# AbnerVictor/OOD-GAN-inversion

Measured on AMD Instinct MI355X. Metric: 1024² face inversions/sec (100 W+ steps), higher is better.
Workload: dtype f16-split (hi+lo f16 operands, f32 accumulate): 3 MFMA/product in every forward conv (fp32-equivalent), 2 in the input-gradient convs (back-propagated gradient rounded to f16 before each contraction, weights keep hi+lo); dL/dW+ vs the float64 reference 1.4e-5..3.6e-5 ('f16s': 1.3e-5..2.6e-5, the ref

## Files before the change

include/oodgan.h:

```cpp
#ifndef OODGAN_H
#define OODGAN_H

#ifdef __cplusplus
extern "C" {
#endif

#define OODGAN_OK 0
#define OODGAN_E_ARG (-1)
#define OODGAN_E_LAUNCH (-2)
#define OODGAN_E_STATE (-3)
#define OODGAN_E_NODEV (-4)

int oodgan_version(void);
const char* oodgan_last_error(void);
int oodgan_device_count(void);
int oodgan_set_tunable(const char* name, long value);
long oodgan_get_tunable(const char* name);
long oodgan_dispatch_count(const char* name);
int oodgan_dispatch_reset(void);
int oodgan_zero(void* p, long bytes, void* stream);

void* oodgan_plan_create(void);
int oodgan_plan_destroy(void* plan);
int oodgan_plan_record_begin(void* plan);
// ... 10 lines not shown
int oodgan_bias_act_bwd(const float* gy, const float* y, float* gx, float* gbias, int B, int C, long HW,
                        float slope, float scale, void* stream);

int oodgan_upfirdn2d(const float* x, const float* kernel, float* y, int planes, int in_h, int in_w,
                     int in_pitch, int out_pitch, int kh, int kw, int up_x, int up_y, int down_x, int down_y,
                     int pad_x0, int pad_x1, int pad_y0, int pad_y1, void* stream);

int oodgan_blur_bias_act(const float* x, const float* kernel, float* y, int B, int C, int in_h, int in_w,
                         int in_pitch, int kh, int kw, int pad0, int pad1, const float* bias, const float* noise,
                         int noise_batch, const float* noise_w, int act, void* stream);


int oodgan_style_affine_fwd(const float* latent, const float* wcat, const float* bcat, const int* row_lat,
                            float* s, int B, int L, int S, int R, float scale, float lr_mul, void* stream);
int oodgan_style_affine_bwd(const float* gs, const float* wcat, const int* lat_start, float* glat,
                            int B, int L, int S, int R, float scale, void* stream);
int oodgan_equal_linear(const float* x, const float* w, const float* b, float* y, int B, int in_dim, int out_dim,
                        float scale, float lr_mul, int activate, void* stream);
int oodgan_equal_linear_grouped(const float* x, const float* w, const float* b, float* y, int B, int G, int in_dim, int out_dim,
                                float scale, float lr_mul, int activate, void* stream);
int oodgan_pixel_norm(const float* x, float* y, int B, int S, void* stream);


int oodgan_weight_sqsum(const float* w, float* wsq, int Co, int Ci, int KK, void* stream);
int oodgan_demod_fwd(const float* s, int s_stride, const float* wsq, float* d, int d_stride,
                     int B, int Ci, int Co, float scale, void* stream);
int oodgan_demod_bwd(const float* s, int s_stride, const float* wsq, const float* d, int d_stride,
                     const float* r, float* gs, int gs_stride, int B, int Ci, int Co, float scale, void* stream);

int oodgan_pack_conv3x3(const float* w, float* wpk, int Co, int Ci, float scale, int transpose, int flip,
                        void* stream);

#define OODGAN_CONV_S1 0
#define OODGAN_CONV_T2 1
#define OODGAN_CONV_S2 2

#define OODGAN_ACT_NONE 0
#define OODGAN_ACT_LRELU 1
#define OODGAN_ACT_PRELU 2

struct oodgan_actbwd_fuse;
typedef struct oodgan_conv_args {
    const float* x;
    const float* wpk;
    const float* in_scale;
    const float* in_shift;
    const float* out_scale;
    const float* bias;
    const float* noise;
    const float* noise_w;
    const float* slope;
    const float* dotx;
    float* dot_part;
    float* y;
    int B, K, M, Hin, Win;
    int in_pitch, out_pitch;
    int in_scale_stride, out_scale_stride;
    int noise_batch;
    int mode, act;
    int dot_nparts;
    const float* in_mul2;
    int x_sform;
    void* ys;
    const float* ys_scale;
    int ys_scale_stride;
    const float* rgb_w;
    const float* rgb_s;
    float* rgb_y;
    int rgb_s_stride;
    float rgb_scale;
    const struct oodgan_actbwd_fuse* fuse;
    int dot_actgrad;
    int groups;
    int y_fform;
    int x_fform;
    int dotx_fform;
    int dotx_sform;
    const float* dotx_scale;
    int dotx_scale_stride;
    void* workspace;
    long workspace_bytes;
    unsigned* ys_vmax;
    int x_hi_only;
} oodgan_conv_args;

typedef struct oodgan_actbwd_fuse {
    const float* g_rgb;
    const float* w_rgb;
    const float* s_rgb;
    const float* noise;
    const float* noise_w;
    const float* bias;
    const float* dscale;
    const float* mul2;
    void* ys;
    float* part_r;
    float* part_t;
    float* part_max;
    int s_rgb_stride, noise_batch, dscale_stride;
    float rgb_scale;
    long nmax;
    int ys_hi_only;
} oodgan_actbwd_fuse;

int oodgan_conv3x3(const oodgan_conv_args* args, void* stream);

long oodgan_pack_conv3x3_f16s_bytes(int Co, int Ci, int transpose);
int oodgan_pack_conv3x3_f16s(const float* w, void* wpk16, float* unscale2, int Co, int Ci, float scale, int transpose,
                             int flip, void* stream);
int oodgan_conv3x3_f16s(const oodgan_conv_args* args, const float* unscale2, void* stream);
int oodgan_conv3x3_f16s_nparts(int mode, int Hin, int Win);
int oodgan_conv3x3_f16s_nparts2(int mode, int Hin, int Win, int x_sform);
int oodgan_conv3x3_s2_fuse_supported(int B, int K, int M, int Hin, int Win);
int oodgan_conv3x3_s2_grouped_supported(int B, int K, int M, int groups, int Hin, int Win);
int oodgan_conv3x3_s1_actgrad_supported(int B, int K, int M, int H, int W);
int oodgan_conv3x3_s1_ys_supported(int B, int K, int M, int H, int W);
int oodgan_conv3x3_xf_supported(int B, int K, int M, int H, int W);
int oodgan_conv3x3_xf_nparts(int B, int H, int W);
long oodgan_conv3x3_tiny_workspace(int mode, int B, int K, int M, int Hin, int Win);

#define OODGAN_VMAX_SLOTS 64
long oodgan_sform_bytes(int B, int C, int H, int W);
int oodgan_to_sform(const float* x, const float* scale, int scale_stride, const float* shift, int shift_stride,
                    const float* mul2, void* out, int B, int C, int H, int W, int in_pitch, unsigned* vmax, void* stream);
long oodgan_sform_phases_bytes(int B, int C, int H, int W);
int oodgan_from_sform(const void* xs, const float* scale, int scale_stride, float* y, int B, int C, int H, int W, void* stream);
int oodgan_blurT_to_sform_phases(const float* g, const float* kernel, const float* scale, int scale_stride,
                                 const float* mul2, void* out, int B, int C, int H, int W, void* stream);
int oodgan_to_sform_phases(const float* x, const float* scale, int scale_stride, const float* mul2, void* out, int B,
                           int C, int H, int W, int in_pitch, void* stream);
int oodgan_to_sform_phases_padtl(const float* x, const float* scale, int scale_stride, const float* mul2, void* out, int B,
                                 int C, int H, int W, int in_pitch, void* stream);
int oodgan_conv3x3_nparts(int mode, int Hin, int Win);
int oodgan_absmax_scaled(const float* x, const float* s, int s_stride, unsigned* vmax, int B, int C, long HW, void* stream);
int oodgan_fwd_range_update(unsigned* vmax, float* q, int* flag, int n, void* stream);
int oodgan_fwd_range_plan(const float* s_all, const float* d_all, const int* row_layer, const int* drow_layer, const float* q,
                          float* s_sc, float* d_sc, int B, int R, int DR, int row0, int nrows, int drow0, int ndrows,
                          void* stream);

int oodgan_blur_act_sform(const float* z, const float* kernel, float* y, void* ys, const float* ys_scale, int ys_scale_stride,
                          const float* bias, const float* noise, int noise_batch, const float* noise_w, int act, int B, int C,
                          int H, int W, int in_pitch, unsigned* vmax, void* stream);
int oodgan_blur_act_fform(const float* z, const float* kernel, float* y, const float* ys_scale, int ys_scale_stride,
                          const float* bias, const float* noise, int noise_batch, const float* noise_w, int act,
                          int B, int C, int H, int W, int in_pitch, unsigned* vmax, int kernel_rank_one, void* stream);
int oodgan_upconv_vblur_supported(int B, int K, int M, int H, int W);
int oodgan_upconv_vblur_fform(const void* xs, const void* wpk2, long wset_bytes, const float* unscale4, const float* kh4,
                              const float* out_scale, int out_scale_stride, const float* bias, const float* noise, int noise_batch,
                              const float* noise_w, int act, const float* ys_scale, int ys_scale_stride, unsigned* vmax, float* y,
                              int B, int K, int M, int H, int W, void* stream);
int oodgan_blur_act_sform_sep(const float* z, const float* kernel, float* y, void* ys, const float* ys_scale, int ys_scale_stride,
                              const float* bias, const float* noise, int noise_batch, const float* noise_w, int act, int B, int C,
                              int H, int W, int in_pitch, unsigned* vmax, int kernel_rank_one, void* stream);

int oodgan_act_bwd_sform_nparts(int H, int W);
int oodgan_act_bwd_sform(const float* g_feat, const float* out, const float* noise, int noise_batch, const float* noise_w,
                         const float* bias, const float* g_rgb, const float* w_rgb, const float* s_rgb, int s_rgb_stride,
                         float rgb_scale, const float* dscale, int dscale_stride, const float* mul2, void* ys, float* part_r,
                         float* part_t, float* part_max, int B, int C, int H, int W, void* stream);
int oodgan_act_bwd_sform_f(const float* out_f, const float* noise, int noise_batch, const float* noise_w, const float* bias,
                           const float* g_rgb, const float* w_rgb, const float* s_rgb, int s_rgb_stride, float rgb_scale,
                           const float* dscale, int dscale_stride, const float* mul2, void* ys, float* part_r, float* part_t,
                           float* part_max, int B, int C, int H, int W, void* stream);
int oodgan_from_fform(const float* f, float* y, int B, int C, int H, int W, void* stream);
int oodgan_act_bwd_blurT_nparts(int H, int W);
int oodgan_act_bwd_blurT_pre_supported(int H, int W);
int oodgan_act_bwd_blurT_sform_phases(const float* g_feat, const float* out, const float* noise, int noise_batch,
                                      const float* noise_w, const float* bias, const float* g_rgb, const float* w_rgb,
                                      const float* s_rgb, int s_rgb_stride, float rgb_scale, const float* dscale,
                                      int dscale_stride, const float* mul2, const float* kernel, void* out_phases,
                                      float* part_r, float* part_t, float* part_max, int B, int C, int H, int W, void* stream);
int oodgan_act_bwd_blurT_hi_supported(int H, int W);
int oodgan_conv3x3_s1_xh_supported(int B, int K, int M, int H, int W);
int oodgan_act_bwd_blurT_sform_phases_hi(const float* g_feat, const float* out, const float* noise, int noise_batch, const float* noise_w,
                                         const float* bias, const float* dscale, int dscale_stride, const float* mul2, const float* kernel,
                                         void* out_phases, float* part_r, float* part_max, int B, int C, int H, int W, void* stream);
int oodgan_absmax_scale_check(const float* part, long n, float* state, int* flag, void* stream);

typedef struct oodgan_reduce_job {
    const float* part;
    float* out;
    int B, C, nparts, out_stride, accumulate;
    const float* part2;
    const float* scale2;
    int nparts2, scale2_stride;
} oodgan_reduce_job;
typedef struct oodgan_demod_bwd_job {
    const float* s; const float* wsq; const float* d; const float* r; float* gs;
    int s_stride, d_stride, gs_stride, B, Ci, Co;
    float scale;
} oodgan_demod_bwd_job;
typedef struct oodgan_demod_fwd_job {
    const float* s; const float* wsq; float* d;
    int s_stride, d_stride, B, Ci, Co;
    float scale;
} oodgan_demod_fwd_job;
typedef struct oodgan_scale_check_job {
    const float* part; long n; float* state;
} oodgan_scale_check_job;
int oodgan_reduce_batch(const oodgan_reduce_job* jobs, int njobs, void* stream);
int oodgan_demod_bwd_batch(const oodgan_demod_bwd_job* jobs, int njobs, void* stream);
int oodgan_demod_fwd_batch(const oodgan_demod_fwd_job* jobs, int njobs, void* stream);
int oodgan_absmax_scale_check_batch(const oodgan_scale_check_job* jobs, int njobs, int* flag, void* stream);

long oodgan_hform_bytes(int B, int C, int H, int W);
int oodgan_to_hform(const float* x, void* out, int B, int C, int H, int W, void* stream);
int oodgan_from_hform(const void* in, float* y, int B, int C, int H, int W, void* stream);
long oodgan_modconv_f16_wbytes(int B, int M, int K);
int oodgan_modconv_f16_pack(const float* weight, const float* style, int style_stride, float scale, int demodulate,
                            int act, void* wpk, int B, int M, int K, void* stream);
int oodgan_modconv_f16_pack_affine(const float* weight, const float* latent, int latent_stride, const float* mod_weight,
                                   const float* mod_bias, int S, float scale, int demodulate, int act, void* wpk, int B, int M,
                                   int K, void* stream);
int oodgan_modconv_f16(const void* x, const void* wpk, const float* noise, int noise_batch, const float* noise_w,
                       const float* bias, int act, void* y, int B, int K, int M, int H, int W, void* stream);
int oodgan_reduce_parts(const float* part, float* out, long rows, int nparts, int accumulate, void* stream);
int oodgan_reduce_parts_cols(const float* part, float* out, int B, int C, int nparts, int out_stride, int accumulate,
                             void* stream);


int oodgan_torgb_fwd(const float* x, const float* w, const float* s, int s_stride, const float* bias,
                     const float* skip, const float* kernel, float* y, int B, int Ci, int H, int W,
                     float scale, void* stream);
int oodgan_torgb_fwd_sform(const float* x, const float* w, const float* s, int s_stride, const float* bias,
                           const float* skip, const float* kernel, float* y, void* ys, const float* ys_scale,
                           int ys_scale_stride, int B, int Ci, int H, int W, float scale, unsigned* vmax, void* stream);
int oodgan_rgb_finish(const float* partial, const float* bias, const float* skip, const float* kernel, float* y, int B, int H,
                      int W, void* stream);
int oodgan_rgb_finish_parts(const float* partial, int nparts, const float* bias, const float* skip, const float* kernel, float* y, int B,
                            int H, int W, void* stream);

int oodgan_feature_modulation(const float* x, const float* c0, const float* c1, float* y, long n, int mode, void* stream);

int oodgan_act_bwd_fused(const float* g_feat, const float* out, const float* noise, int noise_batch,
                         const float* noise_w, const float* bias, const float* g_rgb, const float* w_rgb,
                         const float* s_rgb, int s_rgb_stride, float rgb_scale, float* g_pre,
                         float* part_r, float* part_rgb, int B, int C, long HW, void* stream);
int oodgan_act_bwd_nparts(long HW);
int oodgan_act_bwd_fused_max(const float* g_feat, const float* out, const float* noise, int noise_batch,
                             const float* noise_w, const float* bias, const float* g_rgb, const float* w_rgb,
                             const float* s_rgb, int s_rgb_stride, float rgb_scale, float* g_pre,
                             float* part_r, float* part_rgb, float* part_max, const float* dscale, int dscale_stride, int B,
                             int C, long HW, void* stream);
int oodgan_absmax_scale(const float* part, long n, float* out2, void* stream);
int oodgan_absmax_scale_clear(float* part, long n, float* out2, void* stream);


int oodgan_mse_fwd_bwd(const float* img, const float* target, float* gimg, float* part, float* loss,
                       int B, long CHW, float grad_mul, void* stream);
int oodgan_mse_nparts(long CHW);
int oodgan_mse_fwd_bwd_row(const float* img, const float* target, float* gimg, float* part, float* loss_table,
                           const int* row_dev, int nrows, int B, long CHW, float grad_mul, void* stream);
int oodgan_composite_mse_fwd_bwd(const float* img, const float* target, const float* beta, float* gimg, float* comp, float* part,
                                 float* loss, int B, int C, long HW, int wrt_gen, float grad_mul, void* stream);
int oodgan_composite_mse_fwd_bwd_row(const float* img, const float* target, const float* beta, float* gimg, float* comp, float* part,
                                     float* loss_table, const int* row_dev, int nrows, int B, int C, long HW, int wrt_gen,
                                     float grad_mul, void* stream);
int oodgan_scale_by_plane(float* g, const float* beta, int B, int C, long HW, void* stream);
int oodgan_loss_weight_from_alpha(const float* alpha, float* beta, long n, int power, void* stream);
// ... 59 lines not shown
```

ood-gan-inversion_amd/csrc/bwd_producers.hip:

```cpp
#include "common.hpp"
#include "sform.hpp"
#include <type_traits>
#include <cstdint>
#include <cstdlib>

using namespace oodgan;

typedef _Float16 half8 __attribute__((ext_vector_type(8)));
typedef _Float16 half2v __attribute__((ext_vector_type(2)));

namespace {

struct SPDims { int KC, Hq, Wq; long plane; };

__host__ __device__ inline SPDims sp_dims(int C, int H, int W) {
    SPDims d;
    d.KC = (C + 15) / 16;
    d.Hq = (H + 7) / 8 * 8 + 2;
    d.Wq = (W + 31) / 32 * 32 + 2;
    d.plane = (long)d.Hq * d.Wq * 4;
    return d;
}

struct ActArgs {
    const float* g_feat;
    const float* out;
    const float* noise;
    const float* noise_w;
    const float* bias;
    const float* g_rgb;
    const float* w_rgb;
    const float* s_rgb;
    const float* dscale;
    const float* mul2;
    float* part_r;
    float* part_t;
    float* part_max;
    int noise_batch, s_rgb_stride, dscale_stride;
    float rgb_scale;
    int B, C, H, W, nparts;
};


struct ConstSel { int which, c; bool has; };
__device__ __forceinline__ ConstSel const_sel(const ActArgs& a, int kc) {
    const int t = threadIdx.x;
    ConstSel s;
    s.which = t >> 4;
    s.c = kc * 16 + (t & 15);
    s.has = s.which < 4 ? a.g_rgb != nullptr : s.which == 4 ? a.bias != nullptr : a.dscale != nullptr;
    return s;
}

__device__ __forceinline__ float fetch_const(const ActArgs& a, int b, int kc) {
    float raw = 0.f;
    if (threadIdx.x < 112) {
        const ConstSel s = const_sel(a, kc);
        const int cc = min(s.c, a.C - 1);
        const float* src = a.part_r;
        if (s.has) {
            if (s.which < 3) src = a.w_rgb + s.which * a.C + cc;
            else if (s.which == 3) src = a.s_rgb + (long)b * a.s_rgb_stride + cc;
            else if (s.which == 4) src = a.bias + cc;
            else src = a.dscale + (long)b * a.dscale_stride + cc;
        }
        raw = *src;
    }
    return raw;
}

__device__ __forceinline__ void put_const(const ActArgs& a, int kc, float (*cst)[16], float raw) {
    const int t = threadIdx.x;
    if (t < 112) {
        const ConstSel s = const_sel(a, kc);
        const float m2 = a.mul2 ? a.mul2[1] : 1.f;
        float v;
        if (s.which < 3) v = s.has ? raw * a.rgb_scale : 0.f;
        else if (s.which <= 4) v = s.has ? raw : 0.f;
        else if (s.which == 5) v = (s.has ? raw : 1.f) * m2;
        else v = s.has ? fabsf(raw) : 1.f;
        cst[t >> 4][t & 15] = s.c < a.C ? v : 0.f;
    }
}

__device__ __forceinline__ void load_consts(const ActArgs& a, int b, int kc, float (*cst)[16]) { put_const(a, kc, cst, fetch_const(a, b, kc)); }

constexpr int kP1Chunk = 512;
constexpr int kP1Pitch = kP1Chunk + 4;

__global__ __launch_bounds__(256) void act_bwd_sform_kernel(const ActArgs a, uint4* __restrict__ ys, const SDims yd) {
    __shared__ __attribute__((aligned(16))) float lst[16 * kP1Pitch];
    __shared__ float cst[7][16];
    __shared__ float redm[4];
    const int KC = yd.KC;
    const int bk = blockIdx.y, b = bk / KC, kc = bk % KC;
    const int tid = threadIdx.x;
    const long HW = (long)a.H * a.W;
    load_consts(a, b, kc, cst);
    __syncthreads();
    const float nw = a.noise ? (a.noise_w ? a.noise_w[0] : 1.f) : 0.f;
    const float* np = a.noise ? a.noise + (long)(a.noise_batch > 1 ? b : 0) * HW : nullptr;
    const float* gr = a.g_rgb ? a.g_rgb + (long)b * 3 * HW : nullptr;
    const long p0 = (long)blockIdx.x * kP1Chunk;
    float amax = 0.f;
    {
        const int ch = tid >> 4, q = tid & 15, c = kc * 16 + ch;
        const float w0 = cst[0][ch], w1 = cst[1][ch], w2 = cst[2][ch], sr = cst[3][ch], bv = cst[4][ch], ds = cst[5][ch];
        const long cbase = ((long)b * a.C + c) * HW;
        float acc_r = 0.f, acc_t = 0.f;
#pragma unroll
        for (int k = 0; k < kP1Chunk / 64; ++k) {
            const int lp = 4 * (q + 16 * k);
            const long p = p0 + lp;
            float4 v = make_float4(0.f, 0.f, 0.f, 0.f);
            if (c < a.C && p < HW) {
                const float4 o4 = *reinterpret_cast<const float4*>(a.out + cbase + p);
                float4 g4 = make_float4(0.f, 0.f, 0.f, 0.f), nz = g4, r0 = g4, r1 = g4, r2 = g4;
                if (a.g_feat) g4 = *reinterpret_cast<const float4*>(a.g_feat + cbase + p);
                if (np) nz = *reinterpret_cast<const float4*>(np + p);
                if (gr) {
                    r0 = *reinterpret_cast<const float4*>(gr + p);
                    r1 = *reinterpret_cast<const float4*>(gr + HW + p);
                    r2 = *reinterpret_cast<const float4*>(gr + 2 * HW + p);
// ... 283 lines not shown
    if (tid == 0) a.part_max[((long)b * sp.KC + kc) * a.nparts + tile] = fmaxf(fmaxf(redm[0], redm[1]), fmaxf(redm[2], redm[3]));
    const int ch = tid >> 4, tq = tid & 15;
    const int yrow = tq >> 1, xh = tq & 1;
    float o[32];
    if (sep_ok) {
        float kv[4], kh[4];
#pragma unroll
        for (int i = 0; i < 4; ++i) { kv[i] = ksep[3 - i]; kh[i] = ksep[4 + 3 - i]; }
#pragma unroll
        for (int hf = 0; hf < 2; ++hf) {
            float tmp[20];
#pragma unroll
            for (int j = 0; j < 20; ++j) tmp[j] = 0.f;
#pragma unroll
            for (int aa = 0; aa < 4; ++aa) {
                const float2* row = reinterpret_cast<const float2*>(lin + ch * BT_Q + (yrow + aa) * BT_P + 32 * xh + 16 * hf + 2);
#pragma unroll
                for (int j = 0; j < 10; ++j) {
                    const float2 v = row[j];
                    tmp[2 * j] += kv[aa] * v.x;
                    tmp[2 * j + 1] += kv[aa] * v.y;
                }
            }
#pragma unroll
            for (int j = 0; j < 16; ++j)
                o[16 * hf + j] = kh[0] * tmp[j] + kh[1] * tmp[j + 1] + kh[2] * tmp[j + 2] + kh[3] * tmp[j + 3];
        }
    } else {
#pragma unroll
        for (int j = 0; j < 32; ++j) o[j] = 0.f;
#pragma unroll
        for (int aa = 0; aa < 4; ++aa) {
            const float* row = lin + ch * BT_Q + (yrow + aa) * BT_P + 32 * xh + 2;
            float win[35];
#pragma unroll
            for (int j = 0; j < 35; ++j) win[j] = row[j];
#pragma unroll
            for (int bb = 0; bb < 4; ++bb) {
                const float kv = kf[(3 - aa) * 4 + (3 - bb)];
#pragma unroll
                for (int j = 0; j < 32; ++j) o[j] += kv * win[j + bb];
            }
        }
    }
    const float sc_ = cst[5][ch];
    __syncthreads();
    float* lst = lin;
#pragma unroll
    for (int j = 0; j < 32; ++j) {
        const int Xl = 32 * xh + j;
        const int ph = (yrow & 1) * 2 + (Xl & 1);
        lst[ch * BX_CH + ph * BX_PH + (yrow >> 1) * 32 + ((Xl >> 1) ^ ((yrow & 4) << 1))] = o[j] * sc_;
    }
    __syncthreads();
#pragma unroll
    for (int rep = 0; rep < 2; ++rep) {
        const int pos = tid + rep * 256;
        const int ph = pos >> 7, il = (pos >> 5) & 3, jl = pos & 31;
        const int i = i0 + il, j = j0 + jl;
        if (i > H || j > W) continue;
        half8 h0, h1, l0, l1;
#pragma unroll
        for (int cc = 0; cc < 16; ++cc) {
            float v = lst[cc * BX_CH + ph * BX_PH + il * 32 + (jl ^ ((il & 2) << 2))];
            const int Y = 2 * i + (ph >> 1), X = 2 * j + (ph & 1);
            if (Y > 2 * H || X > 2 * W) v = 0.f;
            const _Float16 hh = (_Float16)v;
            const _Float16 ll = (_Float16)(v - (float)hh);
            if (cc < 8) { h0[cc] = hh; l0[cc] = ll; } else { h1[cc - 8] = hh; l1[cc - 8] = ll; }
        }
        half8* rec = reinterpret_cast<half8*>(outp + ((((long)b * sp.KC + kc) * 4 + ph) * sp.plane + ((long)i * sp.Wq + j) * 4));
        rec[0] = h0; rec[1] = h1; rec[2] = l0; rec[3] = l1;
    }
}


struct StripGeo {
    int nstrips, nseg, seg_rows;
    int tiles_x, tiles_y;
    int extra;
    int hi_only;
};

template <int QN, bool XTRA, bool PRE>
__global__ __launch_bounds__(16 * QN) __attribute__((amdgpu_waves_per_eu((PRE && !XTRA) ? 4 : 2, 4))) void act_bwd_blurT_strip_kernel(const ActArgs a, const float* __restrict__ kern, uint4* __restrict__ outp,
                                                                   int H, int W, SPDims sp, StripGeo geo) {
    constexpr int SW = 4 * QN, NT = 16 * QN, NWV = NT / 64;
    constexpr int BS_RP = SW + 4;
    constexpr int BS_GP = SW + 4;
    static_assert(QN == 16, "a channel row is one DPP row of 16 lanes");
    __shared__ __attribute__((aligned(16))) float gat[2][2][16][BS_GP];
    __shared__ float cst[7][16];
    __shared__ float redm[NWV];
    const int tid = threadIdx.x;
    int w;
    {
        const int total = gridDim.x, bid = blockIdx.x, xcd = bid & 7, idx = bid >> 3, q = total >> 3, r = total & 7;
        w = (xcd < r ? xcd * (q + 1) : r * (q + 1) + (xcd - r) * q) + idx;
    }
    const int strip = w % geo.nstrips; w /= geo.nstrips;
    const int seg = w % geo.nseg; w /= geo.nseg;
    const int kc = w % sp.KC, b = w / sp.KC;
    const int Hg = 2 * H, Wg = 2 * W;
    const long HW = (long)Hg * Wg;
    const int i0 = seg * geo.seg_rows;
    const int i1 = min(i0 + geo.seg_rows, H + 1);
    const int X0 = SW * strip, j0 = (SW / 2) * strip;
    const bool xtra = XTRA && strip == geo.nstrips - 1;
    const float cval = fetch_const(a, b, kc);
    float kp[4][4];
#pragma unroll
    for (int aa = 0; aa < 4; ++aa)
#pragma unroll
        for (int bb = 0; bb < 4; ++bb) kp[aa][bb] = kern[(3 - aa) * 4 + (3 - bb)];
    float kv[4], kh[4];
    bool rank1 = kp[0][0] != 0.f;
    {
        float kmax = 0.f;
#pragma unroll
        for (int aa = 0; aa < 4; ++aa)
#pragma unroll
            for (int bb = 0; bb < 4; ++bb) kmax = fmaxf(kmax, fabsf(kp[aa][bb]));
#pragma unroll
        for (int aa = 0; aa < 4; ++aa) {
            kv[aa] = rank1 ? kp[aa][0] / kp[0][0] : 0.f;
            kh[aa] = kp[0][aa];
        }
#pragma unroll
        for (int aa = 0; aa < 4; ++aa)
#pragma unroll
            for (int bb = 0; bb < 4; ++bb) rank1 = rank1 && fabsf(kp[aa][bb] - kv[aa] * kh[bb]) <= 1e-7f * kmax;
#pragma unroll
        for (int aa = 0; aa < 4; ++aa)
            kv[aa] = __builtin_bit_cast(float, __builtin_amdgcn_readfirstlane(__builtin_bit_cast(int, kv[aa])));
    }
    const int ch = tid / QN, q = tid % QN, c = kc * 16 + ch;
    float bv = 0.f, sc_ = 0.f;
    const int csw = (ch >> 3) & 1;
    const float nw = a.noise ? (a.noise_w ? a.noise_w[0] : 1.f) : 0.f;
    const float* np = a.noise ? a.noise + (long)(a.noise_batch > 1 ? b : 0) * HW : nullptr;
    const long cbase = ((long)b * a.C + c) * HW;
    const bool cok = c < a.C;
    const int gxm = X0 + 4 * q;
    const bool vm = cok && gxm + 3 < Wg;
    const bool vl = cok && q == 0 && X0 >= 2;
    const bool vr = cok && q == QN - 1 && X0 + SW < Wg;

    struct Rows { float4 o[PRE ? 1 : 2], g[2], n[2]; float2 oe[PRE ? 1 : 2], ge[2]; };
    const int gxc = min(gxm, Wg - 4);
    const int ecol = q == QN - 1 ? min(X0 + SW, Wg - 2) : max(X0 - 2, 0);
    const long cbase_c = ((long)b * a.C + min(c, a.C - 1)) * HW;
    const float* gsrc = a.g_feat ? a.g_feat : a.out;
    const bool has_g = a.g_feat != nullptr;
    const float* nsrc = np ? np : gsrc + cbase_c;
    const bool has_n = np != nullptr && gxm + 3 < Wg;
    auto load_rows = [&](int i, Rows& R) __attribute__((always_inline)) {
#pragma unroll
        for (int rr = 0; rr < 2; ++rr) {
            const int rc = min(max(2 * i + 1 + rr, 0), Hg - 1);
            const long p = cbase_c + (long)rc * Wg;
            if (!PRE) {
                R.o[PRE ? 0 : rr] = *reinterpret_cast<const float4*>(a.out + p + gxc);
                R.oe[PRE ? 0 : rr] = *reinterpret_cast<const float2*>(a.out + p + ecol);
            }
            R.g[rr] = *reinterpret_cast<const float4*>(gsrc + p + gxc);
            R.ge[rr] = *reinterpret_cast<const float2*>(gsrc + p + ecol);
            R.n[rr] = *reinterpret_cast<const float4*>(nsrc + (long)rc * Wg + gxc);
        }
    };

    float acc_r = 0.f, amax = 0.f;
    float pend[3][4], pendx[3] = {0.f, 0.f, 0.f};
#pragma unroll
    for (int k = 0; k < 3; ++k)
#pragma unroll
        for (int e = 0; e < 4; ++e) pend[k][e] = 0.f;

    auto step = [&](int i, const Rows& R, auto r1_c) __attribute__((always_inline)) {
        constexpr bool R1 = decltype(r1_c)::value;
        float done[2][4];
        float (*gt)[16][BS_GP] = gat[i & 1];
#pragma unroll
        for (int rr = 0; rr < 2; ++rr) {
            const int r = 2 * i + 1 + rr;
            const bool rok = r >= 0 && r < Hg;
            const bool own = r >= 2 * i0 + 1 || (seg == 0 && r == 0);
            const bool mg = rok && vm && has_g, mn = rok && has_n;
            const bool me0 = rok && has_g && (vl || vr), me1 = rok && has_g && vl;
            const float gv[4] = {mg ? R.g[rr].x : 0.f, mg ? R.g[rr].y : 0.f, mg ? R.g[rr].z : 0.f, mg ? R.g[rr].w : 0.f};
            float gp[4], e0, e1;
            const float nv[4] = {mn ? R.n[rr].x : 0.f, mn ? R.n[rr].y : 0.f, mn ? R.n[rr].z : 0.f, mn ? R.n[rr].w : 0.f};
            const float ge0 = me0 ? R.ge[rr].x : 0.f, ge1 = me1 ? R.ge[rr].y : 0.f;
            if (PRE) {
#pragma unroll
                for (int e = 0; e < 4; ++e) {
                    gp[e] = gv[e];
                    if (own) {
                        acc_r -= gp[e] * (nw * nv[e] + bv);
                        amax = fmaxf(amax, fabsf(gp[e]));
                    }
                }
                e0 = ge0;
                e1 = ge1;
            } else {
                const float4 o4 = R.o[PRE ? 0 : rr];
                const float2 oe = R.oe[PRE ? 0 : rr];
                const bool mo = rok && vm;
                const float ov[4] = {mo ? o4.x : 0.f, mo ? o4.y : 0.f, mo ? o4.z : 0.f, mo ? o4.w : 0.f};
#pragma unroll
                for (int e = 0; e < 4; ++e) {
                    const float o = ov[e];
                    gp[e] = gv[e] * (o > 0.f ? kSqrt2 : 0.2f * kSqrt2);
                    if (own) {
                        const float ycv = (o > 0.f ? o * kInvPos : o * kInvNeg) - nw * nv[e] - bv;
                        acc_r += gp[e] * ycv;
                        amax = fmaxf(amax, fabsf(gp[e]));
                    }
                }
                e0 = ge0 * (oe.x > 0.f ? kSqrt2 : 0.2f * kSqrt2);
                e1 = ge1 * (oe.y > 0.f ? kSqrt2 : 0.2f * kSqrt2);
            }
            float lz = __builtin_bit_cast(float, __builtin_amdgcn_update_dpp(0, __builtin_bit_cast(int, gp[2]), 0x111, 0xF, 0xF, false));
            float lw = __builtin_bit_cast(float, __builtin_amdgcn_update_dpp(0, __builtin_bit_cast(int, gp[3]), 0x111, 0xF, 0xF, false));
            float rx = __builtin_bit_cast(float, __builtin_amdgcn_update_dpp(0, __builtin_bit_cast(int, gp[0]), 0x101, 0xF, 0xF, false));
            if (q == 0) { lz = e0; lw = e1; }
            if (q == QN - 1) rx = e0;
            const float x[7] = {lz, lw, gp[0], gp[1], gp[2], gp[3], rx};
            float dxx = 0.f;
            if constexpr (R1) {
#pragma unroll
                for (int e = 0; e < 4; ++e) {
                    const float hr = __builtin_fmaf(kh[3], x[e + 3], __builtin_fmaf(kh[2], x[e + 2], __builtin_fmaf(kh[1], x[e + 1], kh[0] * x[e])));
                    done[rr][e] = __builtin_fmaf(kv[3], hr, pend[0][e]);
                    pend[0][e] = __builtin_fmaf(kv[2], hr, pend[1][e]);
                    pend[1][e] = __builtin_fmaf(kv[1], hr, pend[2][e]);
                    pend[2][e] = kv[0] * hr;
                }
                if (XTRA && xtra && q == QN - 1) {
                    const float hr = __builtin_fmaf(kh[1], x[5], kh[0] * x[4]);
                    dxx = __builtin_fmaf(kv[3], hr, pendx[0]);
                    pendx[0] = __builtin_fmaf(kv[2], hr, pendx[1]);
                    pendx[1] = __builtin_fmaf(kv[1], hr, pendx[2]);
                    pendx[2] = kv[0] * hr;
                }
            } else {
                float fresh[4];
#pragma unroll
                for (int e = 0; e < 4; ++e) {
                    done[rr][e] = pend[0][e] + (kp[3][0] * x[e] + kp[3][1] * x[e + 1] + kp[3][2] * x[e + 2] + kp[3][3] * x[e + 3]);
                    pend[0][e] = pend[1][e] + (kp[2][0] * x[e] + kp[2][1] * x[e + 1] + kp[2][2] * x[e + 2] + kp[2][3] * x[e + 3]);
                    pend[1][e] = pend[2][e] + (kp[1][0] * x[e] + kp[1][1] * x[e + 1] + kp[1][2] * x[e + 2] + kp[1][3] * x[e + 3]);
                    fresh[e] = kp[0][0] * x[e] + kp[0][1] * x[e + 1] + kp[0][2] * x[e + 2] + kp[0][3] * x[e + 3];
                }
#pragma unroll
                for (int e = 0; e < 4; ++e) pend[2][e] = fresh[e];
                if (XTRA && xtra && q == QN - 1) {
                    dxx = pendx[0] + (kp[3][0] * x[4] + kp[3][1] * x[5]);
                    pendx[0] = pendx[1] + (kp[2][0] * x[4] + kp[2][1] * x[5]);
                    pendx[1] = pendx[2] + (kp[1][0] * x[4] + kp[1][1] * x[5]);
                    pendx[2] = kp[0][0] * x[4] + kp[0][1] * x[5];
                }
            }
            if (XTRA && xtra && q == QN - 1 && i >= i0) gt[rr][ch][SW ^ csw] = dxx * sc_;
        }
        if (i >= i0) {
#pragma unroll
            for (int rr = 0; rr < 2; ++rr) {
                const float d0 = done[rr][0] * sc_, d1 = done[rr][1] * sc_, d2 = done[rr][2] * sc_, d3 = done[rr][3] * sc_;
                *reinterpret_cast<float4*>(&gt[rr][ch][4 * q]) = csw ? make_float4(d1, d0, d3, d2) : make_float4(d0, d1, d2, d3);
            }
        }
        __syncthreads();
        if (i >= i0) {
            static_assert(4 * SW == NT, "one gather task per thread");
            const int ph = tid / SW, v = tid % SW;
            const int py = ph >> 1, px = ph & 1, jl = v >> 1, hf = v & 1;
            const int j = j0 + jl, Xl = 2 * jl + px;
            if (j <= W) {
                const bool zero = (2 * i + py > 2 * H) || (X0 + Xl > 2 * W);
                half8 h8, l8;
#pragma unroll
                for (int cc = 0; cc < 8; ++cc) {
                    float val = gt[py][8 * hf + cc][Xl ^ hf];
                    if (zero) val = 0.f;
                    const _Float16 hh = (_Float16)val;
                    h8[cc] = hh;
                    l8[cc] = (_Float16)(val - (float)hh);
                }
                if (geo.hi_only) {
                    half8* recp = reinterpret_cast<half8*>(outp + ((((long)b * sp.KC + kc) * 4 + ph) * sp.plane + ((long)i * sp.Wq + j) * 2));
                    recp[hf] = h8;
                } else {
                    half8* recp = reinterpret_cast<half8*>(outp + ((((long)b * sp.KC + kc) * 4 + ph) * sp.plane + ((long)i * sp.Wq + j) * 4));
                    recp[hf] = h8;
                    recp[2 + hf] = l8;
                }
            }
            if (XTRA && xtra && tid < 16) {
                const int ph = tid >> 2, sl = tid & 3, py = ph >> 1, px = ph & 1;
                const bool zero = px == 1 || (2 * i + py > 2 * H);
                half8 o8;
#pragma unroll
                for (int cc = 0; cc < 8; ++cc) {
                    float val = zero ? 0.f : gt[py][8 * (sl & 1) + cc][SW ^ (sl & 1)];
                    const _Float16 hh = (_Float16)val;
                    o8[cc] = (sl & 2) ? (_Float16)(val - (float)hh) : hh;
                }
                if (geo.hi_only) {
                    if (sl < 2) reinterpret_cast<half8*>(outp + ((((long)b * sp.KC + kc) * 4 + ph) * sp.plane + ((long)i * sp.Wq + W) * 2))[sl] = o8;
                } else {
                    half8* recp = reinterpret_cast<half8*>(outp + ((((long)b * sp.KC + kc) * 4 + ph) * sp.plane + ((long)i * sp.Wq + W) * 4));
                    recp[sl] = o8;
                }
            }
        }
    };

    Rows ra, rb;
    load_rows(i0 - 2, ra);
    put_const(a, kc, cst, cval);
    __syncthreads();
    bv = cst[4][ch];
    sc_ = cst[5][ch];
    int i = i0 - 2;
    auto walk = [&](auto r1_c) __attribute__((always_inline)) {
        for (; i + 1 < i1; i += 2) {
            load_rows(i + 1, rb);
            step(i, ra, r1_c);
            load_rows(i + 2, ra);
            step(i + 1, rb, r1_c);
        }
        if (i < i1) step(i, ra, r1_c);
    };
    if (rank1) walk(std::true_type{});
    else walk(std::false_type{});

#pragma unroll
    for (int o = QN / 2; o > 0; o >>= 1) acc_r += __shfl_xor(acc_r, o, 64);
    auto put = [&](float* tab, int row, int rows_used, float v) {
        const int r1 = row == rows_used - 1 ? geo.tiles_y : row + 1;
        const int c1 = strip == geo.nstrips - 1 ? geo.tiles_x : strip + 1;
        for (int r = row; r < r1; ++r)
            for (int cx = strip; cx < c1; ++cx) tab[(long)r * geo.tiles_x + cx] = (r == row && cx == strip) ? v : 0.f;
    };
    if (q == 0 && cok) put(a.part_r + ((long)b * a.C + c) * a.nparts, seg, geo.nseg, acc_r);
    amax *= cst[6][ch];
#pragma unroll
    for (int o = 32; o > 0; o >>= 1) amax = fmaxf(amax, __shfl_xor(amax, o, 64));
    if ((tid & 63) == 0) redm[tid >> 6] = amax;
    __syncthreads();
    if (tid == 0) {
        float m = redm[0];
        for (int wv = 1; wv < NWV; ++wv) m = fmaxf(m, redm[wv]);
        put(a.part_max + ((long)b * sp.KC + kc) * a.nparts, seg, geo.nseg, m);
    }
}

__global__ __launch_bounds__(1024) void absmax_scale_check_kernel(const float* __restrict__ part, long n, float* __restrict__ state,
                                                                  int* __restrict__ flag) {
    __shared__ float red[16];
    float m = 0.f;
    bool bad = false;
    for (long i = threadIdx.x; i < n; i += 4096) {
        float v[4];
#pragma unroll
        for (int u = 0; u < 4; ++u) v[u] = i + 1024 * u < n ? part[i + 1024 * u] : 0.f;
#pragma unroll
        for (int u = 0; u < 4; ++u) {
            if (!isfinite(v[u])) bad = true;
            m = fmaxf(m, fabsf(v[u]));
        }
    }
#pragma unroll
    for (int o = 32; o > 0; o >>= 1) m = fmaxf(m, __shfl_xor(m, o, 64));
    if (__any(bad) && (threadIdx.x & 63) == 0) atomicOr(flag, 2);
    if ((threadIdx.x & 63) == 0) red[threadIdx.x >> 6] = m;
    __syncthreads();
    if (threadIdx.x == 0) {
        m = red[0];
#pragma unroll
        for (int i = 1; i < 16; ++i) m = fmaxf(m, red[i]);
        const float used = state[1];
        if (m > 0.f && isfinite(m)) {
            const float scaled = m * used;
            if (!(scaled >= 0.00390625f && scaled < 32768.f)) atomicOr(flag, 1);
        }
        int e = 0;
        if (m > 0.f && isfinite(m)) e = 9 - (int)floorf(log2f(m));
        e = e < -100 ? -100 : (e > 100 ? 100 : e);
        state[0] = ldexpf(1.f, -e);
        state[1] = ldexpf(1.f, e);
    }
}

int fill_args(ActArgs& a, const float* g_feat, const float* out, const float* noise, int noise_batch, const float* noise_w,
              const float* bias, const float* g_rgb, const float* w_rgb, const float* s_rgb, int s_rgb_stride, float rgb_scale,
              const float* dscale, int dscale_stride, const float* mul2, float* part_r, float* part_t, float* part_max, int B,
              int C, int H, int W) {
    OODGAN_REQUIRE(part_r && part_max && mul2 && B > 0 && C > 0 && H > 0 && W > 0, "act_bwd producer: bad args");
    OODGAN_REQUIRE(out || (g_feat && !g_rgb), "act_bwd producer: without out, g_feat must be the pre-activation gradient (no ToRGB branch)");
    OODGAN_REQUIRE(!g_rgb || (w_rgb && s_rgb && part_t), "act_bwd producer: rgb branch needs w_rgb, s_rgb and part_t");
    OODGAN_REQUIRE(noise == nullptr || noise_batch == 1 || noise_batch == B, "act_bwd producer: noise_batch");
    OODGAN_REQUIRE((W % 4) == 0, "act_bwd producer: W must be a multiple of 4");
    a.g_feat = g_feat; a.out = out; a.noise = noise; a.noise_w = noise_w; a.bias = bias;
    a.g_rgb = g_rgb; a.w_rgb = w_rgb; a.s_rgb = s_rgb; a.dscale = dscale; a.mul2 = mul2;
    a.part_r = part_r; a.part_t = g_rgb ? part_t : nullptr; a.part_max = part_max;
    a.noise_batch = noise_batch; a.s_rgb_stride = s_rgb_stride; a.dscale_stride = dscale_stride; a.rgb_scale = rgb_scale;
    a.B = B; a.C = C; a.H = H; a.W = W;
    return OODGAN_OK;
}

}

extern "C" int oodgan_act_bwd_sform_nparts(int H, int W) { return (int)(((long)H * W + kP1Chunk - 1) / kP1Chunk); }

extern "C" int oodgan_act_bwd_sform(const float* g_feat, const float* out, const float* noise, int noise_batch,
                                    const float* noise_w, const float* bias, const float* g_rgb, const float* w_rgb,
                                    const float* s_rgb, int s_rgb_stride, float rgb_scale, const float* dscale, int dscale_stride,
                                    const float* mul2, void* ys, float* part_r, float* part_t, float* part_max, int B, int C,
                                    int H, int W, void* stream) {
    ActArgs a;
    int rc = fill_args(a, g_feat, out, noise, noise_batch, noise_w, bias, g_rgb, w_rgb, s_rgb, s_rgb_stride, rgb_scale, dscale,
                       dscale_stride, mul2, part_r, part_t, part_max, B, C, H, W);
    if (rc != OODGAN_OK) return rc;
    OODGAN_REQUIRE(ys != nullptr, "act_bwd_sform: null output");
    const SDims yd = sform_dims(C, H, W);
    a.nparts = oodgan_act_bwd_sform_nparts(H, W);
    OODGAN_REQUIRE((long)B * yd.KC <= 65535, "act_bwd_sform: B*C too large");
    hipLaunchKernelGGL(act_bwd_sform_kernel, dim3(a.nparts, B * yd.KC), dim3(256), 0, as_stream(stream), a,
                       reinterpret_cast<uint4*>(ys), yd);
    return check_launch("act_bwd_sform");
}

extern "C" int oodgan_act_bwd_sform_f(const float* out_f, const float* noise, int noise_batch, const float* noise_w, const float* bias,
                                      const float* g_rgb, const float* w_rgb, const float* s_rgb, int s_rgb_stride, float rgb_scale,
                                      const float* dscale, int dscale_stride, const float* mul2, void* ys, float* part_r, float* part_t,
                                      float* part_max, int B, int C, int H, int W, void* stream) {
    ActArgs a;
    int rc = fill_args(a, nullptr, out_f, noise, noise_batch, noise_w, bias, g_rgb, w_rgb, s_rgb, s_rgb_stride, rgb_scale, dscale,
                       dscale_stride, mul2, part_r, part_t, part_max, B, C, H, W);
    if (rc != OODGAN_OK) return rc;
    OODGAN_REQUIRE(ys != nullptr && (C % 16) == 0 && (reinterpret_cast<uintptr_t>(out_f) & 15) == 0,
                   "act_bwd_sform_f: needs ys, C %% 16 == 0 and a 16-byte aligned F-form input");
    const SDims yd = sform_dims(C, H, W);
    a.nparts = oodgan_act_bwd_sform_nparts(H, W);
    OODGAN_REQUIRE((long)B * yd.KC <= 65535, "act_bwd_sform_f: B*C too large");
    hipLaunchKernelGGL(act_bwd_sform_f_kernel, dim3(a.nparts, B * yd.KC), dim3(256), 0, as_stream(stream), a,
                       reinterpret_cast<uint4*>(ys), yd);
    return check_launch("act_bwd_sform_f");
}

extern "C" int oodgan_from_fform(const float* f, float* y, int B, int C, int H, int W, void* stream) {
    OODGAN_REQUIRE(f && y && B > 0 && C > 0 && (C % 16) == 0 && H > 0 && W > 0, "from_fform: bad args");
    const long HW = (long)H * W, total = (long)B * C * HW;
    hipLaunchKernelGGL(from_fform_kernel, dim3(stream_grid(total, 256)), dim3(256), 0, as_stream(stream), f, y, C, HW, total);
    return check_launch("from_fform");
}

static bool blurT_strip_enabled() { return oodgan::tunable(oodgan::OODGAN_TUN_BLURT_STRIP) != 0; }

extern "C" int oodgan_act_bwd_blurT_pre_supported(int H, int W) { return H >= 32 && W >= 32 && blurT_strip_enabled() ? 1 : 0; }

extern "C" int oodgan_act_bwd_blurT_nparts(int H, int W) { return ((W + 1 + 31) / 32) * ((H + 1 + 3) / 4); }

static int act_bwd_blurT_impl(const float* g_feat, const float* out, const float* noise, int noise_batch, const float* noise_w, const float* bias,
                              const float* g_rgb, const float* w_rgb, const float* s_rgb, int s_rgb_stride, float rgb_scale, const float* dscale,
                              int dscale_stride, const float* mul2, const float* kernel, void* out_phases, float* part_r, float* part_t, float* part_max,
                              int B, int C, int H, int W, void* stream, int hi_only);

extern "C" int oodgan_act_bwd_blurT_hi_supported(int H, int W) { return H >= 32 && W >= 32 && blurT_strip_enabled() ? 1 : 0; }

extern "C" int oodgan_act_bwd_blurT_sform_phases(const float* g_feat, const float* out, const float* noise, int noise_batch,
                                                 const float* noise_w, const float* bias, const float* g_rgb,
                                                 const float* w_rgb, const float* s_rgb, int s_rgb_stride, float rgb_scale,
                                                 const float* dscale, int dscale_stride, const float* mul2,
                                                 const float* kernel, void* out_phases, float* part_r, float* part_t,
                                                 float* part_max, int B, int C, int H, int W, void* stream) {
    return act_bwd_blurT_impl(g_feat, out, noise, noise_batch, noise_w, bias, g_rgb, w_rgb, s_rgb, s_rgb_stride, rgb_scale, dscale, dscale_stride, mul2, kernel,
                              out_phases, part_r, part_t, part_max, B, C, H, W, stream, 0);
}

extern "C" int oodgan_act_bwd_blurT_sform_phases_hi(const float* g_feat, const float* out, const float* noise, int noise_batch,
                                                    const float* noise_w, const float* bias, const float* dscale, int dscale_stride,
                                                    const float* mul2, const float* kernel, void* out_phases, float* part_r, float* part_max,
                                                    int B, int C, int H, int W, void* stream) {
    OODGAN_REQUIRE(oodgan_act_bwd_blurT_hi_supported(H, W), "act_bwd_blurT hi-only records: the strip walk only (H, W >= 32, tunable blurt_strip)");
    return act_bwd_blurT_impl(g_feat, out, noise, noise_batch, noise_w, bias, nullptr, nullptr, nullptr, 0, 0.f, dscale, dscale_stride, mul2, kernel,
                              out_phases, part_r, nullptr, part_max, B, C, H, W, stream, 1);
}

static int act_bwd_blurT_impl(const float* g_feat, const float* out, const float* noise, int noise_batch, const float* noise_w, const float* bias,
                              const float* g_rgb, const float* w_rgb, const float* s_rgb, int s_rgb_stride, float rgb_scale, const float* dscale,
                              int dscale_stride, const float* mul2, const float* kernel, void* out_phases, float* part_r, float* part_t, float* part_max,
                              int B, int C, int H, int W, void* stream, int hi_only) {
    ActArgs a;
    int rc = fill_args(a, g_feat, out, noise, noise_batch, noise_w, bias, g_rgb, w_rgb, s_rgb, s_rgb_stride, rgb_scale, dscale,
                       dscale_stride, mul2, part_r, part_t, part_max, B, C, 2 * H, 2 * W);
    if (rc != OODGAN_OK) return rc;
    OODGAN_REQUIRE(kernel && out_phases, "act_bwd_blurT: null tensor");
    OODGAN_REQUIRE((reinterpret_cast<uintptr_t>(out) & 15) == 0 && (!g_feat || (reinterpret_cast<uintptr_t>(g_feat) & 15) == 0),
                   "act_bwd_blurT: unaligned input");
    OODGAN_REQUIRE(out || oodgan_act_bwd_blurT_pre_supported(H, W), "act_bwd_blurT: the pre-activated form (out == NULL) exists only in the "
                   "strip walk (H, W >= 32)");
    const SPDims d = sp_dims(C, H, W);
    const int tiles_x = (W + 1 + 31) / 32, tiles_y = (H + 1 + 3) / 4;
    a.nparts = tiles_x * tiles_y;
    const long nb = (long)tiles_x * tiles_y * d.KC * B;
    OODGAN_REQUIRE(nb < (1L << 31), "act_bwd_blurT: grid too large");
    if (!g_rgb && !part_t && H >= 32 && W >= 32 && blurT_strip_enabled()) {
        constexpr int QN = 16;
        StripGeo geo;
        geo.hi_only = hi_only;
        geo.extra = ((W % (2 * QN)) == 0 && W <= 32) ? 1 : 0;
        geo.nstrips = geo.extra ? W / (2 * QN) : (W + 1 + 2 * QN - 1) / (2 * QN);
        geo.tiles_x = tiles_x;
        geo.tiles_y = tiles_y;
        const long base = (long)B * d.KC * geo.nstrips;
        long nseg = (4L * 1024) / base;
        if (nseg < 1) nseg = 1;
        int seg_rows = (int)((H + 1 + nseg - 1) / nseg);
        if (seg_rows < 16) seg_rows = 16;
        geo.seg_rows = seg_rows;
        geo.nseg = (H + 1 + seg_rows - 1) / seg_rows;
        OODGAN_REQUIRE(geo.nseg <= tiles_y && geo.nstrips <= tiles_x, "act_bwd_blurT strip: slot table too small");
        const long nbs = base * geo.nseg;
#define OODGAN_STRIP_LAUNCH(X, P)                                                                                              \
    hipLaunchKernelGGL((act_bwd_blurT_strip_kernel<QN, X, P>), dim3((unsigned)nbs), dim3(256), 0, as_stream(stream), a, kernel, \
                       reinterpret_cast<uint4*>(out_phases), H, W, d, geo)
        if (geo.extra) {
            if (out) OODGAN_STRIP_LAUNCH(true, false); else OODGAN_STRIP_LAUNCH(true, true);
        } else {
            if (out) OODGAN_STRIP_LAUNCH(false, false); else OODGAN_STRIP_LAUNCH(false, true);
        }
#undef OODGAN_STRIP_LAUNCH
        return check_launch("act_bwd_blurT_sform_phases/strip");
    }
    OODGAN_REQUIRE(!hi_only, "act_bwd_blurT hi-only records: not reachable (strip walk refused this call)");
    if (g_rgb)
        hipLaunchKernelGGL(act_bwd_blurT_sp_kernel<true>, dim3((unsigned)nb), dim3(256), 0, as_stream(stream), a, kernel,
                           reinterpret_cast<uint4*>(out_phases), H, W, d, tiles_x, tiles_y);
    else
        hipLaunchKernelGGL(act_bwd_blurT_sp_kernel<false>, dim3((unsigned)nb), dim3(256), 0, as_stream(stream), a, kernel,
                           reinterpret_cast<uint4*>(out_phases), H, W, d, tiles_x, tiles_y);
    return check_launch("act_bwd_blurT_sform_phases");
}

extern "C" int oodgan_absmax_scale_check(const float* part, long n, float* state, int* flag, void* stream) {
    OODGAN_REQUIRE(part && state && flag && n > 0, "absmax_scale_check: bad args");
    hipLaunchKernelGGL(absmax_scale_check_kernel, dim3(1), dim3(1024), 0, as_stream(stream), part, n, state, flag);
    return check_launch("absmax_scale_check");
}
```

ood-gan-inversion_amd/csrc/common.hpp:

```cpp
#pragma once
#include <hip/hip_runtime.h>
#include <cstdio>
#include <cstdarg>
#include <functional>
#include <utility>
#include "../../include/oodgan.h"

namespace oodgan {
struct PlanRec;
extern thread_local PlanRec* tl_plan_rec;
extern int g_null_launch;
void plan_append(std::function<void()>&& f);
template <class F>
inline void launch_rec(F&& f) {
    f();
    if (__builtin_expect(tl_plan_rec != nullptr, 0)) plan_append(std::function<void()>(std::forward<F>(f)));
}
}
#undef hipLaunchKernelGGL
#define hipLaunchKernelGGL(kernelName, numBlocks, numThreads, memPerBlock, streamId, ...)                                        \
    ::oodgan::launch_rec([=]() {                                                                                                 \
        if (!::oodgan::g_null_launch) (kernelName)<<<(numBlocks), (numThreads), (memPerBlock), (streamId)>>>(__VA_ARGS__);      \
    })

namespace oodgan {

void set_error(const char* fmt, ...);

enum { OODGAN_TUN_S1_BIG_MIN_ITEMS = 0, OODGAN_TUN_S2_BIG_MIN_ITEMS, OODGAN_TUN_T2_BIG_MIN_ITEMS, OODGAN_TUN_BLURT_STRIP, OODGAN_TUN_BLUR_STRIP, OODGAN_TUN_UPVB_WAVES, OODGAN_TUN_FEWOUT_QUAD, OODGAN_TUN_TINY_MID_MAX, OODGAN_TUN_STRIPX_WAVES, OODGAN_TUN_COUNT };
long tunable(int id);

enum { OODGAN_DC_STRIPX = 0, OODGAN_DC_STRIP, OODGAN_DC_S1BIG, OODGAN_DC_S1V2, OODGAN_DC_S1PP, OODGAN_DC_TINY, OODGAN_DC_T2BIG,
       OODGAN_DC_T2V2, OODGAN_DC_T2GEN, OODGAN_DC_S2BIG, OODGAN_DC_S2V2, OODGAN_DC_S2GEN, OODGAN_DC_UPVB,
       OODGAN_DC_S1BIG_YS, OODGAN_DC_S2BIG_FUSE, OODGAN_DC_S2BIG_DOTXS,
       OODGAN_DC_S1BIG_G2, OODGAN_DC_S2BIG_G2, OODGAN_DC_STRIPX_G2, OODGAN_DC_S2BIG_XH, OODGAN_DC_S1BIG_XH,
       OODGAN_DC_COMPOSITE_MSE, OODGAN_DC_COUNT };
void count_dispatch(int id);

bool bound_device_ok(const char* what);

inline int check_launch(const char* what) {
    hipError_t e = hipGetLastError();
    if (e != hipSuccess) {
        set_error("%s: %s", what, hipGetErrorString(e));
        return OODGAN_E_LAUNCH;
    }
    return OODGAN_OK;
}

#define OODGAN_REQUIRE(cond, ...)          \
    do {                                    \
        if (!(cond)) {                      \
            oodgan::set_error(__VA_ARGS__); \
            return OODGAN_E_ARG;            \
        }                                   \
    } while (0)

constexpr float kSqrt2 = 1.4142135623730951f;
constexpr float kInvPos = 1.f / kSqrt2, kInvNeg = 1.f / (0.2f * kSqrt2);
constexpr int kWave = 64;

inline hipStream_t as_stream(void* s) { return reinterpret_cast<hipStream_t>(s); }

inline int stream_grid(long work_items, int block) {
    long g = (work_items + block - 1) / block;
    if (g > 2048) g = 2048;
    if (g < 1) g = 1;
    return static_cast<int>(g);
}

__device__ __forceinline__ float wave_sum(float v) {
#pragma unroll
    for (int o = 32; o > 0; o >>= 1) v += __shfl_xor(v, o, 64);
    return v;
}

__device__ __forceinline__ float row_sum16(const float* __restrict__ p, int n, int l) {
    float v[4];
#pragma unroll
    for (int u = 0; u < 4; ++u) v[u] = p[min(l + 16 * u, n - 1)];
#pragma unroll
    for (int u = 0; u < 4; ++u) v[u] = l + 16 * u < n ? v[u] : 0.f;
    float r = (v[0] + v[1]) + (v[2] + v[3]);
    r += __shfl_xor(r, 8, 64);
    r += __shfl_xor(r, 4, 64);
    r += __shfl_xor(r, 2, 64);
    r += __shfl_xor(r, 1, 64);
    return r;
}

__device__ __forceinline__ float row_sum_wave(const float* __restrict__ p, int n, int lane) {
    float a0 = 0.f, a1 = 0.f, a2 = 0.f, a3 = 0.f;
    for (int i0 = lane; i0 < n; i0 += 512) {
        float v[8];
#pragma unroll
        for (int u = 0; u < 8; ++u) v[u] = p[min(i0 + 64 * u, n - 1)];
#pragma unroll
        for (int u = 0; u < 8; ++u) v[u] = i0 + 64 * u < n ? v[u] : 0.f;
        a0 += v[0] + v[4]; a1 += v[1] + v[5]; a2 += v[2] + v[6]; a3 += v[3] + v[7];
    }
    return wave_sum((a0 + a1) + (a2 + a3));
}

__device__ __forceinline__ float row_sum(const float* __restrict__ p, int n, int lane) {
    return n <= 64 ? row_sum16(p, n, lane & 15) : row_sum_wave(p, n, lane);
}

__device__ __forceinline__ float demod_dot(const float* __restrict__ sp, const float* __restrict__ wp, int Ci, int lane) {
    float a0 = 0.f, a1 = 0.f, a2 = 0.f, a3 = 0.f;
    for (int c0 = lane; c0 < Ci; c0 += 512) {
        float sv[8], wv[8];
#pragma unroll
        for (int u = 0; u < 8; ++u) {
            const int ci = min(c0 + 64 * u, Ci - 1);
            sv[u] = sp[ci];
            wv[u] = wp[ci];
        }
#pragma unroll
        for (int u = 0; u < 8; ++u) {
// ... 78 lines not shown
```

ood-gan-inversion_amd/csrc/conv_f16s.hip:

```cpp
#include "conv_common.hpp"
#include <cstdlib>
#include <cstdint>

extern "C" int oodgan_conv3x3_f16s_nparts(int mode, int Hin, int Win);

using namespace oodgan;

namespace oodgan {
int launch_s1pp(const oodgan_conv_args& a, const void* wpk16, const float* unscale, hipStream_t st);
int launch_s1v2(const oodgan_conv_args& a, const void* wpk16, const float* unscale, hipStream_t st);
bool s1_strip_eligible(const oodgan_conv_args& a);
bool s1_big_eligible(const oodgan_conv_args& a);
int launch_s1_big(const oodgan_conv_args& a, const void* wpk16, const float* unscale, hipStream_t st);
int launch_s1_strip(const oodgan_conv_args& a, const void* wpk16, const float* unscale, hipStream_t st);
int launch_s1_stripx(const oodgan_conv_args& a, const void* wpk16, const float* unscale, hipStream_t st);
bool tiny_eligible(const oodgan_conv_args& a);
int launch_tiny(const oodgan_conv_args& a, const void* wpk16, const float* unscale, hipStream_t st);
int launch_t2v2(const oodgan_conv_args& a, const void* wpk16, const float* unscale, hipStream_t st);
int launch_s2v2(const oodgan_conv_args& a, const void* wpk16, const float* unscale, hipStream_t st);
bool s2_big_eligible(const oodgan_conv_args& a);
bool t2_big_eligible(const oodgan_conv_args& a);
int launch_t2_big(const oodgan_conv_args& a, const void* wpk16, const float* unscale, hipStream_t st);
int launch_s2_big(const oodgan_conv_args& a, const void* wpk16, const float* unscale, hipStream_t st);
}
// ... 311 lines not shown
}

__global__ __launch_bounds__(256) void pack_f16s_kernel(const float* __restrict__ w, _Float16* __restrict__ out, int Co, int Ci,
                                                        int Mp, float scale, int transpose, int flip,
                                                        const float* __restrict__ sc2) {
    const int K = transpose ? Co : Ci, M = transpose ? Ci : Co;
    const int nchunk = (K + CK - 1) / CK;
    const long total = (long)nchunk * 9 * 2 * Mp * 8;
    const float s2 = sc2[1] * scale;
    for (long e = blockIdx.x * 256L + threadIdx.x; e < total; e += (long)gridDim.x * 256) {
        const int j = (int)(e & 7);
        long r = e >> 3;
        const int m = (int)(r % Mp); r /= Mp;
        const int h = (int)(r & 1); r >>= 1;
        const int tap = (int)(r % 9);
        const int t = (int)(r / 9);
        const int k = t * CK + 8 * h + j;
        float v = 0.f;
        if (m < M && k < K) {
            const int co = transpose ? k : m, ci = transpose ? m : k;
            v = w[((long)co * Ci + ci) * 9 + (flip ? 8 - tap : tap)] * s2;
        }
        const _Float16 hi = (_Float16)v;
        const _Float16 lo = (_Float16)(v - (float)hi);
        const long base = (((long)t * 9 + tap) * 2) * 2;
        out[((base + 0 * 2 + h) * Mp + m) * 8 + j] = hi;
        out[((base + 1 * 2 + h) * Mp + m) * 8 + j] = lo;
    }
}

}

extern "C" int oodgan_conv3x3_f16s_nparts2(int mode, int Hin, int Win, int x_sform) {
    if (mode == OODGAN_CONV_S2 && x_sform) return (((Hin - 1) / 2 + 7) / 8) * (((Win - 1) / 2 + 31) / 32);
    return oodgan_conv3x3_f16s_nparts(mode, Hin, Win);
}

extern "C" int oodgan_conv3x3_f16s_nparts(int mode, int Hin, int Win) {
    if (mode == OODGAN_CONV_S1) return ((Hin + 7) / 8) * ((Win + 31) / 32) ;
    if (mode == OODGAN_CONV_S2) return (((Hin - 1) / 2 + 7) / 8) * (((Win - 1) / 2 + 31) / 32) * 4;
    return 0;
}

extern "C" long oodgan_pack_conv3x3_f16s_bytes(int Co, int Ci, int transpose) {
    const int M = transpose ? Ci : Co, K = transpose ? Co : Ci;
    const long Mp = (M + 63) / 64 * 64;
    return (long)((K + CK - 1) / CK) * 9 * 2 * 2 * Mp * 16;
}

extern "C" int oodgan_pack_conv3x3_f16s(const float* w, void* wpk16, float* unscale2, int Co, int Ci, float scale, int transpose,
                                        int flip, void* stream) {
    OODGAN_REQUIRE(w && wpk16 && unscale2 && Co > 0 && Ci > 0, "pack_conv3x3_f16s: bad args");
    const int M = transpose ? Ci : Co, K = transpose ? Co : Ci;
    const int Mp = (M + 63) / 64 * 64;
    hipStream_t st = as_stream(stream);
    if (hipMemsetAsync(unscale2, 0, 2 * sizeof(float), st) != hipSuccess) {
        set_error("pack_conv3x3_f16s: memset failed");
        return OODGAN_E_LAUNCH;
    }
    hipLaunchKernelGGL(absmax_kernel, dim3(stream_grid((long)Co * Ci * 9, 256 * 16)), dim3(256), 0, st, w, (long)Co * Ci * 9, scale, unscale2);
    hipLaunchKernelGGL(absmax_finish_kernel, dim3(1), dim3(1), 0, st, unscale2);
    const long total = (long)((K + CK - 1) / CK) * 9 * 2 * Mp * 8;
    hipLaunchKernelGGL(pack_f16s_kernel, dim3(stream_grid(total, 256)), dim3(256), 0, st, w, reinterpret_cast<_Float16*>(wpk16),
                       Co, Ci, Mp, scale, transpose, flip, unscale2);
    return check_launch("pack_conv3x3_f16s");
}

extern "C" int oodgan_conv3x3_s1_actgrad_supported(int B, int K, int M, int H, int W) {
    oodgan_conv_args a = {};
    a.mode = OODGAN_CONV_S1; a.x_sform = 1; a.B = B; a.K = K; a.M = M; a.Hin = H; a.Win = W;
    a.y = reinterpret_cast<float*>(1);
    a.dotx = reinterpret_cast<const float*>(1);
    return (s1_strip_eligible(a) || s1_big_eligible(a)) && oodgan_act_bwd_blurT_pre_supported(H / 2, W / 2) && !(H & 1) && !(W & 1) ? 1 : 0;
}

extern "C" int oodgan_conv3x3_s1_xh_supported(int B, int K, int M, int H, int W) {
    oodgan_conv_args a = {};
    a.mode = OODGAN_CONV_S1; a.x_sform = 1; a.B = B; a.K = K; a.M = M; a.Hin = H; a.Win = W;
    a.y = reinterpret_cast<float*>(1);
    a.dotx = reinterpret_cast<const float*>(1);
    return (H > 8 && W > 8 && !s1_strip_eligible(a) && s1_big_eligible(a)) ? 1 : 0;
}

extern "C" int oodgan_conv3x3_s1_ys_supported(int B, int K, int M, int H, int W) {
    oodgan_conv_args a = {};
    a.mode = OODGAN_CONV_S1; a.x_sform = 1; a.B = B; a.K = K; a.M = M; a.Hin = H; a.Win = W;
    a.ys = reinterpret_cast<void*>(1);
    return s1_big_eligible(a) ? 1 : 0;
}

extern "C" int oodgan_conv3x3_f16s(const oodgan_conv_args* args, const float* unscale2, void* stream) {
    OODGAN_REQUIRE(args != nullptr, "conv3x3_f16s: null args");
    const oodgan_conv_args& a = *args;
    OODGAN_REQUIRE(a.x && a.wpk && unscale2 && (a.y || a.x_sform), "conv3x3_f16s: null tensor");
    OODGAN_REQUIRE(a.B > 0 && a.K > 0 && a.M > 0 && a.Hin > 0 && a.Win > 0, "conv3x3_f16s: bad shape");
    OODGAN_REQUIRE(a.act != OODGAN_ACT_PRELU || a.slope, "conv3x3_f16s: PReLU without slopes");
    OODGAN_REQUIRE(a.noise == nullptr || a.noise_batch == 1 || a.noise_batch == a.B, "conv3x3_f16s: noise_batch");
    if (!bound_device_ok("conv3x3_f16s")) return OODGAN_E_ARG;
    if (a.x_fform) {
        OODGAN_REQUIRE(a.x_fform == 1 || a.x_fform == 2, "conv3x3_f16s: x_fform must be 0, 1 or 2");
        count_dispatch(OODGAN_DC_STRIPX);
        return launch_s1_stripx(a, a.wpk, unscale2, as_stream(stream));
    }
    OODGAN_REQUIRE(!a.dotx_fform, "conv3x3_f16s: an F-form dotx exists only with x_fform == 2");
    OODGAN_REQUIRE(a.rgb_y == nullptr || (a.mode == OODGAN_CONV_S1 && a.x_sform), "conv3x3_f16s: fused ToRGB output only for mode S1 with S-form input");
    OODGAN_REQUIRE(a.fuse == nullptr || (a.mode == OODGAN_CONV_S2 && a.x_sform && a.M >= 64),
                   "conv3x3_f16s: the fused activation backward exists only for mode S2 with S-form input and M >= 64");
    OODGAN_REQUIRE(a.groups <= 1 || (a.mode == OODGAN_CONV_S2 && (!a.x_sform || tiny_eligible(a) || s2_big_eligible(a))),
                   "conv3x3_f16s: groups > 1 only for mode S2 with fp32 NCHW input, or a phase-split S-form input of a shape the 8-wave or the skinny-GEMM kernel "
                   "takes (oodgan_conv3x3_s2_grouped_supported; oodgan_conv3x3_tiny_workspace > 0 with a workspace)");
    OODGAN_REQUIRE(!a.y_fform || (a.mode == OODGAN_CONV_S1 && a.x_sform && s1_strip_eligible(a)),
                   "conv3x3_f16s: the F-form output exists only in the strip kernel (mode S1, S-form input, 16 < K,M <= 32)");
    OODGAN_REQUIRE(!a.dot_actgrad || (a.mode == OODGAN_CONV_S1 && a.x_sform && a.dotx && (s1_strip_eligible(a) || s1_big_eligible(a))),
                   "conv3x3_f16s: dot_actgrad exists only in the strip / 8-wave kernels of mode S1 (oodgan_conv3x3_s1_actgrad_supported)");
    OODGAN_REQUIRE(!a.dotx_sform || (a.mode == OODGAN_CONV_S2 && a.x_sform && a.fuse && a.dotx && a.dotx_scale && a.dotx_scale_stride >= a.M &&
                                     !tiny_eligible(a) && s2_big_eligible(a)),
                   "conv3x3_f16s: dotx_sform needs mode S2, a phase-split S-form input, `fuse`, dotx, dotx_scale and a shape of the 8-wave kernel "
                   "(oodgan_conv3x3_s2_fuse_supported)");
    OODGAN_REQUIRE(a.ys_vmax == nullptr || (a.ys != nullptr && a.mode == OODGAN_CONV_S1 && a.x_sform && !tiny_eligible(a) && !s1_strip_eligible(a) && s1_big_eligible(a)),
                   "conv3x3_f16s: ys_vmax only with ys from the 8-wave stride-1 kernel (oodgan_conv3x3_s1_ys_supported)");
    OODGAN_REQUIRE(a.x_hi_only != 2 || (a.x_sform && a.dotx && !tiny_eligible(a) &&
                                        ((a.mode == OODGAN_CONV_S2 && s2_big_eligible(a)) || (a.mode == OODGAN_CONV_S1 && !s1_strip_eligible(a) && s1_big_eligible(a)))),
                   "conv3x3_f16s: x_hi_only = 2 (32-byte hi-only input records) exists only in the two-instruction 8-wave kernels (S-form input, dotx; mode S2 on a "
                   "shape oodgan_conv3x3_s2_fuse_supported accepts, mode S1 on a shape of the 8-wave stride-1 kernel)");
    hipStream_t st = as_stream(stream);
    switch (a.mode) {
        case OODGAN_CONV_S1:
            if (tiny_eligible(a)) { count_dispatch(OODGAN_DC_TINY); return launch_tiny(a, a.wpk, unscale2, st); }
            if (a.x_sform && s1_strip_eligible(a)) { count_dispatch(OODGAN_DC_STRIP); return launch_s1_strip(a, a.wpk, unscale2, st); }
            if (a.x_sform && s1_big_eligible(a)) { count_dispatch(OODGAN_DC_S1BIG); if (a.ys) count_dispatch(OODGAN_DC_S1BIG_YS); return launch_s1_big(a, a.wpk, unscale2, st); }
            OODGAN_REQUIRE(a.rgb_y == nullptr, "conv3x3_f16s: the fused ToRGB output exists only in the strip kernel (16 < K,M <= 32) and, as partial "
                                               "sums together with ys, in the 8-wave kernel (oodgan_conv3x3_s1_ys_supported)");
            if (a.x_sform) { count_dispatch(OODGAN_DC_S1V2); return launch_s1v2(a, a.wpk, unscale2, st); }
            OODGAN_REQUIRE(a.ys == nullptr, "conv3x3_f16s: S-form output needs the S-form input kernel");
            count_dispatch(OODGAN_DC_S1PP);
            return launch_s1pp(a, a.wpk, unscale2, st);
        case OODGAN_CONV_T2:
            if (a.x_sform && t2_big_eligible(a)) { count_dispatch(OODGAN_DC_T2BIG); return launch_t2_big(a, a.wpk, unscale2, st); }
            if (a.x_sform) { count_dispatch(OODGAN_DC_T2V2); return launch_t2v2(a, a.wpk, unscale2, st); }
            count_dispatch(OODGAN_DC_T2GEN);
            return launch_mode<OODGAN_CONV_T2>(a, a.wpk, unscale2, st);
        case OODGAN_CONV_S2:
            OODGAN_REQUIRE((a.Hin & 1) && (a.Win & 1) && a.Hin >= 3 && a.Win >= 3, "conv3x3_f16s S2: input must be odd-sized");
            if (tiny_eligible(a)) { count_dispatch(OODGAN_DC_TINY); return launch_tiny(a, a.wpk, unscale2, st); }
            if (a.x_sform && s2_big_eligible(a)) { count_dispatch(OODGAN_DC_S2BIG); if (a.fuse) count_dispatch(OODGAN_DC_S2BIG_FUSE); if (a.dotx_sform) count_dispatch(OODGAN_DC_S2BIG_DOTXS); return launch_s2_big(a, a.wpk, unscale2, st); }
            if (a.x_sform) { count_dispatch(OODGAN_DC_S2V2); return launch_s2v2(a, a.wpk, unscale2, st); }
            count_dispatch(OODGAN_DC_S2GEN);
            return launch_mode<OODGAN_CONV_S2>(a, a.wpk, unscale2, st);
        default: break;
    }
    set_error("conv3x3_f16s: unknown mode %d", a.mode);
    return OODGAN_E_ARG;
}
```

ood-gan-inversion_amd/csrc/conv_f16s_big.hip:

```cpp
#include "conv_common.hpp"
#include "sform.hpp"
#include <cstdint>
#include <cstdlib>
#include <type_traits>

using namespace oodgan;

typedef _Float16 half8 __attribute__((ext_vector_type(8)));
typedef __attribute__((address_space(3))) void lds_void;

namespace {

constexpr int BG_R = 18, BG_C = 34;
constexpr int BG_XSLOTS = BG_R * BG_C * 4;
constexpr int BG_XPIECES = (BG_XSLOTS + 63) / 64;
constexpr int BG_XBYTES = BG_XPIECES * 1024;
constexpr int BG_WPIECES = 36;
constexpr int BG_STAGE = BG_XBYTES + BG_WPIECES * 1024;
constexpr int BG_PIECES = BG_XPIECES + BG_WPIECES;
constexpr int BG_RED = 2 * BG_STAGE;
constexpr int BG_SMEM = BG_RED + 8 * 64 * 4;

struct BigConv {
    oodgan_conv_args a;
    const uint4* xs;
    SDims xd;
    const float* w_unscale;
    int tiles_x, tiles_y, mblocks, Mp;
    long out_plane;
    SDims yd;
};

constexpr int BG_ZERO = BG_SMEM;
constexpr int BG_ZBYTES = 3584;
constexpr int BG_CST = BG_SMEM + BG_ZBYTES;
constexpr int BG_NZ = BG_CST + 3 * 64 * 4;
constexpr int BG_RGBW = BG_NZ + 2048;
constexpr int BG_SMEM16 = BG_RGBW + 3 * 64 * 4;
typedef float f32x4v __attribute__((ext_vector_type(4)));

#ifdef OODGAN_CLOCK_STAMP
__device__ unsigned long long* g_s1big_stamp = nullptr;
__device__ long g_s1big_stamp_n = 0;
#endif

template <bool DOT, bool PRE, bool YS = false, bool G2 = false>
__global__ __launch_bounds__(512) void conv_f16s_s1big_kernel(const BigConv p, const uint4* __restrict__ wpk16) {
    constexpr int NW = 8, NT = 2;
    extern __shared__ __attribute__((aligned(16))) unsigned char smem[];
    const oodgan_conv_args& a = p.a;
    const int tid = threadIdx.x, lane = tid & 63;
    const int wave = __builtin_amdgcn_readfirstlane(tid >> 6);
    const int n16 = lane & 15, g = lane >> 4;

    int w = xcd_remap(blockIdx.x, gridDim.x);
    const int mblk = w % p.mblocks;
    w /= p.mblocks;
    const int ntile = p.tiles_x * p.tiles_y;
    const int tile = w % ntile, b = w / ntile;
    const int ty = tile / p.tiles_x, tx = tile % p.tiles_x;
    const int r0 = ty * 16, c0 = tx * 32, m0 = mblk * 64;
    const int H = a.Hin, W = a.Win, M = a.M;

    constexpr int NPW = (BG_PIECES + NW - 1) / NW;
    unsigned off[NPW];
    const bool xh = G2 && a.x_hi_only == 2;
    unsigned xmask = 0;
    const int KC = p.xd.KC;
#pragma unroll
    for (int i = 0; i < NPW; ++i) {
        const int pc = wave + NW * i;
        if (pc < BG_XPIECES) {
            int P = pc * 64 + lane;
            if (P >= BG_XSLOTS) P = BG_XSLOTS - 1;
            const int row = P / (BG_C * 4), q = P % (BG_C * 4);
            const int c = q >> 2, sl = ((q & 3) - 2 * ((c >> 2) & 1)) & 3;
            const int rr = min(r0 + row, p.xd.Hp - 1);
            if (xh) {
                off[i] = (unsigned)((((long)rr * p.xd.Wp + (c0 + c)) * 2 + (sl & 1)) * 16);
                if (sl < 2) xmask |= 1u << i;
            } else {
                off[i] = (unsigned)((((long)rr * p.xd.Wp + (c0 + c)) * 4 + sl) * 16);
                xmask |= 1u << i;
            }
        } else {
            xmask |= 1u << i;
            const int u = (pc - BG_XPIECES) * 64 + lane;
            const int row = u >> 6, j = u & 63;
            off[i] = (unsigned)((((long)row * p.Mp) + m0 + j) * 16);
        }
    }
    const unsigned char* xb = reinterpret_cast<const unsigned char*>(p.xs) + (long)b * KC * p.xd.plane * 16;
    const long xplane_bytes = p.xd.plane * 16;
    const unsigned char* wb = reinterpret_cast<const unsigned char*>(wpk16);
    const long wchunk_bytes = (long)36 * p.Mp * 16;
    const int nchunk = (a.K + 15) / 16;
    auto dma_piece = [&](int t, int buf, int i) {
        const int pc = wave + NW * i;
        if (pc >= BG_PIECES) return;
        unsigned char* dst = smem + buf * BG_STAGE;
        const unsigned char* src = (pc < BG_XPIECES ? xb + (long)t * xplane_bytes : wb + (long)t * wchunk_bytes) + off[i];
        if (!G2 || ((xmask >> i) & 1u))
            __builtin_amdgcn_global_load_lds((const __attribute__((address_space(1))) void*)src, (lds_void*)(dst + pc * 1024), 16, 0, 0);
    };
    for (int i = tid; i < BG_ZBYTES / 16; i += 512) reinterpret_cast<uint4*>(smem + BG_ZERO)[i] = make_uint4(0, 0, 0, 0);
    __syncthreads();

    f32x4v acc[4][4];
#pragma unroll
    for (int mt = 0; mt < 4; ++mt)
#pragma unroll
        for (int n = 0; n < 4; ++n) acc[mt][n] = f32x4v{0.f, 0.f, 0.f, 0.f};

    const unsigned laneA = (unsigned)((((g & 1) * 64 + n16) * 16) + (g >> 1) * 4096);
    const unsigned laneA1 = (unsigned)(((g & 1) * 64 + n16) * 16);
    unsigned offBh[4], offBl[4];
#pragma unroll
    for (int pp = 0; pp < 4; ++pp) {
        const int tp = 2 * pp + (g >> 1), ky = tp / 3, kx = tp % 3, col = n16 + kx;
        offBh[pp] = (unsigned)(ky * (BG_C * 64) + col * 64 + ((((g & 1) + 2 * ((col >> 2) & 1)) & 3) << 4));
        offBl[pp] = (unsigned)(ky * (BG_C * 64) + col * 64 + ((((g & 1) + 2 + 2 * ((col >> 2) & 1)) & 3) << 4));
    }
    const int col8 = n16 + 2;
    const unsigned offB1 = (unsigned)(2 * (BG_C * 64) + col8 * 64 + ((((G2 ? (g & 1) : g) + 2 * ((col8 >> 2) & 1)) & 3) << 4));

    struct AF { half8 x[2], y[2]; };
    struct BF { half8 u[4], v[4]; };
    auto load_a = [&](AF& f, const unsigned char* lw, auto pp_c, auto mh_c) {
        constexpr int pp = decltype(pp_c)::value, mh = decltype(mh_c)::value;
// ... 50 lines not shown
#pragma unroll
            for (int i = 0; i < 2; ++i)
#pragma unroll
                for (int n = 0; n < 4; ++n) acc[2 * mh + i][n] = __builtin_amdgcn_mfma_f32_16x16x32_f16(fa.x[i], fb.u[n], acc[2 * mh + i][n], 0, 0, 0);
#pragma unroll
            for (int i = 0; i < 2; ++i)
#pragma unroll
                for (int n = 0; n < 4; ++n) acc[2 * mh + i][n] = __builtin_amdgcn_mfma_f32_16x16x32_f16(fa.y[i], fb.v[n], acc[2 * mh + i][n], 0, 0, 0);
        }
    };
#define BH_IC(n) std::integral_constant<int, n>{}
#define BH_SB() __builtin_amdgcn_sched_barrier(0)
#ifdef OODGAN_CLOCK_STAMP
    const unsigned long long st_t0 = __builtin_amdgcn_s_memtime(), st_r0 = __builtin_amdgcn_s_memrealtime();
#endif
    float cst_o = 0.f, cst_b = 0.f, cst_s = 1.f, rgb_c0 = 0.f, rgb_c1 = 0.f, rgb_c2 = 0.f;
    if (tid < 64 && m0 + tid < M) {
        const int m = m0 + tid;
        cst_o = a.out_scale ? a.out_scale[(long)b * a.out_scale_stride + m] : 1.f;
        if (!DOT && a.bias) cst_b = a.bias[m];
        if (!DOT && a.act == OODGAN_ACT_PRELU) cst_s = a.slope[m];
        if (YS && a.rgb_y) {
            const float sv = a.rgb_scale * a.rgb_s[(long)b * a.rgb_s_stride + m];
            rgb_c0 = sv * a.rgb_w[m]; rgb_c1 = sv * a.rgb_w[M + m]; rgb_c2 = sv * a.rgb_w[2 * M + m];
        }
    }
    const bool has_nz = !DOT && a.noise != nullptr;
    if (has_nz) {
        const int ry = min(r0 + wave * NT + (lane >> 5), H - 1), rx = min(c0 + (lane & 31), W - 1);
        const float* src = a.noise + (long)(a.noise_batch > 1 ? b : 0) * H * W + (long)ry * W + rx;
        __builtin_amdgcn_global_load_lds((const __attribute__((address_space(1))) void*)src, (lds_void*)(smem + BG_NZ + wave * 256), 4, 0, 0);
    }
#pragma unroll
    for (int i = 0; i < NPW; ++i) dma_piece(0, 0, i);
    if (tid < 64) {
        float* cst = reinterpret_cast<float*>(smem + BG_CST);
        cst[tid] = cst_o;
        if (!DOT) { cst[64 + tid] = cst_b; cst[128 + tid] = cst_s; }
        if (YS) {
            float* rw = reinterpret_cast<float*>(smem + BG_RGBW);
            rw[tid] = rgb_c0; rw[64 + tid] = rgb_c1; rw[128 + tid] = rgb_c2;
        }
        __builtin_amdgcn_s_waitcnt(0xC07F);
    }
    for (int t = 0; t < nchunk; ++t) {
        __builtin_amdgcn_s_waitcnt(0x0F70);
        __builtin_amdgcn_s_barrier();
        const bool pf = t + 1 < nchunk;
        const int nb = (t + 1) & 1;
        const unsigned char* lx = smem + (t & 1) * BG_STAGE + (wave * NT) * (BG_C * 64);
        const unsigned char* lw = smem + (t & 1) * BG_STAGE + BG_XBYTES;
        const unsigned col8r = (unsigned)(2 * (BG_C * 64) + col8 * 64 + ((((g & 1) + 2 * ((col8 >> 2) & 1)) & 3) << 4));
        const unsigned char* lz = g < 2 ? lx + col8r : smem + BG_ZERO;
        AF a0, a1;
        BF b0, b1;
#define BH_DMA(i) if (pf && (i) < NPW) dma_piece(t + 1, nb, (i));
        load_b(b0, lx, lz, BH_IC(0), BH_IC(0)); load_b(b0, lx, lz, BH_IC(0), BH_IC(1));
        load_a(a0, lw, BH_IC(0), BH_IC(0));
        BH_SB();
        load_a(a1, lw, BH_IC(0), BH_IC(1)); load_b(b1, lx, lz, BH_IC(1), BH_IC(0)); BH_DMA(0) BH_SB(); mfma_half(a0, b0, BH_IC(0), BH_IC(0)); BH_SB();
        load_a(a0, lw, BH_IC(1), BH_IC(0)); load_b(b1, lx, lz, BH_IC(1), BH_IC(1)); BH_DMA(1) BH_SB(); mfma_half(a1, b0, BH_IC(0), BH_IC(1)); BH_SB();
        load_a(a1, lw, BH_IC(1), BH_IC(1)); load_b(b0, lx, lz, BH_IC(2), BH_IC(0)); BH_DMA(2) BH_SB(); mfma_half(a0, b1, BH_IC(1), BH_IC(0)); BH_SB();
        load_a(a0, lw, BH_IC(2), BH_IC(0)); load_b(b0, lx, lz, BH_IC(2), BH_IC(1)); BH_DMA(3) BH_SB(); mfma_half(a1, b1, BH_IC(1), BH_IC(1)); BH_SB();
        load_a(a1, lw, BH_IC(2), BH_IC(1)); load_b(b1, lx, lz, BH_IC(3), BH_IC(0)); BH_DMA(4) BH_SB(); mfma_half(a0, b0, BH_IC(2), BH_IC(0)); BH_SB();
        load_a(a0, lw, BH_IC(3), BH_IC(0)); load_b(b1, lx, lz, BH_IC(3), BH_IC(1)); BH_DMA(5) BH_SB(); mfma_half(a1, b0, BH_IC(2), BH_IC(1)); BH_SB();
        load_a(a1, lw, BH_IC(3), BH_IC(1)); load_b(b0, lx, lz, BH_IC(4), BH_IC(0)); BH_DMA(6) BH_SB(); mfma_half(a0, b1, BH_IC(3), BH_IC(0)); BH_SB();
        load_a(a0, lw, BH_IC(4), BH_IC(0)); load_b(b0, lx, lz, BH_IC(4), BH_IC(1)); BH_DMA(7) BH_SB(); mfma_half(a1, b1, BH_IC(3), BH_IC(1)); BH_SB();
        load_a(a1, lw, BH_IC(4), BH_IC(1)); BH_DMA(8) BH_SB(); mfma_half(a0, b0, BH_IC(4), BH_IC(0)); BH_SB();
        BH_DMA(9) BH_SB();
        mfma_half(a1, b0, BH_IC(4), BH_IC(1));
#undef BH_DMA
    }
#undef BH_IC
#undef BH_SB
#ifdef OODGAN_CLOCK_STAMP
    if (tid == 0 && g_s1big_stamp && (long)blockIdx.x < g_s1big_stamp_n) {
        g_s1big_stamp[2 * blockIdx.x] = __builtin_amdgcn_s_memtime() - st_t0;
        g_s1big_stamp[2 * blockIdx.x + 1] = __builtin_amdgcn_s_memrealtime() - st_r0;
    }
#endif

    const float us = (p.w_unscale ? p.w_unscale[0] : 1.f) * (a.in_mul2 ? a.in_mul2[0] : 1.f);
    const float nw = (!DOT && a.noise) ? (a.noise_w ? a.noise_w[0] : 1.f) : 0.f;
    float* red = reinterpret_cast<float*>(smem + BG_RED);
    float osc[16], bia[16], slp[16];
    unsigned moff[16], doff[16];
    float dsum[16];
    const bool prelu = !DOT && a.act == OODGAN_ACT_PRELU;
    const float* cst = reinterpret_cast<const float*>(smem + BG_CST);
#pragma unroll
    for (int q = 0; q < 16; ++q) {
        const int j = 16 * (q >> 2) + 4 * g + (q & 3), m = m0 + j;
        const bool mok = m < M;
        osc[q] = cst[j] * us;
        bia[q] = DOT ? 0.f : cst[64 + j];
        slp[q] = DOT ? 1.f : cst[128 + j];
        moff[q] = mok ? (unsigned)((long)m * p.out_plane * 4) : 0xFFFFFFFFu;
        doff[q] = mok ? (unsigned)((long)m * H * W * 4) : 0u;
        dsum[q] = 0.f;
    }
    const bool mfull = m0 + 64 <= M;
    float ysc[16], ysmax = 0.f;
    if (YS) {
#pragma unroll
        for (int q = 0; q < 16; ++q) {
            const int m = m0 + 16 * (q >> 2) + 4 * g + (q & 3);
            ysc[q] = a.ys_scale ? a.ys_scale[(long)b * a.ys_scale_stride + min(m, M - 1)] : 1.f;
        }
    }
#pragma unroll
    for (int n = 0; n < 4; ++n) {
        const int py = r0 + wave * NT + (n >> 1), px = c0 + 16 * (n & 1) + n16;
        const bool ok = py < H && px < W;
        float nz = 0.f;
        if (has_nz) nz = nw * reinterpret_cast<const float*>(smem + BG_NZ)[wave * 64 + (n >> 1) * 32 + 16 * (n & 1) + n16];
        unsigned char* yr = reinterpret_cast<unsigned char*>(a.y) + ((long)b * M * p.out_plane + (long)py * a.out_pitch + px) * 4;
        const unsigned char* dr = DOT ? reinterpret_cast<const unsigned char*>(a.dotx) + ((long)b * M * H * W + (long)py * W + px) * 4 : nullptr;
        float o[16], dv[16];
        if (DOT) {
#pragma unroll
            for (int q = 0; q < 16; ++q) dv[q] = 0.f;
            if (ok) {
                if (mfull) {
#pragma unroll
                    for (int q = 0; q < 16; ++q) dv[q] = *reinterpret_cast<const float*>(dr + doff[q]);
                } else {
#pragma unroll
                    for (int q = 0; q < 16; ++q)
                        if (moff[q] != 0xFFFFFFFFu) dv[q] = *reinterpret_cast<const float*>(dr + doff[q]);
                }
            }
        }
#pragma unroll
        for (int q = 0; q < 16; ++q) {
            const float v = acc[q >> 2][n][q & 3];
            o[q] = v * osc[q];
            if (DOT) {
                dsum[q] += (v * us) * dv[q];
                if (PRE) o[q] *= dv[q] > 0.f ? kSqrt2 : 0.2f * kSqrt2;
            } else {
                o[q] += nz + bia[q];
                if (a.act == OODGAN_ACT_LRELU) o[q] = (o[q] > 0.f ? o[q] : 0.2f * o[q]) * kSqrt2;
                else if (prelu) o[q] = o[q] > 0.f ? o[q] : slp[q] * o[q];
            }
        }
        if (ok && (!YS || a.y != nullptr)) {
            if (mfull) {
#pragma unroll
                for (int q = 0; q < 16; ++q) *reinterpret_cast<float*>(yr + moff[q]) = o[q];
            } else {
#pragma unroll
                for (int q = 0; q < 16; ++q)
                    if (moff[q] != 0xFFFFFFFFu) *reinterpret_cast<float*>(yr + moff[q]) = o[q];
            }
        }
        if (YS && !DOT && ok) {
#pragma unroll
            for (int mt = 0; mt < 4; ++mt) {
                if (m0 + 16 * mt < M) {
                    const float v0 = o[4 * mt] * ysc[4 * mt], v1 = o[4 * mt + 1] * ysc[4 * mt + 1], v2 = o[4 * mt + 2] * ysc[4 * mt + 2],
                                v3 = o[4 * mt + 3] * ysc[4 * mt + 3];
                    ysmax = fmaxf(fmaxf(ysmax, fmaxf(fabsf(v0), fabsf(v1))), fmaxf(fabsf(v2), fabsf(v3)));
                    uint2 hi, lo;
                    split_pair(v0, v1, hi.x, lo.x);
                    split_pair(v2, v3, hi.y, lo.y);
                    unsigned char* rec = reinterpret_cast<unsigned char*>(a.ys) + sform_unit(p.yd, b, (m0 >> 4) + mt, py, px, g >> 1) * 16 + (g & 1) * 8;
                    *reinterpret_cast<uint2*>(rec) = hi;
                    *reinterpret_cast<uint2*>(rec + 32) = lo;
                }
            }
        }
        if (YS && !DOT && a.rgb_y) {
            const float* rw = reinterpret_cast<const float*>(smem + BG_RGBW);
            float c0 = 0.f, c1 = 0.f, c2 = 0.f;
#pragma unroll
            for (int q = 0; q < 16; ++q) {
                const int j = 16 * (q >> 2) + 4 * g + (q & 3);
                c0 += rw[j] * o[q]; c1 += rw[64 + j] * o[q]; c2 += rw[128 + j] * o[q];
            }
            c0 += __shfl_xor(c0, 16, 64); c1 += __shfl_xor(c1, 16, 64); c2 += __shfl_xor(c2, 16, 64);
            c0 += __shfl_xor(c0, 32, 64); c1 += __shfl_xor(c1, 32, 64); c2 += __shfl_xor(c2, 32, 64);
            if (ok && g == 0) {
                float* rp = a.rgb_y + (((long)mblk * a.B + b) * 3) * ((long)H * W) + (long)py * W + px;
                rp[0] = c0; rp[(long)H * W] = c1; rp[2 * (long)H * W] = c2;
            }
        }
    }
    if (YS && a.ys_vmax) record_vmax(a.ys_vmax, b, ysmax);
    if (DOT) {
#pragma unroll
        for (int q = 0; q < 16; ++q) {
            float v = dsum[q];
            v += dpp_take<0xB1, 0xF>(v);
            v += dpp_take<0x4E, 0xF>(v);
            v += dpp_take<0x141, 0xF>(v);
            v += dpp_take<0x140, 0xF>(v);
            if (n16 == 0) red[wave * 64 + 16 * (q >> 2) + 4 * g + (q & 3)] = v;
        }
        __syncthreads();
        if (tid < 64 && m0 + tid < M) {
            float v = 0.f;
#pragma unroll
            for (int wv = 0; wv < NW; ++wv) v += red[wv * 64 + tid];
            float* dp = a.dot_part + ((long)b * M + m0 + tid) * a.dot_nparts;
            const int tx8 = (W + 31) / 32;
            dp[(long)(2 * ty) * tx8 + tx] = v;
            if (2 * ty + 1 < (H + 7) / 8) dp[(long)(2 * ty + 1) * tx8 + tx] = 0.f;
        }
    }
}

}

namespace oodgan {

bool s1_big_eligible(const oodgan_conv_args& a) {
    const int min_k = 64;
    if (!(a.mode == OODGAN_CONV_S1 && a.x_sform && a.K >= min_k && a.M >= 64 && (a.ys == nullptr ? (a.y != nullptr && a.rgb_y == nullptr) : (a.dotx == nullptr && a.M % 16 == 0)) &&
          (a.act == OODGAN_ACT_NONE || a.act == OODGAN_ACT_LRELU || (a.act == OODGAN_ACT_PRELU && a.slope)) && a.in_scale == nullptr &&
          a.in_shift == nullptr &&
          !(a.dotx && (a.noise || a.bias || a.act != OODGAN_ACT_NONE))))
        return false;
    const long items = (long)((a.Hin + 15) / 16) * ((a.Win + 31) / 32) * a.B * ((a.M + 63) / 64);
    return items >= tunable(OODGAN_TUN_S1_BIG_MIN_ITEMS);
}

int launch_s1_big(const oodgan_conv_args& a_in, const void* wpk16, const float* unscale, hipStream_t st) {
    BigConv p;
    p.a = a_in;
    oodgan_conv_args& a = p.a;
    if (a.out_pitch == 0) a.out_pitch = a.Win;
    p.out_plane = (long)a.Hin * a.out_pitch;
    p.xs = reinterpret_cast<const uint4*>(a.x);
    p.xd = sform_dims(a.K, a.Hin, a.Win);
    p.w_unscale = unscale;
    p.tiles_y = (a.Hin + 15) / 16;
    p.tiles_x = (a.Win + 31) / 32;
    p.Mp = (a.M + 63) / 64 * 64;
    p.mblocks = (a.M + 63) / 64;
    p.yd = sform_dims(a.M, a.Hin, a.Win);
    if (a.dotx) {
        OODGAN_REQUIRE(a.dot_part != nullptr, "conv3x3: dotx without dot_part");
        OODGAN_REQUIRE(a.dot_nparts == ((a.Hin + 7) / 8) * p.tiles_x, "conv3x3 f16s S1: dot_nparts %d != %d", a.dot_nparts,
                       ((a.Hin + 7) / 8) * p.tiles_x);
    }
    OODGAN_REQUIRE((long)a.M * p.out_plane * 4 < (1L << 32) && (long)a.M * a.Hin * a.Win * 4 < (1L << 32), "conv3x3 big: plane too large");
    const long total = (long)p.tiles_x * p.tiles_y * a.B * p.mblocks;
    OODGAN_REQUIRE(total > 0 && total < (1L << 31), "conv3x3: grid too large");
    static bool once = ((void)hipFuncSetAttribute(reinterpret_cast<const void*>(&conv_f16s_s1big_kernel<true, false>), hipFuncAttributeMaxDynamicSharedMemorySize, BG_SMEM16),
                        (void)hipFuncSetAttribute(reinterpret_cast<const void*>(&conv_f16s_s1big_kernel<true, true>), hipFuncAttributeMaxDynamicSharedMemorySize, BG_SMEM16),
                        (void)hipFuncSetAttribute(reinterpret_cast<const void*>(&conv_f16s_s1big_kernel<false, false>), hipFuncAttributeMaxDynamicSharedMemorySize, BG_SMEM16),
                        (void)hipFuncSetAttribute(reinterpret_cast<const void*>(&conv_f16s_s1big_kernel<false, false, true>), hipFuncAttributeMaxDynamicSharedMemorySize, BG_SMEM16),
                        (void)hipFuncSetAttribute(reinterpret_cast<const void*>(&conv_f16s_s1big_kernel<true, false, false, true>), hipFuncAttributeMaxDynamicSharedMemorySize, BG_SMEM16),
                        (void)hipFuncSetAttribute(reinterpret_cast<const void*>(&conv_f16s_s1big_kernel<true, true, false, true>), hipFuncAttributeMaxDynamicSharedMemorySize, BG_SMEM16), true);
    (void)once;
    const uint4* w16 = reinterpret_cast<const uint4*>(wpk16);
    OODGAN_REQUIRE(!a.dot_actgrad || a.dotx, "conv3x3 big: dot_actgrad without dotx");
    const bool g2 = a.x_hi_only != 0 && a.dotx != nullptr;
    OODGAN_REQUIRE(a.x_hi_only != 2 || g2, "conv3x3 big: hi-only input records (x_hi_only = 2) need dotx (the two-instruction instances)");
    if (g2) count_dispatch(OODGAN_DC_S1BIG_G2);
    if (g2 && a.x_hi_only == 2) count_dispatch(OODGAN_DC_S1BIG_XH);
    if (a.dot_actgrad && g2) hipLaunchKernelGGL((conv_f16s_s1big_kernel<true, true, false, true>), dim3((unsigned)total), dim3(512), BG_SMEM16, st, p, w16);
    else if (g2) hipLaunchKernelGGL((conv_f16s_s1big_kernel<true, false, false, true>), dim3((unsigned)total), dim3(512), BG_SMEM16, st, p, w16);
    else if (a.dot_actgrad) hipLaunchKernelGGL((conv_f16s_s1big_kernel<true, true>), dim3((unsigned)total), dim3(512), BG_SMEM16, st, p, w16);
    else if (a.dotx) hipLaunchKernelGGL((conv_f16s_s1big_kernel<true, false>), dim3((unsigned)total), dim3(512), BG_SMEM16, st, p, w16);
    else if (a.ys) hipLaunchKernelGGL((conv_f16s_s1big_kernel<false, false, true>), dim3((unsigned)total), dim3(512), BG_SMEM16, st, p, w16);
    else hipLaunchKernelGGL((conv_f16s_s1big_kernel<false, false>), dim3((unsigned)total), dim3(512), BG_SMEM16, st, p, w16);
    return check_launch("conv3x3_f16s_s1big");
}

}

#ifdef OODGAN_CLOCK_STAMP
extern "C" int oodgan_debug_set_stamp_buffer(void* buf, long n) {
    unsigned long long* p = reinterpret_cast<unsigned long long*>(buf);
    if (hipMemcpyToSymbol(HIP_SYMBOL(g_s1big_stamp), &p, sizeof(p)) != hipSuccess ||
        hipMemcpyToSymbol(HIP_SYMBOL(g_s1big_stamp_n), &n, sizeof(n)) != hipSuccess) {
        oodgan::set_error("debug_set_stamp_buffer: hipMemcpyToSymbol failed");
        return OODGAN_E_LAUNCH;
    }
    return 0;
}
#endif
```

ood-gan-inversion_amd/csrc/runtime.hip:

```cpp
#include "common.hpp"
#include <atomic>
#include <cstdlib>
#include <cstring>
#include <new>

namespace oodgan {
static thread_local char g_err[512] = "";
void set_error(const char* fmt, ...) {
    va_list ap;
    va_start(ap, fmt);
    vsnprintf(g_err, sizeof(g_err), fmt, ap);
    va_end(ap);
}
}

namespace oodgan {
namespace {
struct Tunable { const char* name; const char* env; long def; std::atomic<long> val; std::atomic<int> init; };
Tunable g_tun[OODGAN_TUN_COUNT] = {
    {"s1_big_min_items", "OODGAN_S1_BIG_MIN_ITEMS", 128, {0}, {0}},
    {"s2_big_min_items", "OODGAN_S2_BIG_MIN_ITEMS", 128, {0}, {0}},
    {"t2_big_min_items", "OODGAN_T2_BIG_MIN_ITEMS", 128, {0}, {0}},
    {"blurt_strip", "OODGAN_BLURT_STRIP", 1, {0}, {0}},
    {"blur_strip", "OODGAN_BLUR_STRIP", 1, {0}, {0}},
    {"upvb_waves", "OODGAN_UPVB_WAVES", 12, {0}, {0}},
    {"fewout_quad", "OODGAN_FEWOUT_QUAD", 1, {0}, {0}},
    {"tiny_mid_max", "OODGAN_TINY_MID_MAX", 1024, {0}, {0}},
    {"stripx_waves", "OODGAN_STRIPX_WAVES", 4, {0}, {0}},
};
}
long tunable(int id) {
    Tunable& t = g_tun[id];
    if (!t.init.load(std::memory_order_acquire)) {
        const char* e = getenv(t.env);
        t.val.store(e ? atol(e) : t.def, std::memory_order_relaxed);
        t.init.store(1, std::memory_order_release);
    }
    return t.val.load(std::memory_order_relaxed);
}
}

extern "C" int oodgan_set_tunable(const char* name, long value) {
    OODGAN_REQUIRE(name != nullptr, "set_tunable: null name");
    for (int i = 0; i < oodgan::OODGAN_TUN_COUNT; ++i)
        if (strcmp(name, oodgan::g_tun[i].name) == 0) {
            oodgan::g_tun[i].val.store(value, std::memory_order_relaxed);
            oodgan::g_tun[i].init.store(1, std::memory_order_release);
            return OODGAN_OK;
        }
    oodgan::set_error("set_tunable: unknown tunable '%s'", name);
    return OODGAN_E_ARG;
}
extern "C" long oodgan_get_tunable(const char* name) {
    if (name)
        for (int i = 0; i < oodgan::OODGAN_TUN_COUNT; ++i)
            if (strcmp(name, oodgan::g_tun[i].name) == 0) return oodgan::tunable(i);
    return -1;
}

namespace oodgan {
bool bound_device_ok(const char* what) {
    static std::atomic<int> bound{-1};
    int dev = 0;
    if (hipGetDevice(&dev) != hipSuccess) {
        (void)hipGetLastError();
        set_error("%s: no current HIP device", what);
        return false;
    }
    int expected = -1;
    if (bound.compare_exchange_strong(expected, dev, std::memory_order_acq_rel) || expected == dev) return true;
    set_error("%s: liboodgan_hip.so is bound to HIP device %d (its first use in this process) but device %d is current — one process per GPU "
              "(select the device with HIP_VISIBLE_DEVICES or torch.cuda.set_device before the first call)", what, expected, dev);
    return false;
}
}

namespace oodgan {
namespace {
const char* const g_dc_name[OODGAN_DC_COUNT] = {"stripx", "strip", "s1big", "s1v2", "s1pp", "tiny", "t2big", "t2v2", "t2gen", "s2big", "s2v2", "s2gen", "upvb", "s1big_ys", "s2big_fuse", "s2big_dotx_sform", "s1big_g2", "s2big_g2", "stripx_g2", "s2big_xh", "s1big_xh", "composite_mse"};
std::atomic<long> g_dc[OODGAN_DC_COUNT];
}
void count_dispatch(int id) { g_dc[id].fetch_add(1, std::memory_order_relaxed); }
}
extern "C" long oodgan_dispatch_count(const char* name) {
    if (name)
        for (int i = 0; i < oodgan::OODGAN_DC_COUNT; ++i)
            if (strcmp(name, oodgan::g_dc_name[i]) == 0) return oodgan::g_dc[i].load(std::memory_order_relaxed);
    return -1;
}
extern "C" int oodgan_dispatch_reset(void) {
    for (int i = 0; i < oodgan::OODGAN_DC_COUNT; ++i) oodgan::g_dc[i].store(0, std::memory_order_relaxed);
    return OODGAN_OK;
}

namespace {
__global__ __launch_bounds__(256) void zero_kernel(unsigned char* __restrict__ p, long bytes) {
    const long i = (long)blockIdx.x * 256 + threadIdx.x;
    const long head = (16 - (reinterpret_cast<uintptr_t>(p) & 15)) & 15;
    const long h = head < bytes ? head : bytes;
    const long n16 = (bytes - h) >> 4;
    if (i < n16) reinterpret_cast<uint4*>(p + h)[i] = make_uint4(0u, 0u, 0u, 0u);
    if (i < h) p[i] = 0;
    const long tail = h + (n16 << 4);
    if (i < bytes - tail) p[tail + i] = 0;
}
}

extern "C" int oodgan_zero(void* p, long bytes, void* stream) {
    OODGAN_REQUIRE(p != nullptr && bytes >= 0, "zero: bad args");
    if (bytes == 0) return OODGAN_OK;
    const long items = (bytes >> 4) + 16;
    OODGAN_REQUIRE((items + 255) / 256 < (1L << 31), "zero: too large");
    hipLaunchKernelGGL(zero_kernel, dim3((unsigned)((items + 255) / 256)), dim3(256), 0, oodgan::as_stream(stream),
                       reinterpret_cast<unsigned char*>(p), bytes);
    return oodgan::check_launch("zero");
}

#include <vector>
namespace oodgan {
struct PlanRec {
    std::vector<std::function<void()>> ops;
    bool recording = false;
};
thread_local PlanRec* tl_plan_rec = nullptr;
int g_null_launch = 0;
void plan_append(std::function<void()>&& f) { tl_plan_rec->ops.emplace_back(std::move(f)); }
}

extern "C" void* oodgan_plan_create(void) { return new (std::nothrow) oodgan::PlanRec(); }
extern "C" int oodgan_plan_destroy(void* plan) {
    oodgan::PlanRec* p = static_cast<oodgan::PlanRec*>(plan);
    if (p && oodgan::tl_plan_rec == p) oodgan::tl_plan_rec = nullptr;
    delete p;
    return OODGAN_OK;
}
extern "C" int oodgan_plan_record_begin(void* plan) {
    oodgan::PlanRec* p = static_cast<oodgan::PlanRec*>(plan);
    OODGAN_REQUIRE(p != nullptr, "plan_record_begin: null plan");
    OODGAN_REQUIRE(oodgan::tl_plan_rec == nullptr, "plan_record_begin: this thread is already recording a plan");
    p->ops.clear();
    p->recording = true;
    oodgan::tl_plan_rec = p;
    return OODGAN_OK;
}
extern "C" long oodgan_plan_record_end(void* plan) {
    oodgan::PlanRec* p = static_cast<oodgan::PlanRec*>(plan);
    if (p == nullptr || oodgan::tl_plan_rec != p) {
        oodgan::set_error("plan_record_end: this thread is not recording that plan");
        return -1;
    }
    oodgan::tl_plan_rec = nullptr;
    p->recording = false;
    return (long)p->ops.size();
}
extern "C" long oodgan_plan_size(const void* plan) { return plan ? (long)static_cast<const oodgan::PlanRec*>(plan)->ops.size() : -1; }
extern "C" int oodgan_plan_run(void* plan, int times) {
    oodgan::PlanRec* p = static_cast<oodgan::PlanRec*>(plan);
    OODGAN_REQUIRE(p != nullptr && !p->recording && times >= 0, "plan_run: null plan, a plan still recording, or times < 0");
    OODGAN_REQUIRE(oodgan::tl_plan_rec == nullptr, "plan_run: this thread is recording a plan");
    for (int t = 0; t < times; ++t)
        for (const std::function<void()>& f : p->ops) f();
    return oodgan::check_launch("plan_run");
}
extern "C" int oodgan_plan_set_null_launch(int on) {
    oodgan::g_null_launch = on ? 1 : 0;
    return OODGAN_OK;
}

extern "C" int oodgan_version(void) { return 110; }
extern "C" const char* oodgan_last_error(void) { return oodgan::g_err; }
extern "C" int oodgan_device_count(void) {
    int n = 0;
    if (hipGetDeviceCount(&n) != hipSuccess) {
        (void)hipGetLastError();
        return 0;
    }
    return n;
}
```

ood-gan-inversion_amd/oodgan/_lib.py:

```python
import ctypes
import os
from ctypes import POINTER, Structure, c_char_p, c_float, c_int, c_long, c_void_p

_HERE = os.path.dirname(os.path.abspath(__file__))
LIB_PATH = os.environ.get('OODGAN_LIB') or os.path.join(_HERE, 'liboodgan_hip.so')

CONV_S1, CONV_T2, CONV_S2 = 0, 1, 2
ACT_NONE, ACT_LRELU, ACT_PRELU = 0, 1, 2

P = c_void_p


ABI_VERSION = 110


class ConvArgs(Structure):
    _fields_ = [
        ('x', P), ('wpk', P), ('in_scale', P), ('in_shift', P), ('out_scale', P), ('bias', P), ('noise', P),
        ('noise_w', P), ('slope', P), ('dotx', P), ('dot_part', P), ('y', P),
        ('B', c_int), ('K', c_int), ('M', c_int), ('Hin', c_int), ('Win', c_int),
        ('in_pitch', c_int), ('out_pitch', c_int), ('in_scale_stride', c_int), ('out_scale_stride', c_int),
        ('noise_batch', c_int), ('mode', c_int), ('act', c_int), ('dot_nparts', c_int), ('in_mul2', P),
        ('x_sform', c_int), ('ys', P), ('ys_scale', P), ('ys_scale_stride', c_int),
        ('rgb_w', P), ('rgb_s', P), ('rgb_y', P), ('rgb_s_stride', c_int), ('rgb_scale', c_float), ('fuse', P), ('dot_actgrad', c_int), ('groups', c_int), ('y_fform', c_int), ('x_fform', c_int), ('dotx_fform', c_int), ('dotx_sform', c_int), ('dotx_scale', P), ('dotx_scale_stride', c_int), ('workspace', P), ('workspace_bytes', c_long), ('ys_vmax', P), ('x_hi_only', c_int),
    ]


class ActBwdFuse(Structure):
    _fields_ = [('g_rgb', P), ('w_rgb', P), ('s_rgb', P), ('noise', P), ('noise_w', P), ('bias', P), ('dscale', P), ('mul2', P), ('ys', P),
                ('part_r', P), ('part_t', P), ('part_max', P), ('s_rgb_stride', c_int), ('noise_batch', c_int), ('dscale_stride', c_int),
                ('rgb_scale', c_float), ('nmax', c_long), ('ys_hi_only', c_int)]


class ReduceJob(Structure):
    _fields_ = [('part', P), ('out', P), ('B', c_int), ('C', c_int), ('nparts', c_int), ('out_stride', c_int), ('accumulate', c_int),
                ('part2', P), ('scale2', P), ('nparts2', c_int), ('scale2_stride', c_int)]


class DemodBwdJob(Structure):
    _fields_ = [('s', P), ('wsq', P), ('d', P), ('r', P), ('gs', P), ('s_stride', c_int), ('d_stride', c_int), ('gs_stride', c_int),
                ('B', c_int), ('Ci', c_int), ('Co', c_int), ('scale', c_float)]


class DemodFwdJob(Structure):
    _fields_ = [('s', P), ('wsq', P), ('d', P), ('s_stride', c_int), ('d_stride', c_int), ('B', c_int), ('Ci', c_int), ('Co', c_int),
                ('scale', c_float)]


class ScaleCheckJob(Structure):
    _fields_ = [('part', P), ('n', c_long), ('state', P)]


_SIGS = {
    'oodgan_version': (c_int, []),
    'oodgan_last_error': (c_char_p, []),
    'oodgan_device_count': (c_int, []),
    'oodgan_set_tunable': (c_int, [c_char_p, c_long]),
    'oodgan_get_tunable': (c_long, [c_char_p]),
    'oodgan_dispatch_count': (c_long, [c_char_p]),
    'oodgan_dispatch_reset': (c_int, []),
    'oodgan_zero': (c_int, [P, c_long, P]),
    'oodgan_bias_act_fwd': (c_int, [P, P, P, P, P, c_int, c_int, c_long, c_int, c_float, c_float, P]),
    'oodgan_bias_act_bwd': (c_int, [P, P, P, P, c_int, c_int, c_long, c_float, c_float, P]),
    'oodgan_upfirdn2d': (c_int, [P, P, P] + [c_int] * 15 + [P]),
    'oodgan_blur_bias_act': (c_int, [P, P, P] + [c_int] * 9 + [P, P, c_int, P, c_int, P]),
    'oodgan_style_affine_fwd': (c_int, [P, P, P, P, P, c_int, c_int, c_int, c_int, c_float, c_float, P]),
    'oodgan_style_affine_bwd': (c_int, [P, P, P, P, c_int, c_int, c_int, c_int, c_float, P]),
    'oodgan_equal_linear': (c_int, [P, P, P, P, c_int, c_int, c_int, c_float, c_float, c_int, P]),
    'oodgan_equal_linear_grouped': (c_int, [P, P, P, P, c_int, c_int, c_int, c_int, c_float, c_float, c_int, P]),
    'oodgan_pixel_norm': (c_int, [P, P, c_int, c_int, P]),
    'oodgan_weight_sqsum': (c_int, [P, P, c_int, c_int, c_int, P]),
    'oodgan_demod_fwd': (c_int, [P, c_int, P, P, c_int, c_int, c_int, c_int, c_float, P]),
    'oodgan_demod_bwd': (c_int, [P, c_int, P, P, c_int, P, P, c_int, c_int, c_int, c_int, c_float, P]),
    'oodgan_pack_conv3x3': (c_int, [P, P, c_int, c_int, c_float, c_int, c_int, P]),
    'oodgan_conv3x3': (c_int, [POINTER(ConvArgs), P]),
    'oodgan_conv3x3_nparts': (c_int, [c_int, c_int, c_int]),
    'oodgan_pack_conv3x3_f16s_bytes': (c_long, [c_int, c_int, c_int]),
    'oodgan_pack_conv3x3_f16s': (c_int, [P, P, P, c_int, c_int, c_float, c_int, c_int, P]),
    'oodgan_conv3x3_f16s': (c_int, [POINTER(ConvArgs), P, P]),
    'oodgan_conv3x3_f16s_nparts': (c_int, [c_int, c_int, c_int]),
    'oodgan_conv3x3_f16s_nparts2': (c_int, [c_int, c_int, c_int, c_int]),
    'oodgan_conv3x3_s2_fuse_supported': (c_int, [c_int, c_int, c_int, c_int, c_int]),
    'oodgan_conv3x3_s1_ys_supported': (c_int, [c_int, c_int, c_int, c_int, c_int]),
    'oodgan_conv3x3_s2_grouped_supported': (c_int, [c_int, c_int, c_int, c_int, c_int, c_int]),
    'oodgan_conv3x3_s1_actgrad_supported': (c_int, [c_int, c_int, c_int, c_int, c_int]),
    'oodgan_sform_bytes': (c_long, [c_int, c_int, c_int, c_int]),
    'oodgan_sform_phases_bytes': (c_long, [c_int, c_int, c_int, c_int]),
    'oodgan_blurT_to_sform_phases': (c_int, [P, P, P, c_int, P, P, c_int, c_int, c_int, c_int, P]),
    'oodgan_from_sform': (c_int, [P, P, c_int, P, c_int, c_int, c_int, c_int, P]),
    'oodgan_to_sform_phases': (c_int, [P, P, c_int, P, P, c_int, c_int, c_int, c_int, c_int, P]),
    'oodgan_to_sform_phases_padtl': (c_int, [P, P, c_int, P, P, c_int, c_int, c_int, c_int, c_int, P]),
    'oodgan_to_sform': (c_int, [P, P, c_int, P, c_int, P, P, c_int, c_int, c_int, c_int, c_int, P, P]),
    'oodgan_resize_bicubic_ac': (c_int, [P, P, P, c_int, c_int, c_int, c_int, c_int, P]),
    'oodgan_avgpool': (c_int, [P, P, c_int, c_int, c_int, c_int, c_int, P]),
    'oodgan_blur_act_sform': (c_int, [P, P, P, P, P, c_int, P, P, c_int, P, c_int, c_int, c_int, c_int, c_int, c_int, P, P]),
    'oodgan_blur_act_sform_sep': (c_int, [P, P, P, P, P, c_int, P, P, c_int, P, c_int, c_int, c_int, c_int, c_int, c_int, P, c_int, P]),
    'oodgan_blur_act_fform': (c_int, [P, P, P, P, c_int, P, P, c_int, P, c_int, c_int, c_int, c_int, c_int, c_int, P, c_int, P]),
    'oodgan_conv3x3_xf_supported': (c_int, [c_int, c_int, c_int, c_int, c_int]),
    'oodgan_upconv_vblur_supported': (c_int, [c_int, c_int, c_int, c_int, c_int]),
    'oodgan_upconv_vblur_fform': (c_int, [P, P, c_long, P, P, P, c_int, P, P, c_int, P, c_int, P, c_int, P, P, c_int, c_int, c_int, c_int, c_int, P]),
    'oodgan_conv3x3_xf_nparts': (c_int, [c_int, c_int, c_int]),
    'oodgan_conv3x3_tiny_workspace': (c_long, [c_int, c_int, c_int, c_int, c_int, c_int]),

    'oodgan_absmax_scaled': (c_int, [P, P, c_int, P, c_int, c_int, c_long, P]),
    'oodgan_fwd_range_update': (c_int, [P, P, P, c_int, P]),
    'oodgan_fwd_range_plan': (c_int, [P, P, P, P, P, P, P, c_int, c_int, c_int, c_int, c_int, c_int, c_int, P]),
    'oodgan_act_bwd_sform_nparts': (c_int, [c_int, c_int]),
    'oodgan_act_bwd_sform': (c_int, [P, P, P, c_int, P, P, P, P, P, c_int, c_float, P, c_int, P, P, P, P, P, c_int, c_int, c_int, c_int, P]),
    'oodgan_act_bwd_sform_f': (c_int, [P, P, c_int, P, P, P, P, P, c_int, c_float, P, c_int, P, P, P, P, P, c_int, c_int, c_int, c_int, P]),
    'oodgan_from_fform': (c_int, [P, P, c_int, c_int, c_int, c_int, P]),
    'oodgan_act_bwd_blurT_nparts': (c_int, [c_int, c_int]),
    'oodgan_act_bwd_blurT_pre_supported': (c_int, [c_int, c_int]),
    'oodgan_act_bwd_blurT_sform_phases': (c_int, [P, P, P, c_int, P, P, P, P, P, c_int, c_float, P, c_int, P, P, P, P, P, P, c_int, c_int, c_int, c_int, P]),
    'oodgan_act_bwd_blurT_hi_supported': (c_int, [c_int, c_int]),
    'oodgan_conv3x3_s1_xh_supported': (c_int, [c_int, c_int, c_int, c_int, c_int]),
    'oodgan_act_bwd_blurT_sform_phases_hi': (c_int, [P, P, P, c_int, P, P, P, c_int, P, P, P, P, P, c_int, c_int, c_int, c_int, P]),
    'oodgan_absmax_scale_check': (c_int, [P, c_long, P, P, P]),
    'oodgan_reduce_batch': (c_int, [P, c_int, P]),
    'oodgan_demod_bwd_batch': (c_int, [P, c_int, P]),
    'oodgan_demod_fwd_batch': (c_int, [P, c_int, P]),
    'oodgan_absmax_scale_check_batch': (c_int, [P, c_int, P, P]),
    'oodgan_hform_bytes': (c_long, [c_int, c_int, c_int, c_int]),
    'oodgan_to_hform': (c_int, [P, P, c_int, c_int, c_int, c_int, P]),
    'oodgan_from_hform': (c_int, [P, P, c_int, c_int, c_int, c_int, P]),
    'oodgan_modconv_f16_wbytes': (c_long, [c_int, c_int, c_int]),
    'oodgan_modconv_f16_pack': (c_int, [P, P, c_int, c_float, c_int, c_int, P, c_int, c_int, c_int, P]),
    'oodgan_modconv_f16_pack_affine': (c_int, [P, P, c_int, P, P, c_int, c_float, c_int, c_int, P, c_int, c_int, c_int, P]),
    'oodgan_modconv_f16': (c_int, [P, P, P, c_int, P, P, c_int, P, c_int, c_int, c_int, c_int, c_int, P]),
    'oodgan_reduce_parts': (c_int, [P, P, c_long, c_int, c_int, P]),
    'oodgan_reduce_parts_cols': (c_int, [P, P, c_int, c_int, c_int, c_int, c_int, P]),
    'oodgan_torgb_fwd': (c_int, [P, P, P, c_int, P, P, P, P, c_int, c_int, c_int, c_int, c_float, P]),
    'oodgan_rgb_finish': (c_int, [P, P, P, P, P, c_int, c_int, c_int, P]),
    'oodgan_rgb_finish_parts': (c_int, [P, c_int, P, P, P, P, c_int, c_int, c_int, P]),
    'oodgan_torgb_fwd_sform': (c_int, [P, P, P, c_int, P, P, P, P, P, P, c_int, c_int, c_int, c_int, c_int, c_float, P, P]),
    'oodgan_act_bwd_fused': (c_int, [P, P, P, c_int, P, P, P, P, P, c_int, c_float, P, P, P, c_int, c_int, c_long, P]),
    'oodgan_act_bwd_nparts': (c_int, [c_long]),
    'oodgan_feature_modulation': (c_int, [P, P, P, P, c_long, c_int, P]),
    'oodgan_act_bwd_fused_max': (c_int, [P, P, P, c_int, P, P, P, P, P, c_int, c_float, P, P, P, P, P, c_int, c_int, c_int, c_long, P]),
    'oodgan_absmax_scale': (c_int, [P, c_long, P, P]),
    'oodgan_absmax_scale_clear': (c_int, [P, c_long, P, P]),
    'oodgan_mse_fwd_bwd': (c_int, [P, P, P, P, P, c_int, c_long, c_float, P]),
    'oodgan_mse_fwd_bwd_row': (c_int, [P, P, P, P, P, P, c_int, c_int, c_long, c_float, P]),
    'oodgan_conv2d_s1': (c_int, [P, P, P, P, P, P, c_int, c_int, c_int, c_int, c_int, c_int, c_int, c_int, P]),
    'oodgan_add_mask': (c_int, [P, P, P, c_long, P]),
    'oodgan_maxpool3s2_fwd': (c_int, [P, P, P, c_long, c_int, c_int, P]),
    'oodgan_maxpool3s2_bwd': (c_int, [P, P, P, P, P, c_long, c_int, c_int, P]),
    'oodgan_lpips_prep': (c_int, [P, P, c_int, c_int, c_int, c_float, c_float, POINTER(c_float), POINTER(c_float), P]),
    'oodgan_lpips_img_grad': (c_int, [P, P, c_int, c_int, c_int, c_float, c_float, POINTER(c_float), P]),
    'oodgan_lpips_head': (c_int, [P, P, P, P, P, c_int, c_int, c_long, c_float, c_int, P]),
    'oodgan_lpips_head_nparts': (c_int, [c_long]),
    'oodgan_lpips_finish': (c_int, [POINTER(P), POINTER(c_int), POINTER(c_long), c_int, P, P, c_int, c_int, P]),
    'oodgan_plan_create': (P, []),
    'oodgan_plan_destroy': (c_int, [P]),
    'oodgan_plan_record_begin': (c_int, [P]),
    'oodgan_plan_record_end': (c_long, [P]),
    'oodgan_plan_size': (c_long, [P]),
    'oodgan_plan_run': (c_int, [P, c_int]),
    'oodgan_plan_set_null_launch': (c_int, [c_int]),
    'oodgan_mse_nparts': (c_int, [c_long]),
    'oodgan_composite_mse_fwd_bwd': (c_int, [P, P, P, P, P, P, P, c_int, c_int, c_long, c_int, c_float, P]),
    'oodgan_composite_mse_fwd_bwd_row': (c_int, [P, P, P, P, P, P, P, P, c_int, c_int, c_int, c_long, c_int, c_float, P]),
    'oodgan_scale_by_plane': (c_int, [P, P, c_int, c_int, c_long, P]),
    'oodgan_loss_weight_from_alpha': (c_int, [P, P, c_long, c_int, P]),
    'oodgan_adam_step': (c_int, [P, P, P, P, c_long, c_float, c_float, c_float, c_float, c_int, P]),
    'oodgan_adam_step_dev': (c_int, [P, P, P, P, c_long, c_float, c_float, c_float, c_float, P, P]),
}

_lib = None


def lib():
    global _lib
    if _lib is None:
        if not os.path.exists(LIB_PATH):
            raise RuntimeError(
                f'{LIB_PATH} not found: build it with `python __graft_entry__.py` (hipcc --offload-arch=gfx950); '
                'there is no CPU or PyTorch fallback for the hot path')
        h = ctypes.CDLL(LIB_PATH)
        for name, (res, args) in _SIGS.items():
# ... 47 lines not shown
```

ood-gan-inversion_amd/oodgan/engine.py:

```python
import math
import re

import os

import torch

from . import ops
from ._lib import ACT_LRELU, ACT_NONE, CONV_S1, CONV_S2, CONV_T2
from .synth import generator_channels, make_kernel


_Cols = ops.Cols


class _Layer:
    __slots__ = ('name', 'kind', 'cin', 'cout', 'res', 'lat', 'row', 'drow', 'wpk', 'wpk_bwd', 'wsq', 'w_rgb',
                 'bias', 'noise_w', 'scale', 'noise_idx', 'src', 'sidx', 'wpk_vb')


def _pad_channels_to_16(state, prefix, log_size, ch):
    up16 = lambda c: (c + 15) // 16 * 16
    chp = {r: up16(c) for r, c in ch.items()}
    out = dict(state)

# ... 47 lines not shown
        self.n_latent = self.log_size * 2 - 2
        self.num_layers = (self.log_size - 2) * 2 + 1
        ch = generator_channels(channel_multiplier, narrow)
        used = [ch[2 ** i] for i in range(2, self.log_size + 1)]
        if any(c < 1 for c in used):
            raise ValueError(f'channel counts {used} (narrow={narrow}, channel_multiplier={channel_multiplier})')
        self.padded = any(c % 16 for c in used)
        self.real_channels = dict(ch)
        if self.padded:
            state, _ = _pad_channels_to_16(state, prefix, self.log_size, ch)
        g = lambda k: state[prefix + k].detach().float().contiguous()
        dev = g('input.input').device
        if dev.type != 'cuda':
            raise RuntimeError('GeneratorEngine needs its parameters on a ROCm device (no CPU fallback)')
        self.device = dev
        self.const_input = g('input.input')
        def family(pattern, taps, what):
            pat = re.compile('^' + re.escape(prefix) + pattern + r'\.kernel$')
            held = [v.detach().float().cpu() for k, v in state.items() if pat.match(k)]
            k4 = held[0] if held else make_kernel(tuple(taps)) * 4.0
            if tuple(k4.shape) != (4, 4):
                raise NotImplementedError(f'{what} kernel of shape {tuple(k4.shape)}: the fused producers are built for four taps (every shipped config: [1,3,3,1])')
            if any(h.shape != k4.shape or not torch.equal(h, k4) for h in held):
                raise NotImplementedError(f'the {what} kernels of the state differ between layers')
            return k4.contiguous()

        k4 = family(r'convs\.\d+\.conv\.blur', blur_kernel, 'Blur')
        self.k4x4 = k4.to(dev)
        self.k4x4_flip = torch.flip(self.k4x4, [0, 1]).contiguous()
        self.k4x4_rank1 = bool(torch.linalg.matrix_rank(k4.double()) == 1)
        self.k_up = family(r'to_rgbs\.\d+\.upsample', upsample_kernel, 'Upsample').to(dev)
        self.k_up_flip = torch.flip(self.k_up, [0, 1]).contiguous()
        layers = []

        up16 = lambda c: (c + 15) // 16 * 16

        def styled(name, cin, cout, res, lat, up, nidx):
            L = _Layer()
            L.name, L.kind, L.cin, L.cout, L.res, L.lat, L.noise_idx = name, ('up' if up else 'conv'), up16(cin), up16(cout), res, lat, nidx
            w = g(f'{name}.conv.weight')[0]
            L.scale = 1.0 / math.sqrt(cin * 9)
            L.wpk = ops.pack_conv3x3(w, L.scale, transpose=False, flip=False, precision=self.precision)
            L.wpk_bwd = ops.pack_conv3x3(w, L.scale, transpose=True, flip=not up, precision=self.precision) if with_backward else None
            if L.wpk_bwd is not None:
                L.wpk_bwd.x_hi_only = self.grad_hi_only
            L.wsq = ops.weight_sqsum(w)
            L.wpk_vb = None
            L.bias = g(f'{name}.activate.bias')
            L.noise_w = g(f'{name}.noise.weight')
            layers.append(L)
            return L

        def rgb(name, cin, res, lat):
            L = _Layer()
            L.name, L.kind, L.cin, L.cout, L.res, L.lat = name, 'rgb', up16(cin), 3, res, lat
            L.w_rgb = g(f'{name}.conv.weight').reshape(3, up16(cin)).contiguous()
            L.bias = g(f'{name}.bias').reshape(3).contiguous()
            L.scale = 1.0 / math.sqrt(up16(cin))
            layers.append(L)
            return L

        styled('conv1', ch[4], ch[4], 4, 0, False, 0)
        rgb('to_rgb1', ch[4], 4, 1)
        cin, i = ch[4], 1
        for j in range(self.log_size - 2):
            res = 2 ** (j + 3)
            cout = ch[res]
            styled(f'convs.{2 * j}', cin, cout, res, i, True, 2 * j + 1)
            styled(f'convs.{2 * j + 1}', cout, cout, res, i + 1, False, 2 * j + 2)
            rgb(f'to_rgbs.{j}', cout, res, i + 2)
            cin, i = cout, i + 2
        self.layers = layers
        self.fused_bwd = True
        self.bwd_state, self.bwd_flag = {}, None
        styled = [L for L in layers if L.kind != 'rgb']
        self.layers_styled_last = styled[-1]
        self.fused_fwd = True
        self.next_conv = {a.name: b for a, b in zip(styled[:-1], styled[1:]) if a.kind == 'up' and b.kind == 'conv'}
        self.rgb_next_up = {a.name: b for a, b in zip(layers[:-1], layers[1:]) if a.kind == 'rgb' and b.kind == 'up'}
        self.conv_next_rgb = {a.name: b for a, b in zip(layers[:-1], layers[1:]) if a.kind == 'conv' and b.kind == 'rgb'}
        self.by_name = {L.name: L for L in layers}
        self.fuse_act_bwd = True
        self.hi_records = os.environ.get('OODGAN_HI_RECORDS', '1') != '0'
        self.fused_rgb = True
        self.fuse_x = True
        self.fuse_up = True
        self.save_sform_only = os.environ.get('OODGAN_SAVE_SFORM_ONLY', '1') != '0'
        self.fuse_conv_rgb_64 = True
        self.sform_only_max_res = None
        self.fuse_conv_rgb = os.environ.get('OODGAN_FUSE_CONV_RGB', '1') != '0'
        self.plain_one_pass = os.environ.get('OODGAN_PLAIN_ONE_PASS', '1') != '0'
        Lup = next((a for a, b in zip(styled[:-1], styled[1:]) if a.kind == 'up' and b is styled[-1]), None)
        if (Lup is not None and self.precision == 'f16s' and self.sform and with_backward and Lup.cout % 32 == 0 and Lup.cin % 16 == 0
                and Lup.cout <= 32 and size >= 64):
            Lup.wpk_vb = ops.pack_upconv_vblur(g(f'{Lup.name}.conv.weight')[0], Lup.scale, self.k4x4)
        ops.xf_supported(1, 32, 32, 8, 32)
        self.batched_tail = True
        src = 'input'
        for L in layers:
            L.src = src
            if L.kind != 'rgb':
                src = L.name
        rows, drows, wl, bl, rl = 0, 0, [], [], []
        lat_start = [0] * (self.n_latent + 1)
        row_layer, drow_layer, sidx = [], [], 0
        for L in layers:
            L.row = rows
            wl.append(g(f'{L.name}.conv.modulation.weight'))
            bl.append(g(f'{L.name}.conv.modulation.bias'))
            rl += [L.lat] * L.cin
            rows += L.cin
            lat_start[L.lat + 1] = rows
            if L.kind != 'rgb':
                L.drow = drows
                drows += L.cout
                L.sidx = sidx
                row_layer += [sidx] * L.cin
                drow_layer += [sidx] * L.cout
                sidx += 1
            else:
                L.sidx = -1
                row_layer += [-1] * L.cin
        for l in range(1, self.n_latent + 1):
            lat_start[l] = max(lat_start[l], lat_start[l - 1])
        self.R, self.DR = rows, drows
        self.wcat = torch.cat(wl, 0).contiguous()
        self.bcat = torch.cat(bl, 0).contiguous()
        self.row_lat = torch.tensor(rl, dtype=torch.int32, device=dev)
        self.lat_start = torch.tensor(lat_start, dtype=torch.int32, device=dev)
        self.row_layer = torch.tensor(row_layer, dtype=torch.int32, device=dev)
        self.drow_layer = torch.tensor(drow_layer, dtype=torch.int32, device=dev)
        self.n_styled = sidx
        self.fwd_range = None
        self.carry_range = True
        self.stored_noises = [g(f'noises.noise_{k}') for k in range(self.num_layers)] if (prefix + 'noises.noise_0') in state else None
        self.saved = None

    def clone_shared(self):
        import copy
        e = copy.copy(self)
        e.saved = None
        e.bwd_state, e.bwd_flag = {}, None
        e.fwd_range = None
        e._ranges = {}
        return e

    def reset_fwd_state(self, B=None):
        ranges = self.__dict__.get('_ranges', {})
        todo = list(ranges.values()) if B is None else [r for r in (ranges.get(B),) if r is not None]
        if self.fwd_range is not None and (B is None or self.fwd_range.B == B) and not any(r is self.fwd_range for r in todo):
            todo.append(self.fwd_range)
        for r in todo:
            r.valid = False
            r.flag.zero_()
            r.vm.zero_()

    def fwd_range_violated(self):
        return self.fwd_range is not None and self.fwd_range.violated()

    def _range(self, B):
        if self.fwd_range is None or self.fwd_range.B != B:
            ranges = self.__dict__.setdefault('_ranges', {})
            r = ranges.get(B)
            if r is None:
                r = ranges[B] = ops.FwdRange(self.n_styled, B, self.R, self.DR, self.row_layer, self.drow_layer, self.device)
            self.fwd_range = r
# ... 246 lines not shown
            s = _Cols(s_all, L.row, L.cin)
            d = _Cols(d_all, L.drow, L.cout)
            Hd = x_in.shape[2]
            carry = carry_scale and self.fused_bwd and self.sform and (L.kind == 'conv' or Hd >= 4)
            st = self.bwd_state.get(L.name) if carry else None
            Rg, prev_rgb = prev_rgb, None
            rgb_kw = {} if Rg is None else dict(g_rgb=gskip[L.res], w_rgb=Rg.w_rgb, s_rgb=_Cols(s_all, Rg.row, Rg.cin))
            if st is not None and fused_in is not None:
                gin, rsum, tsum, part_m = fused_in.dst, fused_in.r, None, fused_in.part_m
                fused_in = None
                mul2, g_pre = st, None
            elif st is not None and xf_bwd:
                gin, rsum, tsum, part_m = None, None, None, None
                mul2, g_pre = st, None
            elif st is not None:
                t_into = None if Rg is None else _Cols(gs_all, Rg.row, Rg.cin)
                if L.kind == 'conv':
                    gin = ops.sform_scratch(B, L.cout, out.shape[2], out.shape[3], self.device)
                    rsum, tsum, part_m = ops.act_bwd_producer(out, g_feat, nz, L.noise_w, L.bias, d, st, gin, t_into=t_into, jobs=jobs, **rgb_kw)
                elif fused_pre is not None:
                    gin = ops.sform_phases_scratch(B, L.cout, Hd, Hd, self.device)
                    rsum, tsum, part_m = ops.act_bwd_producer(None, g_feat, nz, L.noise_w, L.bias, d, st, gin, blur_kernel=self.k4x4_flip,
                                                              jobs=jobs, dot_of=fused_pre, hi_only=self._hi_records(B, L, Hd, Rg))
                    fused_pre = None
                else:
                    gin = ops.sform_phases_scratch(B, L.cout, Hd, Hd, self.device)
                    rsum, tsum, part_m = ops.act_bwd_producer(out, g_feat, nz, L.noise_w, L.bias, d, st, gin,
                                                              blur_kernel=self.k4x4_flip, t_into=t_into, jobs=jobs,
                                                              hi_only=self._hi_records(B, L, Hd, Rg), **rgb_kw)
                mul2, g_pre = st, None
            else:
                if Rg is not None:
                    g_pre, rsum, tsum, mul2 = ops.act_bwd_fused(out, g_feat, nz, L.noise_w, L.bias, gskip[L.res], Rg.w_rgb,
                                                                _Cols(s_all, Rg.row, Rg.cin), want_scale=True, dscale=d)
                else:
                    g_pre, rsum, tsum, mul2 = ops.act_bwd_fused(out, g_feat, nz, L.noise_w, L.bias, want_scale=True, dscale=d)
                if carry:
                    self.bwd_state[L.name] = mul2
                    if self.bwd_flag is None:
                        self.bwd_flag = torch.zeros(1, dtype=torch.int32, device=self.device)
            if Rg is not None and tsum is not None:
                gs_all[:, Rg.row:Rg.row + Rg.cin] = tsum
            deferred = st is not None and jobs is not None
            xa = None
            if st is not None and xf_bwd:
                xa = ops.ActBwdX(nz, L.noise_w, L.bias, d, st, gskip[L.res], Rg.w_rgb, _Cols(s_all, Rg.row, Rg.cin),
                                 t_into=_Cols(gs_all, Rg.row, Rg.cin))
                pre = None
                Lp = self.by_name.get(L.src)
                if (Lp is not None and Lp.kind == 'up' and self.fuse_act_bwd and self.bwd_state.get(L.src) is not None
                        and ops.s1_actgrad_supported(B, L.cout, L.cin, out.shape[2], out.shape[3])):
                    pre = ops.DotActGrad()
                dx, dot = ops.conv3x3(out, L.wpk_bwd, L.cin, CONV_S1, out_scale=s, dotx=x_in, in_mul2=mul2,
                                      dot_into=_Cols(gs_all, L.row, L.cin), jobs=jobs, dot_actgrad=pre, xf_act=xa)
                rsum, part_m = xa.r, xa.part_m
                fused_in, fused_pre = None, pre
            if deferred:
                jobs.add_demod(_Cols(s_all, L.row, L.cin), L.wsq, _Cols(d_all, L.drow, L.cout), rsum, _Cols(gs_all, L.row, L.cin), B, L.cin,
                               L.cout, L.scale)
            else:
                check(lib().oodgan_demod_bwd(ctypes.c_void_p(s_all.data_ptr() + 4 * L.row), self.R, ctypes.c_void_p(L.wsq.data_ptr()),
                                             ctypes.c_void_p(d_all.data_ptr() + 4 * L.drow), self.DR, ctypes.c_void_p(rsum.data_ptr()),
                                             ctypes.c_void_p(gs_all.data_ptr() + 4 * L.row), self.R, B, L.cin, L.cout, L.scale,
                                             ops._stream()), 'demod_bwd')
            if xa is not None:
                if deferred:
                    jobs.add_check(part_m, st)
                else:
                    ops.absmax_scale_check(part_m, st, self.bwd_flag)
            elif st is not None:
                fz = None
                Lp = self.by_name.get(L.src)
                stp = self.bwd_state.get(L.src) if (L.kind == 'up' and Lp is not None and self.fuse_act_bwd) else None
                if stp is not None and ops.s2_fuse_supported(B, L.cout, L.cin, 2 * Hd + 1, 2 * Hd + 1):
                    Rp = self.conv_next_rgb[Lp.name]
                    hi = bool(self.grad_hi_only and self.hi_records and ops.s1_xh_supported(B, Lp.cout, Lp.cin, Hd, Hd))
                    fz = ops.ActBwdFusion((ops.sform_hi_scratch if hi else ops.sform_scratch)(B, Lp.cout, Hd, Hd, self.device), noises[Lp.noise_idx],
                                          Lp.noise_w, Lp.bias, _Cols(d_all, Lp.drow, Lp.cout), stp, g_rgb=gskip[Lp.res], w_rgb=Rp.w_rgb,
                                          s_rgb=_Cols(s_all, Rp.row, Rp.cin), t_into=_Cols(gs_all, Rp.row, Rp.cin), hi_only=hi)
                pre = None
                if (L.kind == 'conv' and Lp is not None and Lp.kind == 'up' and self.fuse_act_bwd and self.bwd_state.get(L.src) is not None
                        and ops.s1_actgrad_supported(B, L.cout, L.cin, out.shape[2], out.shape[3])):
                    pre = ops.DotActGrad()
                dx, dot = ops.conv3x3(gin, L.wpk_bwd, L.cin, CONV_S1 if L.kind == 'conv' else CONV_S2, out_scale=s, dotx=x_in,
                                      in_mul2=mul2, dot_into=_Cols(gs_all, L.row, L.cin), jobs=jobs, fuse=fz, want_y=fz is None,
                                      dot_actgrad=pre)
                fused_in, fused_pre = fz, pre
                del gin
                if deferred:
                    jobs.add_check(part_m, st)
                else:
                    ops.absmax_scale_check(part_m, st, self.bwd_flag)
            elif L.kind == 'conv':
                if self.sform:
                    gs_ = ops.to_sform(g_pre, d, mul2, out=ops.sform_scratch(B, L.cout, g_pre.shape[2], g_pre.shape[3], self.device))
                    dx, dot = ops.conv3x3(gs_, L.wpk_bwd, L.cin, CONV_S1, out_scale=s, dotx=x_in, in_mul2=mul2)
                    del gs_
                else:
                    dx, dot = ops.conv3x3(g_pre, L.wpk_bwd, L.cin, CONV_S1, in_scale=d, out_scale=s, dotx=x_in, in_mul2=mul2)
            else:
                if self.sform and Hd >= 4:
                    gp = ops.blurT_to_sform_phases(g_pre, self.k4x4_flip, d, mul2,
                                                   out=ops.sform_phases_scratch(B, L.cout, Hd, Hd, self.device))
                    dx, dot = ops.conv3x3(gp, L.wpk_bwd, L.cin, CONV_S2, out_scale=s, dotx=x_in, in_mul2=mul2)
                else:
                    H2 = 2 * Hd + 1
                    P2 = (H2 + 3) // 4 * 4
                    g2 = ops.upfirdn2d(g_pre, self.k4x4_flip, pad=(2, 2), out_pitch=P2)
                    dx, dot = ops.conv3x3(g2, L.wpk_bwd, L.cin, CONV_S2, in_scale=d, out_scale=s, dotx=x_in, in_hw=(H2, H2),
                                          in_pitch=P2, in_mul2=mul2)
                    del g2
            if dot is not None:
                gs_all[:, L.row:L.row + L.cin] += dot
            g_feat = dx
            del g_pre
        if jobs is not None:
            jobs.run(self.bwd_flag)
        self.last_gs = gs_all
        return ops.style_affine_backward(gs_all, self.wcat, self.lat_start, self.n_latent, grad_div=grad_scale)


_SIDE = {}


def _side_streams(device, n):
    pool = _SIDE.setdefault(str(device), [])
    while len(pool) < n:
        pool.append(torch.cuda.Stream(device=device))
    return pool[:n]


MULTI_STREAM_S1_BIG_MIN_ITEMS = int(os.environ.get('OODGAN_MULTI_STREAM_S1_BIG_MIN_ITEMS', '64'))
_S1_BIG_DEFAULT = 128

_FLAG = {}
_PLAN_POOLS = {}


def _plan_pool(device, batch):
    if os.environ.get('OODGAN_PLAN_POOL_CACHE', '1') == '0':
        return torch.cuda.MemPool()
    key = (str(device), ops._stream_handle(), int(batch))
    pool = _PLAN_POOLS.get(key)
    if pool is None:
        pool = _PLAN_POOLS[key] = torch.cuda.MemPool()
    return pool


def _flag_stream(device):
    st = _FLAG.get(str(device))
    if st is None:
        st = _FLAG[str(device)] = torch.cuda.Stream(device=device)
    return st


class _WRun:

    def __init__(self, inv, eng, target, w0, noises, steps, stream, dev_counter, keep_traj, beta=None):
        self.inv, self.eng, self.stream, self.steps = inv, eng, stream, steps
        self.target, self.noises = target, noises
        self.beta = beta
        self.w = w0.detach().clone().contiguous()
        self.m, self.v = torch.zeros_like(self.w), torch.zeros_like(self.w)
        self.gmul = ops.loss_scale_for(target.numel() // target.shape[0])
        self.t = 0
        self.dev_t = torch.zeros(1, dtype=torch.int32, device=self.w.device) if dev_counter else None
        self.lbuf = torch.empty(steps, self.w.shape[0], device=self.w.device, dtype=torch.float32)
        self.lp = inv.lpips if (inv.lpips is not None and inv.lpips_weight != 0.0) else None
        self.lp_target = self.lp.target_taps(target) if self.lp is not None else None
# ... 335 lines not shown
```

ood-gan-inversion_amd/oodgan/ops.py:

```python
import ctypes
import os
import math

import torch

from . import _lib
from ._lib import ACT_LRELU, ACT_NONE, ACT_PRELU, CONV_S1, CONV_S2, CONV_T2, ConvArgs, check

SQRT2 = 2 ** 0.5


def _p(t):
    return None if t is None else ctypes.c_void_p(t.data_ptr())


_RAW_STREAM = getattr(torch._C, '_cuda_getCurrentRawStream', None)
_DEV_INDEX = None


def _stream_handle():
    global _DEV_INDEX
    if _RAW_STREAM is None:
        return torch.cuda.current_stream().cuda_stream
    if _DEV_INDEX is None:
# ... 186 lines not shown
    check(_lib.lib().oodgan_equal_linear(_p(x), _p(w), _p(_opt(bias, 'bias')), _p(y), B, I, O, 1.0, 1.0, 0, _stream()), 'linear')
    return y


def pixel_norm(x):
    x = _dev(x)
    y = torch.empty_like(x)
    check(_lib.lib().oodgan_pixel_norm(_p(x), _p(y), x.shape[0], x.shape[1], _stream()), 'pixel_norm')
    return y


def weight_sqsum(weight):
    w = _dev(weight, 'weight')
    Co, Ci = w.shape[0], w.shape[1]
    out = torch.empty(Co, Ci, device=w.device, dtype=torch.float32)
    check(_lib.lib().oodgan_weight_sqsum(_p(w), _p(out), Co, Ci, w.shape[2] * w.shape[3], _stream()), 'weight_sqsum')
    return out


def demod(s, wsq, scale):
    s = _dev(s, 's')
    B, Ci = s.shape
    Co = wsq.shape[0]
    d = torch.empty(B, Co, device=s.device, dtype=torch.float32)
    check(_lib.lib().oodgan_demod_fwd(_p(s), Ci, _p(wsq), _p(d), Co, B, Ci, Co, float(scale), _stream()), 'demod_fwd')
    return d


class SForm:
    __slots__ = ('data', 'B', 'C', 'H', 'W', 'hi_only')

    def __init__(self, B, C, H, W, device):
        n = _lib.lib().oodgan_sform_bytes(B, C, H, W)
        self.data = torch.zeros(n // 2, device=device, dtype=torch.float16)
        self.B, self.C, self.H, self.W = B, C, H, W
        self.hi_only = False

    def data_ptr(self):
        return self.data.data_ptr()

    @property
    def shape(self):
        return (self.B, self.C, self.H, self.W)


class FForm:
    __slots__ = ('data', 'B', 'C', 'H', 'W')

    def __init__(self, data):
        self.data = data
        self.B, self.C, self.H, self.W = data.shape

    def data_ptr(self):
        return self.data.data_ptr()

    @property
    def shape(self):
        return (self.B, self.C, self.H, self.W)

    def to_nchw(self):
        y = torch.empty(self.B, self.C, self.H, self.W, device=self.data.device, dtype=torch.float32)
        check(_lib.lib().oodgan_from_fform(_p(self.data), _p(y), self.B, self.C, self.H, self.W, _stream()), 'from_fform')
        return y


class SFormSaved:
    __slots__ = ('sform', 'scale')

    def __init__(self, sform, scale):
        self.sform, self.scale = sform, scale

    @property
    def shape(self):
        return self.sform.shape

    def to_nchw(self):
        B, C, H, W = self.sform.shape
        y = torch.empty(B, C, H, W, device=self.sform.data.device, dtype=torch.float32)
        sc = self.scale
        check(_lib.lib().oodgan_from_sform(_p(self.sform), _p(sc), 0 if sc is None else sc.shape[1], _p(y), B, C, H, W, _stream()), 'from_sform')
        return y


class SFormPhases:
    __slots__ = ('data', 'B', 'C', 'H', 'W', 'hi_only')

    def __init__(self, B, C, H, W, device):
        n = _lib.lib().oodgan_sform_phases_bytes(B, C, H, W)
        self.data = torch.zeros(n // 2, device=device, dtype=torch.float16)
        self.B, self.C, self.H, self.W = B, C, H, W
        self.hi_only = False

    def data_ptr(self):
        return self.data.data_ptr()

    @property
    def shape(self):
        return (self.B, self.C, 2 * self.H + 1, 2 * self.W + 1)


def to_sform_phases(x, H, W, scale=None, mul2=None, out=None, in_pitch=0, pad_tl=False):
    x = _dev(x)
    B, C = x.shape[0], x.shape[1]
    if out is None:
        out = SFormPhases(B, C, H, W, x.device)
    out.hi_only = False
    fn = _lib.lib().oodgan_to_sform_phases_padtl if pad_tl else _lib.lib().oodgan_to_sform_phases
    check(fn(_p(x), _p(_opt(scale, 'scale')), 0 if scale is None else scale.shape[1], _p(mul2), _p(out), B, C, H, W, in_pitch, _stream()),
          'to_sform_phases')
    return out


def blurT_to_sform_phases(g, kernel, scale=None, mul2=None, out=None):
    g = _dev(g)
    B, C = g.shape[0], g.shape[1]
    H, W = g.shape[2] // 2, g.shape[3] // 2
    if out is None:
        out = SFormPhases(B, C, H, W, g.device)
    out.hi_only = False
    check(_lib.lib().oodgan_blurT_to_sform_phases(_p(g), _p(_dev(kernel)), _p(_opt(scale, 'scale')),
                                                  0 if scale is None else scale.shape[1], _p(mul2), _p(out), B, C, H, W,
                                                  _stream()), 'blurT_to_sform_phases')
    return out


_SFORM_POOL = {}


def sform_phases_scratch(B, C, H, W, device):
    key = ('ph', B, C, H, W, str(device), _stream_handle())
    buf = _SFORM_POOL.get(key)
    if buf is None:
        buf = _SFORM_POOL[key] = SFormPhases(B, C, H, W, device)
    return buf


_WS_POOL = {}
USE_TINY = True


def conv_workspace(nbytes, device):
    key = (nbytes, str(device), _stream_handle())
    buf = _WS_POOL.get(key)
    if buf is None:
        buf = _WS_POOL[key] = torch.empty(nbytes // 4, device=device, dtype=torch.int32)
    return buf


def drop_stream_scratch(stream_handle):
    for pool in (_SFORM_POOL, _WS_POOL):
        for key in [k for k in pool if k[-1] == stream_handle]:
            del pool[key]
    for key in [k for k in _VMAX_POOL if k[1] == stream_handle]:
        del _VMAX_POOL[key]


def sform_scratch(B, C, H, W, device, tag=0):
    key = (B, C, H, W, str(device), tag, _stream_handle())
    buf = _SFORM_POOL.get(key)
    if buf is None:
        buf = _SFORM_POOL[key] = SForm(B, C, H, W, device)
    return buf


def to_sform(x, scale=None, mul2=None, out=None, in_hw=None, in_pitch=0, vmax=None, shift=None):
    x = _dev(x)
# ... 80 lines not shown
        x = _dev(x)
        B, C = x.shape[0], x.shape[1]
        check(_lib.lib().oodgan_absmax_scaled(_p(x), _p(s), s.shape[1], _p(self.vm[l]), B, C, x.numel() // (B * C), _stream()),
              'absmax_scaled')
        check(_lib.lib().oodgan_fwd_range_update(_p(self.vm[l]), _p(self.q[l]), None, B, _stream()), 'fwd_range_update')

    def update_exact(self, l):
        check(_lib.lib().oodgan_fwd_range_update(_p(self.vm[l]), _p(self.q[l]), None, self.B, _stream()), 'fwd_range_update')

    def finish(self):
        check(_lib.lib().oodgan_fwd_range_update(_p(self.vm), _p(self.q), _p(self.flag), self.L * self.B, _stream()), 'fwd_range_update')

    def violated(self):
        return int(self.flag.item()) != 0


class BwdJobs:

    def __init__(self):
        self.reduce, self.reduce_acc, self.demod, self.check, self.keep = [], [], [], [], []

    def add_reduce(self, part, out_ptr_obj, B, C, nparts, out_stride, accumulate, second=None):
        (self.reduce_acc if accumulate else self.reduce).append(_reduce_job(part, out_ptr_obj, B, C, nparts, out_stride, accumulate, second))
        self.keep += [part, out_ptr_obj, second]

    def add_demod(self, s, wsq, d, r, gs, B, Ci, Co, scale):
        self.demod.append(_lib.DemodBwdJob(_p(s), _p(wsq), _p(d), _p(r), _p(gs), s.shape[1], d.shape[1], gs.shape[1], B, Ci, Co,
                                           float(scale)))
        self.keep += [s, wsq, d, r, gs]

    def add_check(self, part, state):
        self.check.append(_lib.ScaleCheckJob(_p(part), part.numel(), _p(state)))
        self.keep += [part, state]

    def run(self, flag):
        L = _lib.lib()
        if self.reduce:
            arr = (_lib.ReduceJob * len(self.reduce))(*self.reduce)
            check(L.oodgan_reduce_batch(arr, len(self.reduce), _stream()), 'reduce_batch')
        if self.demod:
            arr = (_lib.DemodBwdJob * len(self.demod))(*self.demod)
            check(L.oodgan_demod_bwd_batch(arr, len(self.demod), _stream()), 'demod_bwd_batch')
        if self.reduce_acc:
            arr = (_lib.ReduceJob * len(self.reduce_acc))(*self.reduce_acc)
            check(L.oodgan_reduce_batch(arr, len(self.reduce_acc), _stream()), 'reduce_batch')
        if self.check:
            arr = (_lib.ScaleCheckJob * len(self.check))(*self.check)
            check(L.oodgan_absmax_scale_check_batch(arr, len(self.check), _p(flag), _stream()), 'absmax_scale_check_batch')
        self.reduce, self.reduce_acc, self.demod, self.check, self.keep = [], [], [], [], []


def _reduce_job(part, out, B, C, nparts, out_stride, accumulate, second=None):
    j = _lib.ReduceJob(_p(part), _p(out), B, C, nparts, out_stride, 1 if accumulate else 0)
    if second is not None:
        part2, scale2 = second
        j.part2, j.scale2, j.nparts2, j.scale2_stride = _p(part2), _p(scale2), part2.shape[2], scale2.shape[1]
    return j


def _reduce_into(part, B, C, npart, into, accumulate):
    check(_lib.lib().oodgan_reduce_parts_cols(_p(part), _p(into), B, C, npart, into.shape[1], 1 if accumulate else 0, _stream()),
          'reduce_parts_cols')


def _reduce_parts(part, rows, npart):
    out = torch.empty(part.shape[0], part.shape[1], device=part.device, dtype=torch.float32)
    check(_lib.lib().oodgan_reduce_parts(_p(part), _p(out), rows, npart, 0, _stream()), 'reduce')
    return out


def blurT_hi_supported(H, W):
    return bool(_lib.lib().oodgan_act_bwd_blurT_hi_supported(H, W))


def act_bwd_producer(out, g_feat, noise, noise_weight, bias, dscale, mul2, dst, g_rgb=None, w_rgb=None, s_rgb=None,
                     blur_kernel=None, t_into=None, jobs=None, dot_of=None, hi_only=False):
    pre = out is None
    assert not pre or (dot_of is not None and dot_of.dot_part is not None)
    fform = isinstance(out, FForm)
    if fform:
        assert g_feat is None and blur_kernel is None, 'F-form: the last styled conv only (no conv gradient, no blur)'
        o = out.data
    else:
        o = _dev(g_feat, 'g_feat') if pre else _dev(out, 'out')
    B, C, H, W = o.shape
    L = _lib.lib()
    up = blur_kernel is not None
    npart = L.oodgan_act_bwd_blurT_nparts(H // 2, W // 2) if up else L.oodgan_act_bwd_sform_nparts(H, W)
    KC = (C + 15) // 16
    part_r = torch.empty(B, C, npart, device=o.device, dtype=torch.float32)
    part_t = torch.empty(B, C, npart, device=o.device, dtype=torch.float32) if g_rgb is not None else None
    part_m = torch.empty(B * KC * npart, device=o.device, dtype=torch.float32)
    nz = _opt(noise, 'noise')
    common = [_p(_opt(g_feat, 'g_feat')), _p(None if pre else o), _p(nz), 1 if nz is None else nz.shape[0], _p(_opt(noise_weight, 'nw')),
              _p(_opt(bias, 'bias')), _p(_opt(g_rgb, 'g_rgb')), _p(None if w_rgb is None else _dev(w_rgb).reshape(3, C)),
              _p(_opt(s_rgb, 's_rgb')), 0 if s_rgb is None else s_rgb.shape[1], 1.0 / math.sqrt(C), _p(_dev(dscale, 'dscale')),
              dscale.shape[1], _p(mul2)]
    if fform:
        check(L.oodgan_act_bwd_sform_f(*common[1:], _p(dst), _p(part_r), _p(part_t), _p(part_m), B, C, H, W, _stream()), 'act_bwd_sform_f')
    elif up and hi_only:
        assert g_rgb is None and part_t is None
        check(L.oodgan_act_bwd_blurT_sform_phases_hi(*common[:6], *common[11:], _p(_dev(blur_kernel)), _p(dst), _p(part_r), _p(part_m),
                                                     B, C, H // 2, W // 2, _stream()), 'act_bwd_blurT_sform_phases_hi')
        dst.hi_only = True
    elif up:
        check(L.oodgan_act_bwd_blurT_sform_phases(*common, _p(_dev(blur_kernel)), _p(dst), _p(part_r), _p(part_t), _p(part_m),
                                                  B, C, H // 2, W // 2, _stream()), 'act_bwd_blurT_sform_phases')
        dst.hi_only = False
    else:
        check(L.oodgan_act_bwd_sform(*common, _p(dst), _p(part_r), _p(part_t), _p(part_m), B, C, H, W, _stream()),
              'act_bwd_sform')
    second = (dot_of.dot_part, dot_of.scale) if pre else None
    if jobs is not None:
        r = torch.empty(B, C, device=o.device, dtype=torch.float32)
        jobs.add_reduce(part_r, r, B, C, npart, C, False, second)
        if part_t is not None:
            jobs.add_reduce(part_t, t_into, B, C, npart, t_into.shape[1], False)
        return r, None, part_m
    if pre:
        r = torch.empty(B, C, device=o.device, dtype=torch.float32)
        job = _reduce_job(part_r, r, B, C, npart, C, False, second)
        check(L.oodgan_reduce_batch(ctypes.byref(job), 1, _stream()), 'reduce_batch')
    else:
        r = _reduce_parts(part_r, B * C, npart)
    t = None
    if part_t is not None:
        if t_into is not None:
            _reduce_into(part_t, B, C, npart, t_into, False)
        else:
            t = _reduce_parts(part_t, B * C, npart)
    return r, t, part_m


def absmax_scale_check(part_max, state, flag):
    check(_lib.lib().oodgan_absmax_scale_check(_p(part_max), part_max.numel(), _p(state), _p(flag), _stream()), 'absmax_scale_check')


class HForm:
    __slots__ = ('buf', 'B', 'C', 'H', 'W')

    def __init__(self, B, C, H, W, device):
        self.B, self.C, self.H, self.W = B, C, H, W
        self.buf = torch.zeros(_lib.lib().oodgan_hform_bytes(B, C, H, W) // 2, dtype=torch.float16, device=device)

    def data_ptr(self):
        return self.buf.data_ptr()

    def to_nchw(self):
        y = torch.empty(self.B, self.C, self.H, self.W, device=self.buf.device, dtype=torch.float32)
        check(_lib.lib().oodgan_from_hform(_p(self), _p(y), self.B, self.C, self.H, self.W, _stream()), 'from_hform')
        return y


def to_hform(x, out=None):
    x = _dev(x)
    B, C, H, W = x.shape
    if out is None:
        out = HForm(B, C, H, W, x.device)
    check(_lib.lib().oodgan_to_hform(_p(x), _p(out), B, C, H, W, _stream()), 'to_hform')
    return out


def modconv_f16_pack(weight, style, demodulate=True, act='none', out=None, latent=None, mod_weight=None, mod_bias=None):
    weight = _dev(weight).reshape(weight.shape[-4:])
    M, K = weight.shape[0], weight.shape[1]
    B = (style if style is not None else latent).shape[0]
    wpk = out if out is not None else torch.empty(_lib.lib().oodgan_modconv_f16_wbytes(B, M, K) // 2, dtype=torch.float16, device=weight.device)
    if style is not None:
        style = _dev(style)
        check(_lib.lib().oodgan_modconv_f16_pack(_p(weight), _p(style), style.stride(0), 1.0 / math.sqrt(K * 9), int(demodulate),
                                                 _F16_ACT[act], _p(wpk), B, M, K, _stream()), 'modconv_f16_pack')
    else:
        latent, mod_weight = _dev(latent, 'latent'), _dev(mod_weight, 'mod_weight')
        check(_lib.lib().oodgan_modconv_f16_pack_affine(_p(weight), _p(latent), latent.stride(0), _p(mod_weight), _p(_opt(mod_bias, 'mod_bias')),
                                                        latent.shape[1], 1.0 / math.sqrt(K * 9), int(demodulate), _F16_ACT[act], _p(wpk), B, M, K,
                                                        _stream()), 'modconv_f16_pack_affine')
    return wpk, M, K, act


_F16_ACT = {'none': ACT_NONE, 'lrelu': ACT_LRELU}


# ... 33 lines not shown
        precision = 'f16s'
    w = _dev(weight, 'weight')
    Co, Ci = w.shape[0], w.shape[1]
    M, K = (Ci, Co) if transpose else (Co, Ci)
    if precision == 'f32':
        Mp = (M + 63) // 64 * 64
        out = torch.empty(K, 9, Mp, device=w.device, dtype=torch.float32)
        check(_lib.lib().oodgan_pack_conv3x3(_p(w), _p(out), Co, Ci, float(scale), int(transpose), int(flip), _stream()), 'pack')
        return PackedConv(out, None, 'f32', M)
    nbytes = _lib.lib().oodgan_pack_conv3x3_f16s_bytes(Co, Ci, int(transpose))
    out = torch.empty(nbytes // 2, device=w.device, dtype=torch.float16)
    unscale = torch.empty(2, device=w.device, dtype=torch.float32)
    check(_lib.lib().oodgan_pack_conv3x3_f16s(_p(w), _p(out), _p(unscale), Co, Ci, float(scale), int(transpose), int(flip),
                                              _stream()), 'pack_f16s')
    return PackedConv(out, unscale, 'f16s', M)


class PackedUpVB:
    __slots__ = ('data', 'unscale4', 'kh', 'wset_bytes', 'M', 'K')

    def __init__(self, data, unscale4, kh, wset_bytes, M, K):
        self.data, self.unscale4, self.kh, self.wset_bytes, self.M, self.K = data, unscale4, kh, wset_bytes, M, K


def rank_one_factors(k2d):
    kf = torch.flip(k2d.detach().double().cpu(), [0, 1])
    if kf.shape != (4, 4) or not torch.isfinite(kf).all() or float(kf.abs().max()) == 0.0:
        return None
    i, j = divmod(int(kf.abs().argmax()), 4)
    kv, kh = kf[:, j] / kf[i, j], kf[i, :].clone()
    if float((torch.outer(kv, kh) - kf).abs().max()) > 1e-12 * float(kf.abs().max()):
        return None
    return kv, kh


def pack_upconv_vblur(weight, scale, k2d):
    f = rank_one_factors(k2d)
    if f is None:
        return None
    kv, kh = f
    w = _dev(weight, 'weight')
    Co, Ci = w.shape[0], w.shape[1]
    wv = torch.zeros(2, Co, Ci, 3, 3, device=w.device, dtype=torch.float64)
    for py in range(2):
        for a in range(4):
            for ky in range(3):
                t = py + a - 1 - ky
                if t % 2 == 0 and -1 <= t // 2 <= 1:
                    wv[py, :, :, t // 2 + 1, :] += float(kv[a]) * w[:, :, ky, :].double()
    wv = wv.float().contiguous()
    L = _lib.lib()
    nbytes = L.oodgan_pack_conv3x3_f16s_bytes(Co, Ci, 0)
    data = torch.empty(nbytes, device=w.device, dtype=torch.float16)
    unscale4 = torch.empty(4, device=w.device, dtype=torch.float32)
    for py in range(2):
        check(L.oodgan_pack_conv3x3_f16s(_p(wv[py]), ctypes.c_void_p(data.data_ptr() + py * nbytes),
                                         ctypes.c_void_p(unscale4.data_ptr() + 8 * py), Co, Ci, float(scale), 0, 0, _stream()), 'pack_f16s')
    return PackedUpVB(data, unscale4, kh.float().to(w.device).contiguous(), nbytes, Co, Ci)


def upconv_vblur_supported(B, K, M, H, W):
    return bool(_lib.lib().oodgan_upconv_vblur_supported(B, K, M, H, W))


def upconv_vblur_fform(xs, wvb, out_scale=None, bias=None, noise=None, noise_weight=None, act=True, ys_scale=None, vmax=None):
    assert isinstance(xs, SForm) and isinstance(wvb, PackedUpVB)
    B, K, H, W = xs.shape
    assert K == wvb.K
    M = wvb.M
    y = torch.empty(B, M, 2 * H, 2 * W, device=xs.data.device, dtype=torch.float32)
    nz = _opt(noise, 'noise')
    check(_lib.lib().oodgan_upconv_vblur_fform(_p(xs), _p(wvb.data), wvb.wset_bytes, _p(wvb.unscale4), _p(wvb.kh),
                                               _p(_opt(out_scale, 'out_scale')), 0 if out_scale is None else out_scale.shape[1],
                                               _p(_opt(bias, 'bias')), _p(nz), 1 if nz is None else nz.shape[0],
                                               _p(_opt(noise_weight, 'nw')), ACT_LRELU if act else ACT_NONE,
                                               _p(_opt(ys_scale, 'ys_scale')), 0 if ys_scale is None else ys_scale.shape[1], _p(vmax),
                                               _p(y), B, K, M, H, W, _stream()), 'upconv_vblur_fform')
    return FForm(y)


def conv3x3(x, wpk, M, mode=CONV_S1, in_scale=None, in_shift=None, out_scale=None, bias=None, noise=None,
            noise_weight=None, act=ACT_NONE, slope=None, dotx=None, in_hw=None, in_pitch=0, out=None, out_pitch=0,
            in_mul2=None, ys=None, ys_scale=None, want_y=True, dot_into=None, rgb=None, jobs=None, fuse=None, dot_actgrad=None,
            groups=1, y_fform=False, xf_act=None, tiny_max=8, vmax=None):
    sform_in = isinstance(x, (SForm, SFormPhases))
    fform_in = isinstance(x, FForm)
    if fform_in:
        assert mode == CONV_S1 and wpk.precision == 'f16s'
        y_fform = xf_act is None
    elif not sform_in:
        x = _dev(x)
    B, K = x.shape[0], x.shape[1] // max(1, groups)
    H, W = in_hw if in_hw is not None else (x.shape[2], x.shape[3])
    if mode == CONV_S1:
        oh, ow = H, W
    elif mode == CONV_T2:
        oh, ow = 2 * H + 1, 2 * W + 1
        if out_pitch == 0:
            out_pitch = (ow + 3) // 4 * 4
    else:
        oh, ow = (H - 1) // 2, (W - 1) // 2
    pitch = out_pitch if out_pitch else ow
    if out is None and want_y:
        out = torch.empty(B, M, oh, pitch, device=x.data.device if (sform_in or fform_in) else x.device, dtype=torch.float32)
    a = ConvArgs()
    a.x, a.wpk, a.y = _p(x), _p(wpk), _p(out)
    a.in_scale, a.in_shift, a.out_scale = _p(_opt(in_scale, 'in_scale')), _p(_opt(in_shift, 'in_shift')), _p(_opt(out_scale, 'out_scale'))
    a.bias, a.noise, a.noise_w, a.slope = _p(_opt(bias, 'bias')), _p(_opt(noise, 'noise')), _p(_opt(noise_weight, 'nw')), _p(_opt(slope, 'slope'))
    a.B, a.K, a.M, a.Hin, a.Win = B, K, M, H, W
    a.in_pitch, a.out_pitch = in_pitch, out_pitch
    a.in_scale_stride = in_scale.shape[1] if in_scale is not None else 0
    a.out_scale_stride = out_scale.shape[1] if out_scale is not None else 0
    a.noise_batch = noise.shape[0] if noise is not None else 1
    a.mode, a.act = mode, act
    a.in_mul2 = _p(in_mul2)
    a.x_sform = 1 if sform_in else 0
    a.x_fform = (2 if xf_act is not None else 1) if fform_in else 0
    ws = None
    if sform_in and USE_TINY and wpk.precision == 'f16s' and mode in (CONV_S1, CONV_S2) and min(oh, ow) <= tiny_max:
        nb = _lib.lib().oodgan_conv3x3_tiny_workspace(mode, B, K, M, H, W)
        if nb > 0:
            ws = conv_workspace(nb, x.data.device)
            a.workspace, a.workspace_bytes = _p(ws), nb
    a.groups = int(groups)
    a.x_hi_only = 1 if (wpk.x_hi_only and dotx is not None) else 0
    if isinstance(x, (SForm, SFormPhases)) and x.hi_only:
        assert a.x_hi_only == 1, 'hi-only input records need the two-instruction input-gradient conv (precision f16s-g2, dotx)'
        a.x_hi_only = 2
    a.y_fform = 1 if y_fform else 0
    a.ys, a.ys_scale = _p(ys), _p(_opt(ys_scale, 'ys_scale'))
    a.ys_vmax = _p(vmax)
    rgb_y = None
    if rgb is not None:
        w_rgb, s_rgb = rgb
        nrgb = 1 if M <= 32 else (M + 63) // 64
        rgb_y = torch.empty(*((B, 3, oh, ow) if nrgb == 1 else (nrgb, B, 3, oh, ow)), device=x.data.device if sform_in or fform_in else x.device,
                            dtype=torch.float32)
        a.rgb_w, a.rgb_s, a.rgb_y = _p(_dev(w_rgb, 'w_rgb').reshape(3, M)), _p(_dev(s_rgb, 's_rgb')), _p(rgb_y)
        a.rgb_s_stride, a.rgb_scale = s_rgb.shape[1], 1.0 / math.sqrt(M)
    a.ys_scale_stride = ys_scale.shape[1] if ys_scale is not None else 0
    fz = None
    if fuse is not None:
        fz = fuse.struct(B, M, oh, ow)
        a.fuse = ctypes.cast(ctypes.pointer(fz), ctypes.c_void_p)
    if xf_act is not None:
        fz = xf_act.struct(B, K, H, W)
        a.fuse = ctypes.cast(ctypes.pointer(fz), ctypes.c_void_p)
    part = None
    if dotx is not None:
        dot_f = isinstance(dotx, FForm)
        dot_s = isinstance(dotx, SFormSaved)
        if dot_s and fuse is None:
            dotx, dot_s = dotx.to_nchw(), False
        dx_ = dotx.data if dot_f else (dotx.sform.data if dot_s else _dev(dotx, 'dotx'))
        a.dotx_fform = 1 if dot_f else 0
        if dot_s:
            a.dotx_sform, a.dotx_scale, a.dotx_scale_stride = 1, _p(dotx.scale), dotx.scale.shape[1]
        if fform_in:
            npart = _lib.lib().oodgan_conv3x3_xf_nparts(B, H, W)
        elif wpk.precision == 'f16s':
            npart = _lib.lib().oodgan_conv3x3_f16s_nparts2(mode, H, W, 1 if sform_in else 0)
        else:
            npart = _lib.lib().oodgan_conv3x3_nparts(mode, H, W)
        part = torch.empty(B, M, npart, device=dx_.device, dtype=torch.float32)
        a.dotx, a.dot_part, a.dot_nparts = _p(dx_), _p(part), npart
        if dot_actgrad is not None:
            a.dot_actgrad = 1
            dot_actgrad.dot_part, dot_actgrad.scale = part, out_scale
    if wpk.precision == 'f16s':
        check(_lib.lib().oodgan_conv3x3_f16s(ctypes.byref(a), _p(wpk.unscale), _stream()), 'conv3x3_f16s')
    else:
        check(_lib.lib().oodgan_conv3x3(ctypes.byref(a), _stream()), 'conv3x3')
    if fuse is not None:
        fuse.finish(part, a.dot_nparts, jobs)
    if xf_act is not None:
        xf_act.finish(jobs)
    if dotx is not None:
        if dot_into is not None:
            if jobs is not None:
                jobs.add_reduce(part, dot_into, B, M, a.dot_nparts, dot_into.shape[1], True)
            else:
                _reduce_into(part, B, M, a.dot_nparts, dot_into, True)
            return out, None
        dot = torch.empty(B, M, device=dx_.device, dtype=torch.float32)
        check(_lib.lib().oodgan_reduce_parts(_p(part), _p(dot), B * M, a.dot_nparts, 0, _stream()), 'reduce_parts')
        return out, dot
    if y_fform:
        out = FForm(out)
    if rgb is not None:
# ... 312 lines not shown
```

Measured before the change: 8.134.

## Store stride-1 input-gradient planes as scaled f16 and read them in blurT producer

The stride-1 backward conv with dot_actgrad can now write its dx*act' output as f16 planes, pre-scaled by the next layer's mul2 factor. The blur-transpose activation-backward producer gains an f16-input variant that reads these planes and undoes the scale. This halves the bytes written and read for these large intermediate gradient planes between the two kernels. The cost is extra rounding of the gradient to f16, which the consumer already does before its contraction, plus a risk of overflow if the scale is poorly chosen.

```diff
diff --git a/include/oodgan.h b/include/oodgan.h
--- a/include/oodgan.h
+++ b/include/oodgan.h
@@ -116,6 +116,8 @@
     long workspace_bytes;
     unsigned* ys_vmax;
     int x_hi_only;
+    int y_h16;
+    const float* y_mul2;
 } oodgan_conv_args;
 
 typedef struct oodgan_actbwd_fuse {
@@ -149,6 +151,7 @@
 int oodgan_conv3x3_s2_grouped_supported(int B, int K, int M, int groups, int Hin, int Win);
 int oodgan_conv3x3_s1_actgrad_supported(int B, int K, int M, int H, int W);
 int oodgan_conv3x3_s1_ys_supported(int B, int K, int M, int H, int W);
+int oodgan_conv3x3_s1_dx16_supported(int B, int K, int M, int H, int W);
 int oodgan_conv3x3_xf_supported(int B, int K, int M, int H, int W);
 int oodgan_conv3x3_xf_nparts(int B, int H, int W);
 long oodgan_conv3x3_tiny_workspace(int mode, int B, int K, int M, int Hin, int Win);
@@ -209,6 +212,10 @@
 int oodgan_act_bwd_blurT_sform_phases_hi(const float* g_feat, const float* out, const float* noise, int noise_batch, const float* noise_w,
                                          const float* bias, const float* dscale, int dscale_stride, const float* mul2, const float* kernel,
                                          void* out_phases, float* part_r, float* part_max, int B, int C, int H, int W, void* stream);
+int oodgan_act_bwd_blurT_in16_supported(int H, int W);
+int oodgan_act_bwd_blurT_sform_phases_hi16(const void* g_pre_h16, const float* noise, int noise_batch, const float* noise_w, const float* bias,
+                                           const float* dscale, int dscale_stride, const float* mul2, const float* kernel, void* out_phases,
+                                           float* part_r, float* part_max, int B, int C, int H, int W, void* stream);
 int oodgan_absmax_scale_check(const float* part, long n, float* state, int* flag, void* stream);
 
 typedef struct oodgan_reduce_job {
diff --git a/ood-gan-inversion_amd/csrc/bwd_producers.hip b/ood-gan-inversion_amd/csrc/bwd_producers.hip
--- a/ood-gan-inversion_amd/csrc/bwd_producers.hip
+++ b/ood-gan-inversion_amd/csrc/bwd_producers.hip
@@ -8,6 +8,7 @@
 
 typedef _Float16 half8 __attribute__((ext_vector_type(8)));
 typedef _Float16 half2v __attribute__((ext_vector_type(2)));
+typedef _Float16 half4v __attribute__((ext_vector_type(4)));
 
 namespace {
 
@@ -39,6 +40,7 @@
     int noise_batch, s_rgb_stride, dscale_stride;
     float rgb_scale;
     int B, C, H, W, nparts;
+    int g_h16;
 };
 
 
@@ -488,7 +490,7 @@
     int hi_only;
 };
 
-template <int QN, bool XTRA, bool PRE>
+template <int QN, bool XTRA, bool PRE, bool G16 = false>
 __global__ __launch_bounds__(16 * QN) __attribute__((amdgpu_waves_per_eu((PRE && !XTRA) ? 4 : 2, 4))) void act_bwd_blurT_strip_kernel(const ActArgs a, const float* __restrict__ kern, uint4* __restrict__ outp,
                                                                    int H, int W, SPDims sp, StripGeo geo) {
     constexpr int SW = 4 * QN, NT = 16 * QN, NWV = NT / 64;
@@ -552,13 +554,16 @@
     const bool vl = cok && q == 0 && X0 >= 2;
     const bool vr = cok && q == QN - 1 && X0 + SW < Wg;
 
-    struct Rows { float4 o[PRE ? 1 : 2], g[2], n[2]; float2 oe[PRE ? 1 : 2], ge[2]; };
+    static_assert(!G16 || PRE, "f16 gradient planes: the pre-activated form only");
+    typedef typename std::conditional<G16, half4v, float4>::type G4;
+    typedef typename std::conditional<G16, half2v, float2>::type G2;
+    struct Rows { float4 o[PRE ? 1 : 2], n[2]; G4 g[2]; float2 oe[PRE ? 1 : 2]; G2 ge[2]; };
     const int gxc = min(gxm, Wg - 4);
     const int ecol = q == QN - 1 ? min(X0 + SW, Wg - 2) : max(X0 - 2, 0);
     const long cbase_c = ((long)b * a.C + min(c, a.C - 1)) * HW;
     const float* gsrc = a.g_feat ? a.g_feat : a.out;
     const bool has_g = a.g_feat != nullptr;
-    const float* nsrc = np ? np : gsrc + cbase_c;
+    const float* nsrc = np ? np : (G16 ? a.part_r : gsrc + cbase_c);
     const bool has_n = np != nullptr && gxm + 3 < Wg;
     auto load_rows = [&](int i, Rows& R) __attribute__((always_inline)) {
 #pragma unroll
@@ -569,9 +574,16 @@
                 R.o[PRE ? 0 : rr] = *reinterpret_cast<const float4*>(a.out + p + gxc);
                 R.oe[PRE ? 0 : rr] = *reinterpret_cast<const float2*>(a.out + p + ecol);
             }
-            R.g[rr] = *reinterpret_cast<const float4*>(gsrc + p + gxc);
-            R.ge[rr] = *reinterpret_cast<const float2*>(gsrc + p + ecol);
-            R.n[rr] = *reinterpret_cast<const float4*>(nsrc + (long)rc * Wg + gxc);
+            if constexpr (G16) {
+                const _Float16* g16 = reinterpret_cast<const _Float16*>(gsrc);
+                R.g[rr] = *reinterpret_cast<const half4v*>(g16 + p + gxc);
+                R.ge[rr] = *reinterpret_cast<const half2v*>(g16 + p + ecol);
+                R.n[rr] = *reinterpret_cast<const float4*>(nsrc + (np ? (long)rc * Wg + gxc : 0));
+            } else {
+                R.g[rr] = *reinterpret_cast<const float4*>(gsrc + p + gxc);
+                R.ge[rr] = *reinterpret_cast<const float2*>(gsrc + p + ecol);
+                R.n[rr] = *reinterpret_cast<const float4*>(nsrc + (long)rc * Wg + gxc);
+            }
         }
     };
 
@@ -593,10 +605,10 @@
             const bool own = r >= 2 * i0 + 1 || (seg == 0 && r == 0);
             const bool mg = rok && vm && has_g, mn = rok && has_n;
             const bool me0 = rok && has_g && (vl || vr), me1 = rok && has_g && vl;
-            const float gv[4] = {mg ? R.g[rr].x : 0.f, mg ? R.g[rr].y : 0.f, mg ? R.g[rr].z : 0.f, mg ? R.g[rr].w : 0.f};
+            const float gv[4] = {mg ? (float)R.g[rr].x : 0.f, mg ? (float)R.g[rr].y : 0.f, mg ? (float)R.g[rr].z : 0.f, mg ? (float)R.g[rr].w : 0.f};
             float gp[4], e0, e1;
             const float nv[4] = {mn ? R.n[rr].x : 0.f, mn ? R.n[rr].y : 0.f, mn ? R.n[rr].z : 0.f, mn ? R.n[rr].w : 0.f};
-            const float ge0 = me0 ? R.ge[rr].x : 0.f, ge1 = me1 ? R.ge[rr].y : 0.f;
+            const float ge0 = me0 ? (float)R.ge[rr].x : 0.f, ge1 = me1 ? (float)R.ge[rr].y : 0.f;
             if (PRE) {
 #pragma unroll
                 for (int e = 0; e < 4; ++e) {
@@ -728,6 +740,8 @@
     __syncthreads();
     bv = cst[4][ch];
     sc_ = cst[5][ch];
+    const float un16 = G16 ? a.mul2[0] : 1.f;
+    if (G16) sc_ *= un16;
     int i = i0 - 2;
     auto walk = [&](auto r1_c) __attribute__((always_inline)) {
         for (; i + 1 < i1; i += 2) {
@@ -743,6 +757,7 @@
 
 #pragma unroll
     for (int o = QN / 2; o > 0; o >>= 1) acc_r += __shfl_xor(acc_r, o, 64);
+    if (G16) { acc_r *= un16; amax *= un16; }
     auto put = [&](float* tab, int row, int rows_used, float v) {
         const int r1 = row == rows_used - 1 ? geo.tiles_y : row + 1;
         const int c1 = strip == geo.nstrips - 1 ? geo.tiles_x : strip + 1;
@@ -808,6 +823,7 @@
     OODGAN_REQUIRE(!g_rgb || (w_rgb && s_rgb && part_t), "act_bwd producer: rgb branch needs w_rgb, s_rgb and part_t");
     OODGAN_REQUIRE(noise == nullptr || noise_batch == 1 || noise_batch == B, "act_bwd producer: noise_batch");
     OODGAN_REQUIRE((W % 4) == 0, "act_bwd producer: W must be a multiple of 4");
+    a.g_h16 = 0;
     a.g_feat = g_feat; a.out = out; a.noise = noise; a.noise_w = noise_w; a.bias = bias;
     a.g_rgb = g_rgb; a.w_rgb = w_rgb; a.s_rgb = s_rgb; a.dscale = dscale; a.mul2 = mul2;
     a.part_r = part_r; a.part_t = g_rgb ? part_t : nullptr; a.part_max = part_max;
@@ -893,6 +909,19 @@
     OODGAN_REQUIRE(oodgan_act_bwd_blurT_hi_supported(H, W), "act_bwd_blurT hi-only records: the strip walk only (H, W >= 32, tunable blurt_strip)");
     return act_bwd_blurT_impl(g_feat, out, noise, noise_batch, noise_w, bias, nullptr, nullptr, nullptr, 0, 0.f, dscale, dscale_stride, mul2, kernel,
                               out_phases, part_r, nullptr, part_max, B, C, H, W, stream, 1);
+}
+
+extern "C" int oodgan_act_bwd_blurT_in16_supported(int H, int W) {
+    return oodgan_act_bwd_blurT_hi_supported(H, W) && oodgan::tunable(oodgan::OODGAN_TUN_DX_H16) != 0 ? 1 : 0;
+}
+
+extern "C" int oodgan_act_bwd_blurT_sform_phases_hi16(const void* g_pre_h16, const float* noise, int noise_batch, const float* noise_w, const float* bias,
+                                                      const float* dscale, int dscale_stride, const float* mul2, const float* kernel, void* out_phases,
+                                                      float* part_r, float* part_max, int B, int C, int H, int W, void* stream) {
+    OODGAN_REQUIRE(oodgan_act_bwd_blurT_in16_supported(H, W), "act_bwd_blurT f16 input planes: the strip walk only (H, W >= 32, tunables blurt_strip, dx_h16)");
+    OODGAN_REQUIRE(g_pre_h16 != nullptr, "act_bwd_blurT f16 input planes: null g_pre");
+    return act_bwd_blurT_impl(reinterpret_cast<const float*>(g_pre_h16), nullptr, noise, noise_batch, noise_w, bias, nullptr, nullptr, nullptr, 0, 0.f, dscale,
+                              dscale_stride, mul2, kernel, out_phases, part_r, nullptr, part_max, B, C, H, W, stream, 2);
 }
 
 static int act_bwd_blurT_impl(const float* g_feat, const float* out, const float* noise, int noise_batch, const float* noise_w, const float* bias,
@@ -916,7 +945,8 @@
     if (!g_rgb && !part_t && H >= 32 && W >= 32 && blurT_strip_enabled()) {
         constexpr int QN = 16;
         StripGeo geo;
-        geo.hi_only = hi_only;
+        geo.hi_only = hi_only != 0;
+        a.g_h16 = hi_only == 2 ? 1 : 0;
         geo.extra = ((W % (2 * QN)) == 0 && W <= 32) ? 1 : 0;
         geo.nstrips = geo.extra ? W / (2 * QN) : (W + 1 + 2 * QN - 1) / (2 * QN);
         geo.tiles_x = tiles_x;
@@ -933,7 +963,15 @@
 #define OODGAN_STRIP_LAUNCH(X, P)                                                                                              \
     hipLaunchKernelGGL((act_bwd_blurT_strip_kernel<QN, X, P>), dim3((unsigned)nbs), dim3(256), 0, as_stream(stream), a, kernel, \
                        reinterpret_cast<uint4*>(out_phases), H, W, d, geo)
-        if (geo.extra) {
+        if (a.g_h16) {
+            oodgan::count_dispatch(oodgan::OODGAN_DC_BLURT_IN16);
+            if (geo.extra)
+                hipLaunchKernelGGL((act_bwd_blurT_strip_kernel<QN, true, true, true>), dim3((unsigned)nbs), dim3(256), 0, as_stream(stream), a, kernel,
+                                   reinterpret_cast<uint4*>(out_phases), H, W, d, geo);
+            else
+                hipLaunchKernelGGL((act_bwd_blurT_strip_kernel<QN, false, true, true>), dim3((unsigned)nbs), dim3(256), 0, as_stream(stream), a, kernel,
+                                   reinterpret_cast<uint4*>(out_phases), H, W, d, geo);
+        } else if (geo.extra) {
             if (out) OODGAN_STRIP_LAUNCH(true, false); else OODGAN_STRIP_LAUNCH(true, true);
         } else {
             if (out) OODGAN_STRIP_LAUNCH(false, false); else OODGAN_STRIP_LAUNCH(false, true);
diff --git a/ood-gan-inversion_amd/csrc/common.hpp b/ood-gan-inversion_amd/csrc/common.hpp
--- a/ood-gan-inversion_amd/csrc/common.hpp
+++ b/ood-gan-inversion_amd/csrc/common.hpp
@@ -27,14 +27,14 @@
 
 void set_error(const char* fmt, ...);
 
-enum { OODGAN_TUN_S1_BIG_MIN_ITEMS = 0, OODGAN_TUN_S2_BIG_MIN_ITEMS, OODGAN_TUN_T2_BIG_MIN_ITEMS, OODGAN_TUN_BLURT_STRIP, OODGAN_TUN_BLUR_STRIP, OODGAN_TUN_UPVB_WAVES, OODGAN_TUN_FEWOUT_QUAD, OODGAN_TUN_TINY_MID_MAX, OODGAN_TUN_STRIPX_WAVES, OODGAN_TUN_COUNT };
+enum { OODGAN_TUN_S1_BIG_MIN_ITEMS = 0, OODGAN_TUN_S2_BIG_MIN_ITEMS, OODGAN_TUN_T2_BIG_MIN_ITEMS, OODGAN_TUN_BLURT_STRIP, OODGAN_TUN_BLUR_STRIP, OODGAN_TUN_UPVB_WAVES, OODGAN_TUN_FEWOUT_QUAD, OODGAN_TUN_TINY_MID_MAX, OODGAN_TUN_STRIPX_WAVES, OODGAN_TUN_DX_H16, OODGAN_TUN_COUNT };
 long tunable(int id);
 
 enum { OODGAN_DC_STRIPX = 0, OODGAN_DC_STRIP, OODGAN_DC_S1BIG, OODGAN_DC_S1V2, OODGAN_DC_S1PP, OODGAN_DC_TINY, OODGAN_DC_T2BIG,
        OODGAN_DC_T2V2, OODGAN_DC_T2GEN, OODGAN_DC_S2BIG, OODGAN_DC_S2V2, OODGAN_DC_S2GEN, OODGAN_DC_UPVB,
        OODGAN_DC_S1BIG_YS, OODGAN_DC_S2BIG_FUSE, OODGAN_DC_S2BIG_DOTXS,
        OODGAN_DC_S1BIG_G2, OODGAN_DC_S2BIG_G2, OODGAN_DC_STRIPX_G2, OODGAN_DC_S2BIG_XH, OODGAN_DC_S1BIG_XH,
-       OODGAN_DC_COMPOSITE_MSE, OODGAN_DC_COUNT };
+       OODGAN_DC_COMPOSITE_MSE, OODGAN_DC_S1BIG_DX16, OODGAN_DC_BLURT_IN16, OODGAN_DC_COUNT };
 void count_dispatch(int id);
 
 bool bound_device_ok(const char* what);
diff --git a/ood-gan-inversion_amd/csrc/conv_f16s.hip b/ood-gan-inversion_amd/csrc/conv_f16s.hip
--- a/ood-gan-inversion_amd/csrc/conv_f16s.hip
+++ b/ood-gan-inversion_amd/csrc/conv_f16s.hip
@@ -417,6 +417,10 @@
     return (H > 8 && W > 8 && !s1_strip_eligible(a) && s1_big_eligible(a)) ? 1 : 0;
 }
 
+extern "C" int oodgan_conv3x3_s1_dx16_supported(int B, int K, int M, int H, int W) {
+    return (tunable(OODGAN_TUN_DX_H16) != 0 && oodgan_conv3x3_s1_xh_supported(B, K, M, H, W) && oodgan_conv3x3_s1_actgrad_supported(B, K, M, H, W)) ? 1 : 0;
+}
+
 extern "C" int oodgan_conv3x3_s1_ys_supported(int B, int K, int M, int H, int W) {
     oodgan_conv_args a = {};
     a.mode = OODGAN_CONV_S1; a.x_sform = 1; a.B = B; a.K = K; a.M = M; a.Hin = H; a.Win = W;
@@ -458,6 +462,10 @@
                                         ((a.mode == OODGAN_CONV_S2 && s2_big_eligible(a)) || (a.mode == OODGAN_CONV_S1 && !s1_strip_eligible(a) && s1_big_eligible(a)))),
                    "conv3x3_f16s: x_hi_only = 2 (32-byte hi-only input records) exists only in the two-instruction 8-wave kernels (S-form input, dotx; mode S2 on a "
                    "shape oodgan_conv3x3_s2_fuse_supported accepts, mode S1 on a shape of the 8-wave stride-1 kernel)");
+    OODGAN_REQUIRE(!a.y_h16 || (a.mode == OODGAN_CONV_S1 && a.x_sform && a.dotx && a.dot_actgrad && a.x_hi_only && a.out_pitch == 0 && !tiny_eligible(a) &&
+                                !s1_strip_eligible(a) && s1_big_eligible(a)),
+                   "conv3x3_f16s: y_h16 (f16 planes of dx * act') exists only in the two-instruction dot_actgrad instance of the 8-wave stride-1 kernel "
+                   "(oodgan_conv3x3_s1_dx16_supported), dense rows");
     hipStream_t st = as_stream(stream);
     switch (a.mode) {
         case OODGAN_CONV_S1:
diff --git a/ood-gan-inversion_amd/csrc/conv_f16s_big.hip b/ood-gan-inversion_amd/csrc/conv_f16s_big.hip
--- a/ood-gan-inversion_amd/csrc/conv_f16s_big.hip
+++ b/ood-gan-inversion_amd/csrc/conv_f16s_big.hip
@@ -44,7 +44,7 @@
 __device__ long g_s1big_stamp_n = 0;
 #endif
 
-template <bool DOT, bool PRE, bool YS = false, bool G2 = false>
+template <bool DOT, bool PRE, bool YS = false, bool G2 = false, bool Y16 = false>
 __global__ __launch_bounds__(512) void conv_f16s_s1big_kernel(const BigConv p, const uint4* __restrict__ wpk16) {
     constexpr int NW = 8, NT = 2;
     extern __shared__ __attribute__((aligned(16))) unsigned char smem[];
@@ -261,6 +261,7 @@
 
     const float us = (p.w_unscale ? p.w_unscale[0] : 1.f) * (a.in_mul2 ? a.in_mul2[0] : 1.f);
     const float nw = (!DOT && a.noise) ? (a.noise_w ? a.noise_w[0] : 1.f) : 0.f;
+    const float usy = Y16 ? us * a.y_mul2[1] : us;
     float* red = reinterpret_cast<float*>(smem + BG_RED);
     float osc[16], bia[16], slp[16];
     unsigned moff[16], doff[16];
@@ -271,10 +272,10 @@
     for (int q = 0; q < 16; ++q) {
         const int j = 16 * (q >> 2) + 4 * g + (q & 3), m = m0 + j;
         const bool mok = m < M;
-        osc[q] = cst[j] * us;
+        osc[q] = cst[j] * usy;
         bia[q] = DOT ? 0.f : cst[64 + j];
         slp[q] = DOT ? 1.f : cst[128 + j];
-        moff[q] = mok ? (unsigned)((long)m * p.out_plane * 4) : 0xFFFFFFFFu;
+        moff[q] = mok ? (unsigned)((long)m * p.out_plane * (Y16 ? 2 : 4)) : 0xFFFFFFFFu;
         doff[q] = mok ? (unsigned)((long)m * H * W * 4) : 0u;
         dsum[q] = 0.f;
     }
@@ -293,7 +294,7 @@
         const bool ok = py < H && px < W;
         float nz = 0.f;
         if (has_nz) nz = nw * reinterpret_cast<const float*>(smem + BG_NZ)[wave * 64 + (n >> 1) * 32 + 16 * (n & 1) + n16];
-        unsigned char* yr = reinterpret_cast<unsigned char*>(a.y) + ((long)b * M * p.out_plane + (long)py * a.out_pitch + px) * 4;
+        unsigned char* yr = reinterpret_cast<unsigned char*>(a.y) + ((long)b * M * p.out_plane + (long)py * a.out_pitch + px) * (Y16 ? 2 : 4);
         const unsigned char* dr = DOT ? reinterpret_cast<const unsigned char*>(a.dotx) + ((long)b * M * H * W + (long)py * W + px) * 4 : nullptr;
         float o[16], dv[16];
         if (DOT) {
@@ -326,11 +327,17 @@
         if (ok && (!YS || a.y != nullptr)) {
             if (mfull) {
 #pragma unroll
-                for (int q = 0; q < 16; ++q) *reinterpret_cast<float*>(yr + moff[q]) = o[q];
+                for (int q = 0; q < 16; ++q) {
+                    if (Y16) *reinterpret_cast<_Float16*>(yr + moff[q]) = (_Float16)o[q];
+                    else *reinterpret_cast<float*>(yr + moff[q]) = o[q];
+                }
             } else {
 #pragma unroll
                 for (int q = 0; q < 16; ++q)
-                    if (moff[q] != 0xFFFFFFFFu) *reinterpret_cast<float*>(yr + moff[q]) = o[q];
+                    if (moff[q] != 0xFFFFFFFFu) {
+                        if (Y16) *reinterpret_cast<_Float16*>(yr + moff[q]) = (_Float16)o[q];
+                        else *reinterpret_cast<float*>(yr + moff[q]) = o[q];
+                    }
             }
         }
         if (YS && !DOT && ok) {
@@ -431,7 +438,8 @@
                         (void)hipFuncSetAttribute(reinterpret_cast<const void*>(&conv_f16s_s1big_kernel<false, false>), hipFuncAttributeMaxDynamicSharedMemorySize, BG_SMEM16),
                         (void)hipFuncSetAttribute(reinterpret_cast<const void*>(&conv_f16s_s1big_kernel<false, false, true>), hipFuncAttributeMaxDynamicSharedMemorySize, BG_SMEM16),
                         (void)hipFuncSetAttribute(reinterpret_cast<const void*>(&conv_f16s_s1big_kernel<true, false, false, true>), hipFuncAttributeMaxDynamicSharedMemorySize, BG_SMEM16),
-                        (void)hipFuncSetAttribute(reinterpret_cast<const void*>(&conv_f16s_s1big_kernel<true, true, false, true>), hipFuncAttributeMaxDynamicSharedMemorySize, BG_SMEM16), true);
+                        (void)hipFuncSetAttribute(reinterpret_cast<const void*>(&conv_f16s_s1big_kernel<true, true, false, true>), hipFuncAttributeMaxDynamicSharedMemorySize, BG_SMEM16),
+                        (void)hipFuncSetAttribute(reinterpret_cast<const void*>(&conv_f16s_s1big_kernel<true, true, false, true, true>), hipFuncAttributeMaxDynamicSharedMemorySize, BG_SMEM16), true);
     (void)once;
     const uint4* w16 = reinterpret_cast<const uint4*>(wpk16);
     OODGAN_REQUIRE(!a.dot_actgrad || a.dotx, "conv3x3 big: dot_actgrad without dotx");
@@ -439,7 +447,14 @@
     OODGAN_REQUIRE(a.x_hi_only != 2 || g2, "conv3x3 big: hi-only input records (x_hi_only = 2) need dotx (the two-instruction instances)");
     if (g2) count_dispatch(OODGAN_DC_S1BIG_G2);
     if (g2 && a.x_hi_only == 2) count_dispatch(OODGAN_DC_S1BIG_XH);
-    if (a.dot_actgrad && g2) hipLaunchKernelGGL((conv_f16s_s1big_kernel<true, true, false, true>), dim3((unsigned)total), dim3(512), BG_SMEM16, st, p, w16);
+    const bool y16 = a.y_h16 != 0;
+    OODGAN_REQUIRE(!y16 || (g2 && a.dot_actgrad && a.y && a.y_mul2 && (reinterpret_cast<uintptr_t>(a.y) & 1) == 0),
+                   "conv3x3 big: y_h16 needs x_hi_only, dot_actgrad, y and y_mul2 (oodgan_conv3x3_s1_dx16_supported)");
+    if (y16) {
+        count_dispatch(OODGAN_DC_S1BIG_DX16);
+        hipLaunchKernelGGL((conv_f16s_s1big_kernel<true, true, false, true, true>), dim3((unsigned)total), dim3(512), BG_SMEM16, st, p, w16);
+    }
+    else if (a.dot_actgrad && g2) hipLaunchKernelGGL((conv_f16s_s1big_kernel<true, true, false, true>), dim3((unsigned)total), dim3(512), BG_SMEM16, st, p, w16);
     else if (g2) hipLaunchKernelGGL((conv_f16s_s1big_kernel<true, false, false, true>), dim3((unsigned)total), dim3(512), BG_SMEM16, st, p, w16);
     else if (a.dot_actgrad) hipLaunchKernelGGL((conv_f16s_s1big_kernel<true, true>), dim3((unsigned)total), dim3(512), BG_SMEM16, st, p, w16);
     else if (a.dotx) hipLaunchKernelGGL((conv_f16s_s1big_kernel<true, false>), dim3((unsigned)total), dim3(512), BG_SMEM16, st, p, w16);
diff --git a/ood-gan-inversion_amd/csrc/runtime.hip b/ood-gan-inversion_amd/csrc/runtime.hip
--- a/ood-gan-inversion_amd/csrc/runtime.hip
+++ b/ood-gan-inversion_amd/csrc/runtime.hip
@@ -27,6 +27,7 @@
     {"fewout_quad", "OODGAN_FEWOUT_QUAD", 1, {0}, {0}},
     {"tiny_mid_max", "OODGAN_TINY_MID_MAX", 1024, {0}, {0}},
     {"stripx_waves", "OODGAN_STRIPX_WAVES", 4, {0}, {0}},
+    {"dx_h16", "OODGAN_DX_H16", 1, {0}, {0}},
 };
 }
 long tunable(int id) {
@@ -77,7 +78,7 @@
 
 namespace oodgan {
 namespace {
-const char* const g_dc_name[OODGAN_DC_COUNT] = {"stripx", "strip", "s1big", "s1v2", "s1pp", "tiny", "t2big", "t2v2", "t2gen", "s2big", "s2v2", "s2gen", "upvb", "s1big_ys", "s2big_fuse", "s2big_dotx_sform", "s1big_g2", "s2big_g2", "stripx_g2", "s2big_xh", "s1big_xh", "composite_mse"};
+const char* const g_dc_name[OODGAN_DC_COUNT] = {"stripx", "strip", "s1big", "s1v2", "s1pp", "tiny", "t2big", "t2v2", "t2gen", "s2big", "s2v2", "s2gen", "upvb", "s1big_ys", "s2big_fuse", "s2big_dotx_sform", "s1big_g2", "s2big_g2", "stripx_g2", "s2big_xh", "s1big_xh", "composite_mse", "s1big_dx16", "blurT_in16"};
 std::atomic<long> g_dc[OODGAN_DC_COUNT];
 }
 void count_dispatch(int id) { g_dc[id].fetch_add(1, std::memory_order_relaxed); }
@@ -167,7 +168,7 @@
     return OODGAN_OK;
 }
 
-extern "C" int oodgan_version(void) { return 110; }
+extern "C" int oodgan_version(void) { return 111; }
 extern "C" const char* oodgan_last_error(void) { return oodgan::g_err; }
 extern "C" int oodgan_device_count(void) {
     int n = 0;
diff --git a/ood-gan-inversion_amd/oodgan/_lib.py b/ood-gan-inversion_amd/oodgan/_lib.py
--- a/ood-gan-inversion_amd/oodgan/_lib.py
+++ b/ood-gan-inversion_amd/oodgan/_lib.py
@@ -11,7 +11,7 @@
 P = c_void_p
 
 
-ABI_VERSION = 110
+ABI_VERSION = 111
 
 
 class ConvArgs(Structure):
@@ -22,7 +22,7 @@
         ('in_pitch', c_int), ('out_pitch', c_int), ('in_scale_stride', c_int), ('out_scale_stride', c_int),
         ('noise_batch', c_int), ('mode', c_int), ('act', c_int), ('dot_nparts', c_int), ('in_mul2', P),
         ('x_sform', c_int), ('ys', P), ('ys_scale', P), ('ys_scale_stride', c_int),
-        ('rgb_w', P), ('rgb_s', P), ('rgb_y', P), ('rgb_s_stride', c_int), ('rgb_scale', c_float), ('fuse', P), ('dot_actgrad', c_int), ('groups', c_int), ('y_fform', c_int), ('x_fform', c_int), ('dotx_fform', c_int), ('dotx_sform', c_int), ('dotx_scale', P), ('dotx_scale_stride', c_int), ('workspace', P), ('workspace_bytes', c_long), ('ys_vmax', P), ('x_hi_only', c_int),
+        ('rgb_w', P), ('rgb_s', P), ('rgb_y', P), ('rgb_s_stride', c_int), ('rgb_scale', c_float), ('fuse', P), ('dot_actgrad', c_int), ('groups', c_int), ('y_fform', c_int), ('x_fform', c_int), ('dotx_fform', c_int), ('dotx_sform', c_int), ('dotx_scale', P), ('dotx_scale_stride', c_int), ('workspace', P), ('workspace_bytes', c_long), ('ys_vmax', P), ('x_hi_only', c_int), ('y_h16', c_int), ('y_mul2', P),
     ]
 
 
@@ -95,6 +95,9 @@
     'oodgan_avgpool': (c_int, [P, P, c_int, c_int, c_int, c_int, c_int, P]),
     'oodgan_blur_act_sform': (c_int, [P, P, P, P, P, c_int, P, P, c_int, P, c_int, c_int, c_int, c_int, c_int, c_int, P, P]),
     'oodgan_blur_act_sform_sep': (c_int, [P, P, P, P, P, c_int, P, P, c_int, P, c_int, c_int, c_int, c_int, c_int, c_int, P, c_int, P]),
+    'oodgan_conv3x3_s1_dx16_supported': (c_int, [c_int, c_int, c_int, c_int, c_int]),
+    'oodgan_act_bwd_blurT_in16_supported': (c_int, [c_int, c_int]),
+    'oodgan_act_bwd_blurT_sform_phases_hi16': (c_int, [P, P, c_int, P, P, P, c_int, P, P, P, P, P, c_int, c_int, c_int, c_int, P]),
     'oodgan_blur_act_fform': (c_int, [P, P, P, P, c_int, P, P, c_int, P, c_int, c_int, c_int, c_int, c_int, c_int, P, c_int, P]),
     'oodgan_conv3x3_xf_supported': (c_int, [c_int, c_int, c_int, c_int, c_int]),
     'oodgan_upconv_vblur_supported': (c_int, [c_int, c_int, c_int, c_int, c_int]),
diff --git a/ood-gan-inversion_amd/oodgan/engine.py b/ood-gan-inversion_amd/oodgan/engine.py
--- a/ood-gan-inversion_amd/oodgan/engine.py
+++ b/ood-gan-inversion_amd/oodgan/engine.py
@@ -153,6 +153,7 @@
         self.by_name = {L.name: L for L in layers}
         self.fuse_act_bwd = True
         self.hi_records = os.environ.get('OODGAN_HI_RECORDS', '1') != '0'
+        self.dx_h16 = True
         self.fused_rgb = True
         self.fuse_x = True
         self.fuse_up = True
@@ -565,9 +566,14 @@
                 if (L.kind == 'conv' and Lp is not None and Lp.kind == 'up' and self.fuse_act_bwd and self.bwd_state.get(L.src) is not None
                         and ops.s1_actgrad_supported(B, L.cout, L.cin, out.shape[2], out.shape[3])):
                     pre = ops.DotActGrad()
+                dx16 = None
+                Ho = x_in.shape[2]
+                if (pre is not None and self.grad_hi_only and self.dx_h16 and ops.s1_dx16_supported(B, L.cout, L.cin, Ho, Ho)
+                        and ops.blurT_in16_supported(Ho // 2, Ho // 2) and self._hi_records(B, Lp, Ho // 2, None)):
+                    dx16 = ops.half_planes_scratch(B, L.cin, Ho, Ho, self.device, tag='dx')
                 dx, dot = ops.conv3x3(gin, L.wpk_bwd, L.cin, CONV_S1 if L.kind == 'conv' else CONV_S2, out_scale=s, dotx=x_in,
                                       in_mul2=mul2, dot_into=_Cols(gs_all, L.row, L.cin), jobs=jobs, fuse=fz, want_y=fz is None,
-                                      dot_actgrad=pre)
+                                      dot_actgrad=pre, out=dx16, y_h16_mul2=self.bwd_state[L.src] if dx16 is not None else None)
                 fused_in, fused_pre = fz, pre
                 del gin
                 if deferred:
diff --git a/ood-gan-inversion_amd/oodgan/ops.py b/ood-gan-inversion_amd/oodgan/ops.py
--- a/ood-gan-inversion_amd/oodgan/ops.py
+++ b/ood-gan-inversion_amd/oodgan/ops.py
@@ -292,6 +292,22 @@
         return y
 
 
+def half_planes_scratch(B, C, H, W, device, tag=0):
+    key = ('h16', B, C, H, W, str(device), tag, _stream_handle())
+    buf = _SFORM_POOL.get(key)
+    if buf is None:
+        buf = _SFORM_POOL[key] = torch.empty(B, C, H, W, device=device, dtype=torch.float16)
+    return buf
+
+
+def s1_dx16_supported(B, K, M, H, W):
+    return bool(_lib.lib().oodgan_conv3x3_s1_dx16_supported(B, K, M, H, W))
+
+
+def blurT_in16_supported(H, W):
+    return bool(_lib.lib().oodgan_act_bwd_blurT_in16_supported(H, W))
+
+
 class SFormPhases:
     __slots__ = ('data', 'B', 'C', 'H', 'W', 'hi_only')
 
@@ -538,7 +554,8 @@
         assert g_feat is None and blur_kernel is None, 'F-form: the last styled conv only (no conv gradient, no blur)'
         o = out.data
     else:
-        o = _dev(g_feat, 'g_feat') if pre else _dev(out, 'out')
+        g16 = pre and g_feat.dtype == torch.float16
+        o = (g_feat if g16 else _dev(g_feat, 'g_feat')) if pre else _dev(out, 'out')
     B, C, H, W = o.shape
     L = _lib.lib()
     up = blur_kernel is not None
@@ -548,12 +565,17 @@
     part_t = torch.empty(B, C, npart, device=o.device, dtype=torch.float32) if g_rgb is not None else None
     part_m = torch.empty(B * KC * npart, device=o.device, dtype=torch.float32)
     nz = _opt(noise, 'noise')
-    common = [_p(_opt(g_feat, 'g_feat')), _p(None if pre else o), _p(nz), 1 if nz is None else nz.shape[0], _p(_opt(noise_weight, 'nw')),
+    common = [_p(o if pre else _opt(g_feat, 'g_feat')), _p(None if pre else o), _p(nz), 1 if nz is None else nz.shape[0], _p(_opt(noise_weight, 'nw')),
               _p(_opt(bias, 'bias')), _p(_opt(g_rgb, 'g_rgb')), _p(None if w_rgb is None else _dev(w_rgb).reshape(3, C)),
               _p(_opt(s_rgb, 's_rgb')), 0 if s_rgb is None else s_rgb.shape[1], 1.0 / math.sqrt(C), _p(_dev(dscale, 'dscale')),
               dscale.shape[1], _p(mul2)]
     if fform:
         check(L.oodgan_act_bwd_sform_f(*common[1:], _p(dst), _p(part_r), _p(part_t), _p(part_m), B, C, H, W, _stream()), 'act_bwd_sform_f')
+    elif up and pre and g16:
+        assert hi_only and g_rgb is None and g_feat.is_contiguous()
+        check(L.oodgan_act_bwd_blurT_sform_phases_hi16(common[0], *common[2:6], *common[11:], _p(_dev(blur_kernel)), _p(dst), _p(part_r), _p(part_m),
+                                                       B, C, H // 2, W // 2, _stream()), 'act_bwd_blurT_sform_phases_hi16')
+        dst.hi_only = True
     elif up and hi_only:
         assert g_rgb is None and part_t is None
         check(L.oodgan_act_bwd_blurT_sform_phases_hi(*common[:6], *common[11:], _p(_dev(blur_kernel)), _p(dst), _p(part_r), _p(part_m),
@@ -753,7 +775,7 @@
 def conv3x3(x, wpk, M, mode=CONV_S1, in_scale=None, in_shift=None, out_scale=None, bias=None, noise=None,
             noise_weight=None, act=ACT_NONE, slope=None, dotx=None, in_hw=None, in_pitch=0, out=None, out_pitch=0,
             in_mul2=None, ys=None, ys_scale=None, want_y=True, dot_into=None, rgb=None, jobs=None, fuse=None, dot_actgrad=None,
-            groups=1, y_fform=False, xf_act=None, tiny_max=8, vmax=None):
+            groups=1, y_fform=False, xf_act=None, tiny_max=8, vmax=None, y_h16_mul2=None):
     sform_in = isinstance(x, (SForm, SFormPhases))
     fform_in = isinstance(x, FForm)
     if fform_in:
@@ -776,6 +798,9 @@
         out = torch.empty(B, M, oh, pitch, device=x.data.device if (sform_in or fform_in) else x.device, dtype=torch.float32)
     a = ConvArgs()
     a.x, a.wpk, a.y = _p(x), _p(wpk), _p(out)
+    if y_h16_mul2 is not None:
+        assert out is not None and out.dtype == torch.float16 and tuple(out.shape) == (B, M, oh, ow) and dot_actgrad is not None
+        a.y_h16, a.y_mul2 = 1, _p(y_h16_mul2)
     a.in_scale, a.in_shift, a.out_scale = _p(_opt(in_scale, 'in_scale')), _p(_opt(in_shift, 'in_shift')), _p(_opt(out_scale, 'out_scale'))
     a.bias, a.noise, a.noise_w, a.slope = _p(_opt(bias, 'bias')), _p(_opt(noise, 'noise')), _p(_opt(noise_weight, 'nw')), _p(_opt(slope, 'slope'))
     a.B, a.K, a.M, a.Hin, a.Win = B, K, M, H, W
```

Measured after the change: 8.198, median of 2. About the same (+0.8%).
